# Shmaug/Stratum

Hardware: AMD Instinct MI355X
Metric: Mray/s at 1920x1080x1spp (1M-tri scene) (higher is better)
Workload: dtype f32; 1 GPU; procedural atrium, 1002352 triangles, 1920x1080, 1 sample(s)/pixel/step, default BDPT flags, radiance + albedo/visibility/depth/prev-uv AOVs written, pixel-tile shard 64x32 over 1 GPU(s); parallelism=single GPU, exchange=none, world_size=1, backend=none

## Files before the change

__graft_entry__.py:

```python
import os
import subprocess
import sys

ROOT = os.path.dirname(os.path.abspath(__file__))
if ROOT not in sys.path:
    sys.path.insert(0, ROOT)

CSRC = os.path.join(ROOT, "stratum_amd", "csrc")
LIB = os.path.join(ROOT, "stratum_amd", "libstratum_hip.so")

HIPCC_FLAGS = [
    "--offload-arch=gfx950",
    "-O3",
    "-std=c++17",
    "-fPIC",
    "-shared",
    "-ffp-contract=off",
    "-fno-fast-math",
    "-Wall",
    "-Wno-cuda-compat",
]


PRODUCT_SOURCES = ("api.hip", "shade_plain.hip", "shade_lt.hip", "shade_media.hip", "shade_media_lt.hip", "shade_media_lt2.hip", "trace_kernels.hip", "lbvh.hip", "lvc.hip", "hashgrid.hip", "wide.hip", "bvh_build.cpp",
                   "hdr_writer.cpp")


def _newer(target, sources):
    if not os.path.exists(target):
        return True
    t = os.path.getmtime(target)
    return any(os.path.getmtime(s) > t for s in sources)


def build_product(force=False):
    srcs = [os.path.join(CSRC, f) for f in PRODUCT_SOURCES]
    deps = srcs + [os.path.join(CSRC, f) for f in os.listdir(CSRC) if f.endswith(".h")]
    deps += [os.path.join(ROOT, "include", f) for f in os.listdir(os.path.join(ROOT, "include"))]
    if force or _newer(LIB, deps):
        from concurrent.futures import ThreadPoolExecutor

        hipcc = os.environ.get("HIPCC", "/opt/rocm/bin/hipcc")
        objdir = os.path.join(ROOT, "stratum_amd", "_obj")
        os.makedirs(objdir, exist_ok=True)
        compile_flags = [f for f in HIPCC_FLAGS if f != "-shared"]
        objs = [os.path.join(objdir, os.path.basename(s) + ".o") for s in srcs]

        headers = [d for d in deps if d not in srcs] + [os.path.abspath(__file__)]

        def compile_one(pair):
            src, obj = pair
            if force or _newer(obj, [src] + headers):
                subprocess.check_call([hipcc] + compile_flags + ["-c", "-o", obj, src])

        with ThreadPoolExecutor(max_workers=min(len(srcs), os.cpu_count() or 1)) as pool:
            list(pool.map(compile_one, zip(srcs, objs)))
        subprocess.check_call([hipcc, "--offload-arch=gfx950", "-shared", "-fPIC", "-o", LIB] + objs)
# ... 88 lines not shown
```

include/sthip.h:

```cpp
#ifndef STHIP_H
#define STHIP_H

#include <stdint.h>
#include "sthip_wire.h"

#ifdef __cplusplus
extern "C" {
#endif

#define STHIP_ABI_VERSION 11

typedef struct sthip_ctx sthip_ctx;

enum sthip_status {
  STHIP_OK = 0,
  STHIP_ERR_INVALID_ARGUMENT = -1,
  STHIP_ERR_NO_DEVICE = -2,
  STHIP_ERR_HIP = -3,
  STHIP_ERR_UNSUPPORTED = -4,
  STHIP_ERR_NO_SCENE = -5
};

typedef struct sthip_image_desc {
  const float* pixels;
// ... 120 lines not shown
  uint64_t rays_total;
  uint64_t rays_path;
  uint64_t rays_shadow;
  uint64_t nodes_visited;
  uint64_t tris_tested;
  uint64_t nodes_visited_shadow;
  uint64_t tris_tested_shadow;
  float ms_trace;
  float ms_shade;
  float ms_total;
  uint32_t launches_trace;
  uint32_t bvh_node_bytes;
  uint32_t bvh_tri_bytes;
  uint64_t bvh_nodes;
  uint64_t bvh_tris;
  float bvh_build_ms;
  float bvh_build_gpu_ms;
  uint64_t inner_slots[2];
  uint64_t tri_slots[2];
  uint64_t round_slots[2];
  uint64_t busy_rounds[2];
  uint64_t rays_primary_packets;
  uint64_t nodes_visited_primary;
  uint64_t tris_tested_primary;
  float ms_trace_primary;
  uint32_t launches_primary;
  uint64_t lane_states[8];
  uint64_t rays_answered;
  uint32_t paths_per_seed;
  uint32_t seeds_in_flight;
  uint64_t max_paths_in_flight;
  uint32_t batch_halvings;
  uint32_t full_rebuilds;
} sthip_stats;
int sthip_get_stats(sthip_ctx* ctx, sthip_stats* out);

enum { STHIP_CEILING_TRIAD = 0, STHIP_CEILING_NODE_GATHER_TABLE = 1, STHIP_CEILING_NODE_GATHER_L2 = 2, STHIP_CEILING_NODE_GATHER_L1 = 3 };
int sthip_measure_ceiling(sthip_ctx* ctx, uint32_t kind, double* gbytes_per_s);

int sthip_set_option(sthip_ctx* ctx, const char* name, int64_t value);


typedef struct sthip_accumulate_desc {
  uint32_t width, height;
  uint32_t view_count;
  uint32_t reprojection;
  uint32_t demodulate_albedo;
  float history_limit;
  uint32_t device_ptrs;
  uint32_t instance_count;
  const sthip_ViewData* gViews;
  const float* gRadiance;
  const float* gAlbedo;
  const sthip_VisibilityInfo* gVisibility;
  const sthip_DepthInfo* gDepth;
  const float* gPrevUVs;
  const sthip_VisibilityInfo* gPrevVisibility;
  const sthip_DepthInfo* gPrevDepth;
  const float* gPrevAccumColor;
  const float* gPrevAccumMoments;
  const uint32_t* gInstanceIndexMap;
  float* gAccumColor;
  float* gAccumMoments;
} sthip_accumulate_desc;
int sthip_accumulate(sthip_ctx* ctx, const sthip_accumulate_desc* desc);

// ... 43 lines not shown
```

stratum_amd/csrc/api.hip:

```cpp
#include <hip/hip_runtime.h>
#include <stdio.h>
#include <stdlib.h>
#include <string.h>

#include <algorithm>
#include <chrono>
#include <string>
#include <vector>

#include "../../include/sthip.h"
#include "bvh_build.h"
#include "kernel_instances.h"
#include "post.h"
#include "ceilings.h"

STHIP_DECLARE_KERNEL_INSTANCES

namespace sthip {
hipError_t lvc_compact(const float4* staging, uint32_t slots_per_seed, uint32_t seeds, uint32_t vertices_per_seed, float4* cache, uint32_t* counts, uint32_t* flags, uint32_t* offsets,
                       void* tmp, size_t& tmp_bytes, hipStream_t stream, uint32_t rec = 4, uint32_t flag_at = 2);
hipError_t hashgrid_build_device(const uint2* keys, const uint32_t* count, uint32_t slots, uint32_t buckets, uint32_t* checksums, uint32_t* counters, uint32_t* indices, uint32_t* dest, uint32_t* owner,
                                 uint32_t* bucket_of, uint32_t* append_index, uint32_t* sorted_bucket, uint32_t* sorted_append, unsigned long long* key64, unsigned long long* sorted_key64, void* tmp,
                                 size_t& tmp_bytes, hipStream_t stream, bool force_serial = false);
}
// ... 143 lines not shown
  std::vector<uint8_t> materials_host;
  std::vector<std::pair<uint32_t, uint32_t>> image_dims;
  uint32_t distribution_count = 0;
  bool has_specular = false;
  DevBuf<sthip_PackedVertexData> vertices;
  DevBuf<uint8_t> indices;
  DevBuf<sthip_InstanceData> instances;
  DevBuf<sthip_TransformData> xf, inv_xf, motion_xf;
  DevBuf<uint8_t> materials;
  DevBuf<uint32_t> lights;
  DevBuf<DeviceImage> images;
  DevBuf<float4> image_texels;
  uint32_t image_count = 0;
  DevBuf<float2> cone;
  uint32_t instance_count = 0, light_count = 0;
  DevBuf<BvhNodeSlot> nodes;
  DevBuf<BvhTri> tris;
  DevBuf<TlasEntry> entries;
  DevBuf<WideNode> wide_nodes;
  DevBuf<TlasEntry> wide_entries;
  DevBuf<Wide8Node> wide8_nodes;
  DevBuf<TlasEntry> wide8_entries;
  std::vector<Wide8Node> wide8_host;
  size_t wide8_node_count = 0;
  uint32_t tri_min_lanes = 1;
  DeviceBvh bvh{};
  uint64_t bvh_nodes = 0, bvh_tris = 0;
  PinnedNodes nodes_host;
  DevBuf<BvhNode> raw_nodes;
  DevBuf<BvhNodePacked> top_nodes;
  DevBuf<TlasEntry> top_entries;
  bool use_treetop = false;
  bool embed_leaves = false;
  int use_wide = 1;
  size_t wide_node_count = 0;
  sthip::DeviceWideScratch* wide_scratch = nullptr;
  bool want_wide = false;
  bool lds_materials = true;
  DevBuf<uint8_t> views;
  DevBuf<float4> ray_o, ray_d, hit, beta, radiance, shadow_sum, accum, shadow_rays, light_vertices, conn, media_state, shadow_hit, shadow_ext, shadow_result;
  DevBuf<uint32_t> view_medium;
  DevBuf<uint32_t> meta, queue0, queue1, queue_kept;
  int cull_terminal = 1;
  DevBuf<unsigned long long> counters;
  DevBuf<float> distributions;
  DevBuf<float4> presampled;
  DevBuf<float4> bdpt;
  DevBuf<float4> rr;
  DevBuf<uint2> cs_nee, cs_lvc;
  DevBuf<float4> lvc_staging, path_contrib;
  DevBuf<uint32_t> lvc_count, lvc_flags, lvc_offsets;
  DevBuf<uint8_t> lvc_tmp;
  DevBuf<float4> hg_appends, hg_compact, hg_data;
  DevBuf<uint32_t> hg_count, hg_flags, hg_offsets, hg_dest, hg_checksums, hg_counters, hg_indices;
  DevBuf<uint32_t> hg_owner, hg_bucket_of, hg_append, hg_sorted_bucket, hg_sorted_append;
  DevBuf<unsigned long long> hg_key64, hg_sorted_key64;
  DevBuf<uint2> hg_keys;
  DevBuf<uint8_t> hg_tmp;
  DevBuf<float4> lg_appends, lg_compact, lg_data;
  DevBuf<uint32_t> lg_checksums, lg_counters, lg_indices;
  DevBuf<uint32_t> light_trace;
  DevBuf<DeviceImage1> images1;
  DevBuf<float> image1_texels;
  DevBuf<BvhTriUv> tri_uvs;
  DevBuf<BvhTriShade> tri_shade;
  DevBuf<uint32_t> hit_leaf;
// ... 33 lines not shown
  DevBuf<float4> deep_rays;
  DevBuf<uint32_t> deep_count;
  sthip_stats stats{};
  hipError_t last_hip_error = hipSuccess;
  bool render_launched = false;
  bool stats_pending = false;
  hipEvent_t ev[2] = {nullptr, nullptr};
};

#define STHIP_MAX_STACK_LDS ((size_t)152 * 1024)
#define STHIP_MAX_STACK_DEPTH 512u

static const void* trace_kernel(bool count, bool alpha, bool bounded, bool top) {
  static const void* const table[16] = {
      (const void*)&k_trace<false, false, false, false>, (const void*)&k_trace<true, false, false, false>, (const void*)&k_trace<false, true, false, false>, (const void*)&k_trace<true, true, false, false>,
      (const void*)&k_trace<false, false, true, false>,  (const void*)&k_trace<true, false, true, false>,  (const void*)&k_trace<false, true, true, false>,  (const void*)&k_trace<true, true, true, false>,
      (const void*)&k_trace<false, false, false, true>,  (const void*)&k_trace<true, false, false, true>,  (const void*)&k_trace<false, true, false, true>,  (const void*)&k_trace<true, true, false, true>,
      (const void*)&k_trace<false, false, true, true>,   (const void*)&k_trace<true, false, true, true>,   (const void*)&k_trace<false, true, true, true>,   (const void*)&k_trace<true, true, true, true>};
  return table[(count ? 1 : 0) | (alpha ? 2 : 0) | (bounded ? 4 : 0) | (top ? 8 : 0)];
}
static const void* trace_kernel_wide8(bool count, bool alpha, bool bounded) {
  static const void* const table[8] = {
      (const void*)&k_trace<false, false, false, false, 2>, (const void*)&k_trace<true, false, false, false, 2>, (const void*)&k_trace<false, true, false, false, 2>, (const void*)&k_trace<true, true, false, false, 2>,
      (const void*)&k_trace<false, false, true, false, 2>,  (const void*)&k_trace<true, false, true, false, 2>,  (const void*)&k_trace<false, true, true, false, 2>,  (const void*)&k_trace<true, true, true, false, 2>};
  return table[(count ? 1 : 0) | (alpha ? 2 : 0) | (bounded ? 4 : 0)];
}
static const void* trace_kernel_wide(bool count, bool alpha, bool bounded) {
  static const void* const table[8] = {
      (const void*)&k_trace<false, false, false, false, 1>, (const void*)&k_trace<true, false, false, false, 1>, (const void*)&k_trace<false, true, false, false, 1>, (const void*)&k_trace<true, true, false, false, 1>,
      (const void*)&k_trace<false, false, true, false, 1>,  (const void*)&k_trace<true, false, true, false, 1>,  (const void*)&k_trace<false, true, true, false, 1>,  (const void*)&k_trace<true, true, true, false, 1>};
  return table[(count ? 1 : 0) | (alpha ? 2 : 0) | (bounded ? 4 : 0)];
}

#define HIP_TRY(ctx, expr)                                                                            \
  do {                                                                                                \
    hipError_t _e = (expr);                                                                           \
    if (_e != hipSuccess) {                                                                           \
      (ctx)->error = std::string(#expr) + ": " + hipGetErrorString(_e);                               \
      (ctx)->last_hip_error = _e;                                                                     \
      return STHIP_ERR_HIP;                                                                           \
    }                                                                                                 \
  } while (0)

static void fill_counter_stats(sthip_ctx* ctx, const unsigned long long* c) {
  ctx->stats.rays_total = c[CNT_RAYS_CLOSEST] + c[CNT_RAYS_SHADOW];
  ctx->stats.rays_path = c[CNT_RAYS_CLOSEST] - c[CNT_CROSSINGS];
  ctx->stats.rays_shadow = c[CNT_RAYS_SHADOW];
  ctx->stats.nodes_visited = c[CNT_NODES];
  ctx->stats.tris_tested = c[CNT_TRIS];
  ctx->stats.nodes_visited_shadow = c[CNT_NODES + 1];
  ctx->stats.tris_tested_shadow = c[CNT_TRIS + 1];
  for (int k = 0; k < 2; k++) {
    ctx->stats.inner_slots[k] = c[CNT_INNER_SLOTS + k];
    ctx->stats.tri_slots[k] = c[CNT_TRI_SLOTS + k];
    ctx->stats.round_slots[k] = c[CNT_ROUND_SLOTS + k];
    ctx->stats.busy_rounds[k] = c[CNT_BUSY_ROUNDS + k];
  }
  for (int k = 0; k < 8; k++) ctx->stats.lane_states[k] = c[CNT_LANE_STATES + k];
  ctx->stats.rays_answered = c[CNT_RAYS_ANSWERED];
  ctx->stats.nodes_visited_primary = c[CNT_NODES_PRIMARY];
  ctx->stats.tris_tested_primary = c[CNT_TRIS_PRIMARY];
}

static uint32_t grid_for_early(const sthip_ctx* ctx, size_t n) {
  const size_t blocks = (n + STHIP_BLOCK - 1) / STHIP_BLOCK;
  return (uint32_t)std::max<size_t>(1, std::min(blocks, (size_t)ctx->cu_count * 32));
}

static int fail(sthip_ctx* ctx, int code, const std::string& msg) {
  ctx->error = msg;
  return code;
}

extern "C" {

int sthip_abi_version(void) { return STHIP_ABI_VERSION; }

int sthip_create(int device, sthip_ctx** out_ctx) {
  if (!out_ctx) {
    g_create_error = "out_ctx is NULL";
    return STHIP_ERR_INVALID_ARGUMENT;
  }
  *out_ctx = nullptr;
  int count = 0;
  hipError_t e = hipGetDeviceCount(&count);
  if (e != hipSuccess || count == 0) {
    g_create_error = std::string("no HIP device: ") + (e != hipSuccess ? hipGetErrorString(e) : "device count is 0") +
                     " (libstratum_hip has no CPU backend)";
    return STHIP_ERR_NO_DEVICE;
  }
  if (device < 0 || device >= count) {
    g_create_error = "device index out of range";
    return STHIP_ERR_INVALID_ARGUMENT;
  }
  e = hipSetDevice(device);
  if (e != hipSuccess) {
    g_create_error = std::string("hipSetDevice: ") + hipGetErrorString(e);
    return STHIP_ERR_HIP;
  }
  sthip_ctx* ctx = new sthip_ctx();
  ctx->device = device;
  hipDeviceProp_t prop;
  if (hipGetDeviceProperties(&prop, device) == hipSuccess) {
    ctx->cu_count = prop.multiProcessorCount;
    size_t free_bytes = 0, total_bytes = 0;
    if (hipMemGetInfo(&free_bytes, &total_bytes) != hipSuccess) free_bytes = prop.totalGlobalMem;
    uint64_t paths = 1ull << 18;
    while (paths * 2 * 4096 <= (uint64_t)free_bytes && paths < (1ull << 27)) paths *= 2;
    ctx->max_paths_in_flight = paths;
  }
  (void)hipEventCreate(&ctx->ev[0]);
  (void)hipEventCreate(&ctx->ev[1]);
  {
    const int lds_max = 160 * 1024;
    for (int k = 0; k < 16; k++) (void)hipFuncSetAttribute(trace_kernel((k & 1) != 0, (k & 2) != 0, (k & 4) != 0, (k & 8) != 0), hipFuncAttributeMaxDynamicSharedMemorySize, lds_max);
    for (int k = 0; k < 8; k++) (void)hipFuncSetAttribute(trace_kernel_wide((k & 1) != 0, (k & 2) != 0, (k & 4) != 0), hipFuncAttributeMaxDynamicSharedMemorySize, lds_max);
    for (int k = 0; k < 8; k++) (void)hipFuncSetAttribute(trace_kernel_wide8((k & 1) != 0, (k & 2) != 0, (k & 4) != 0), hipFuncAttributeMaxDynamicSharedMemorySize, lds_max);
    (void)hipFuncSetAttribute(reinterpret_cast<const void*>(&k_trace_batch<false, false>), hipFuncAttributeMaxDynamicSharedMemorySize, lds_max);
    (void)hipFuncSetAttribute(reinterpret_cast<const void*>(&k_trace_batch<true, false>), hipFuncAttributeMaxDynamicSharedMemorySize, lds_max);
    (void)hipFuncSetAttribute(reinterpret_cast<const void*>(&k_trace_batch<false, true>), hipFuncAttributeMaxDynamicSharedMemorySize, lds_max);
    (void)hipFuncSetAttribute(reinterpret_cast<const void*>(&k_trace_batch<true, true>), hipFuncAttributeMaxDynamicSharedMemorySize, lds_max);
  }
  ctx->stats.bvh_node_bytes = sizeof(BvhNodePacked);
  ctx->stats.bvh_tri_bytes = sizeof(BvhTri);
  *out_ctx = ctx;
  return STHIP_OK;
}

void sthip_destroy(sthip_ctx* ctx) {
  if (!ctx) return;
  (void)hipSetDevice(ctx->device);
  (void)hipDeviceSynchronize();
  sthip::device_wide_scratch_destroy(ctx->wide_scratch);
  ctx->wide_scratch = nullptr;
  ctx->vertices.release();
  ctx->volume_words.release();
  ctx->volumes.release();
  ctx->indices.release();
  ctx->instances.release();
  ctx->xf.release();
  ctx->inv_xf.release();
  ctx->motion_xf.release();
  ctx->materials.release();
  ctx->lights.release();
  ctx->images.release();
  ctx->image_texels.release();
  ctx->cone.release();
  ctx->nodes.release();
  ctx->tris.release();
  ctx->entries.release();
// ... 56 lines not shown
int sthip_set_shard(sthip_ctx* ctx, uint32_t shard_rank, uint32_t shard_count, uint32_t tile_w, uint32_t tile_h) {
  if (!ctx) return STHIP_ERR_INVALID_ARGUMENT;
  if (shard_count == 0 || shard_rank >= shard_count || tile_w == 0 || tile_h == 0 || (tile_w & 7u) || (tile_h & 7u))
    return fail(ctx, STHIP_ERR_INVALID_ARGUMENT, "shard: need rank < count and tile sizes that are multiples of 8");
  ctx->shard_rank = shard_rank;
  ctx->shard_count = shard_count;
  ctx->tile_w = tile_w;
  ctx->tile_h = tile_h;
  return STHIP_OK;
}

int sthip_set_option(sthip_ctx* ctx, const char* name, int64_t value) {
  if (!ctx || !name) return STHIP_ERR_INVALID_ARGUMENT;
  if (!strcmp(name, "count_traversal"))
    ctx->count_traversal = value != 0;
  else if (!strcmp(name, "time_kernels"))
    ctx->time_kernels = value != 0;
  else if (!strcmp(name, "fuse_trace"))
    ctx->fuse_trace = value != 0;
  else if (!strcmp(name, "packet_primary"))
    ctx->packet_primary = value != 0;
  else if (!strcmp(name, "answer_last_rays"))
    ctx->answer_last_rays = value != 0;
  else if (!strcmp(name, "cull_terminal"))
    ctx->cull_terminal = value != 0;
  else if (!strcmp(name, "refill_idle"))
    ctx->refill_idle = (uint32_t)std::min<int64_t>(64, std::max<int64_t>(1, value));
  else if (!strcmp(name, "bvh_builder"))
    ctx->bvh_builder = value == 1 ? 1 : 0;
  else if (!strcmp(name, "lds_materials"))
    ctx->lds_materials = value != 0;
  else if (!strcmp(name, "embed_leaves"))
    ctx->embed_leaves = value != 0;
  else if (!strcmp(name, "keep_scene")) {
    ctx->keep_scene = value != 0;
    if (!ctx->keep_scene) ctx->kept = KeptScene();
  } else if (!strcmp(name, "wide_bvh"))
    ctx->use_wide = (int)std::min<int64_t>(std::max<int64_t>(value, 0), 3);
  else if (!strcmp(name, "poison_deep_queue")) {
    if (value && ctx->deep_count.p) {
      const uint32_t junk[2] = {5u, 3u};
      (void)hipSetDevice(ctx->device);
      (void)hipStreamSynchronize(ctx->stream);
      if (hipMemcpy(ctx->deep_count.p, junk, 8, hipMemcpyHostToDevice) != hipSuccess) return fail(ctx, STHIP_ERR_HIP, "poison_deep_queue: copy failed");
    }
  } else if (!strcmp(name, "tri_min_lanes"))
    ctx->tri_min_lanes = ctx->bvh.wide8_tri_min = (uint32_t)std::min<int64_t>(std::max<int64_t>(value, 1), 64);
  else if (!strcmp(name, "lbvh_algorithm"))
    ctx->lbvh_algorithm = value == 0 ? 0 : 1;
  else if (!strcmp(name, "lds_stack_levels")) {
    ctx->lds_stack_cap = ctx->lds_stack_threshold = (uint32_t)std::min<int64_t>(std::max<int64_t>(value, 4), 150);
  } else if (!strcmp(name, "ploc_radius"))
    ctx->ploc_radius = (int)std::min<int64_t>(std::max<int64_t>(value, 1), 32);
  else if (!strcmp(name, "sah_top"))
    ctx->sah_top_size = value <= 0 ? 0u : (uint32_t)std::min<int64_t>(std::max<int64_t>(value, 16), 1 << 20);
  else if (!strcmp(name, "max_paths_in_flight"))
    ctx->max_paths_in_flight = (uint64_t)std::max<int64_t>(1, value);
  else if (!strcmp(name, "trace_blocks_per_cu"))
    ctx->trace_blocks_per_cu = (uint32_t)std::min<int64_t>(16, std::max<int64_t>(0, value));
  else if (!strcmp(name, "treetop"))
    ctx->use_treetop = value != 0;
  else if (!strcmp(name, "hashgrid_serial"))
    ctx->hashgrid_serial = value != 0;
  else if (!strcmp(name, "reuse_grids_persist")) {
    ctx->reuse_persist = value != 0;
    ctx->reuse_grids_valid = false;
// ... 174 lines not shown
  if (s->image_count && !s->gImages) return fail(ctx, STHIP_ERR_INVALID_ARGUMENT, "scene: image_count > 0 but gImages is NULL");
  if (s->image1_count && !s->gImage1s) return fail(ctx, STHIP_ERR_INVALID_ARGUMENT, "scene: image1_count > 0 but gImage1s is NULL");
  if (s->volume_count && !s->gVolumes) return fail(ctx, STHIP_ERR_INVALID_ARGUMENT, "scene: volume_count > 0 but gVolumes is NULL");
  sthip::BuiltBvh built;
  std::string err;
  const uint32_t n = s->instance_count;
  const bool device_build = ctx->bvh_builder == sthip::BVH_BUILDER_LBVH_GPU;
  sthip::DeviceBuildTarget target;
  if (device_build) {
    ctx->has_scene = false;
    HIP_TRY(ctx, ctx->vertices.ensure(std::max(1u, s->vertex_count)));
    HIP_TRY(ctx, ctx->indices.ensure((size_t)s->indices_bytes + 8));
    if (s->vertex_count) HIP_TRY(ctx, hipMemcpy(ctx->vertices.p, s->gVertices, (size_t)s->vertex_count * sizeof(sthip_PackedVertexData), hipMemcpyHostToDevice));
    HIP_TRY(ctx, hipMemset(ctx->indices.p + s->indices_bytes, 0, 8));
    if (s->indices_bytes) HIP_TRY(ctx, hipMemcpy(ctx->indices.p, s->gIndices, s->indices_bytes, hipMemcpyHostToDevice));
    target.vertices = ctx->vertices.p;
    target.vertex_count = s->vertex_count;
    target.indices = ctx->indices.p;
    target.stream = ctx->stream;
    target.algorithm = ctx->lbvh_algorithm;
    target.ploc_radius = ctx->ploc_radius;
    target.sah_top_size = ctx->lbvh_algorithm == 1 ? ctx->sah_top_size : 0;
    target.user = ctx;
    target.reserve = [](void* user, size_t node_capacity, size_t tri_capacity, sthip::DeviceBuildTarget& self) {
      sthip_ctx* c = (sthip_ctx*)user;
      if (c->nodes.ensure(node_capacity) != hipSuccess || c->raw_nodes.ensure(node_capacity) != hipSuccess || c->tris.ensure(tri_capacity) != hipSuccess) return false;
      self.nodes = c->nodes.p;
      self.raw_nodes = c->raw_nodes.p;
      self.tris = c->tris.p;
      return true;
    };
  }
  const auto t_build0 = std::chrono::steady_clock::now();
  if (!sthip::build_scene_bvh(*s, built, err, ctx->bvh_builder, device_build ? &target : nullptr, ctx->embed_leaves && STHIP_NODE_STRIDE == 48))
    return fail(ctx, err.find("only triangle") != std::string::npos ? STHIP_ERR_UNSUPPORTED : STHIP_ERR_INVALID_ARGUMENT, "scene: " + err);

  if (((size_t)built.dev_nodes + built.nodes.size() + 2 * built.entries.size() + 2) * sizeof(BvhNodeSlot) > 0xFFFFFFFFull || ((size_t)built.dev_tris + built.tris.size()) * sizeof(BvhTri) > 0xFFFFFFFFull)
    return fail(ctx, STHIP_ERR_UNSUPPORTED, "scene: the acceleration structure exceeds 4 GiB (the traversal addresses nodes and triangles with 32-bit byte offsets)");
  if (built.stack_depth > STHIP_MAX_STACK_DEPTH) return fail(ctx, STHIP_ERR_UNSUPPORTED, "scene: the acceleration structure is too deep for the traversal stack (use the SAH builder)");
  ctx->stats.bvh_build_ms = std::chrono::duration<float, std::milli>(std::chrono::steady_clock::now() - t_build0).count();
  ctx->stats.bvh_build_gpu_ms = built.gpu_build_ms;
  {
    std::vector<EmitterBounds> bounds;
    bool usable = true;
    for (uint32_t i = 0; i < s->instance_count && usable; i++) {
      if ((s->gInstances[i].packed[0] & 0xF) != STHIP_INSTANCE_TYPE_TRIANGLES || !(ctx->inst_flags_host[i] & INST_FLAG_EMITS)) continue;
      if (bounds.size() == STHIP_MAX_EMITTER_BOUNDS) {
        usable = false;
        break;
      }
      const uint32_t prims = (s->gInstances[i].packed[1] >> 12) & 0xFFFFu, stride = s->gInstances[i].packed[1] >> 28;
      const uint32_t first_vertex = s->gInstances[i].packed[2];
      const uint8_t* ib = (const uint8_t*)s->gIndices + s->gInstances[i].packed[3];
      EmitterBounds b{};
      for (int a = 0; a < 3; a++) b.lo[a] = __builtin_inff(), b.hi[a] = -__builtin_inff();
      for (uint32_t k = 0; k < 3 * prims; k++) {
        uint32_t index;
        if (stride == 2) {
          uint16_t w;
          memcpy(&w, ib + 2 * (size_t)k, 2);
          index = w;
        } else {
          memcpy(&index, ib + 4 * (size_t)k, 4);
        }
        if ((size_t)first_vertex + index >= s->vertex_count) {
          usable = false;
          break;
// ... 195 lines not shown
    ctx->bvh.image1_texels = ctx->image1_texels.p;
    ctx->bvh.alpha_test = 0;
    ctx->bvh.flip_uvs = 0;
  }
  {
    size_t words = 0;
    for (uint32_t i = 0; i < s->volume_count; i++) {
      built.volumes[i].first_word = (uint32_t)words;
      words += (size_t)(s->gVolumes[i].bytes / 4);
    }
    if (words > 0xFFFFFFFFull) return fail(ctx, STHIP_ERR_INVALID_ARGUMENT, "scene: gVolumes exceed 16 GiB");
    HIP_TRY(ctx, ctx->volume_words.ensure(std::max<size_t>(1, words)));
    HIP_TRY(ctx, ctx->volumes.ensure(std::max<size_t>(1, built.volumes.size())));
    for (uint32_t i = 0; i < s->volume_count; i++)
      HIP_TRY(ctx, hipMemcpy(ctx->volume_words.p + built.volumes[i].first_word, s->gVolumes[i].data, (size_t)s->gVolumes[i].bytes, hipMemcpyHostToDevice));
    if (!built.volumes.empty()) HIP_TRY(ctx, hipMemcpy(ctx->volumes.p, built.volumes.data(), built.volumes.size() * sizeof(DeviceVolume), hipMemcpyHostToDevice));
    ctx->volume_count = s->volume_count;
    ctx->has_volumes = false;
    ctx->volume_instances = 0;
    ctx->instance_is_volume.assign(n, 0);
    for (uint32_t i = 0; i < n; i++)
      if ((s->gInstances[i].packed[0] & 0xF) == STHIP_INSTANCE_TYPE_VOLUME) {
        ctx->has_volumes = true;
        ctx->volume_instances++;
        ctx->instance_is_volume[i] = 1;
      }
    ctx->bvh.volumes = ctx->volumes.p;
  }
  ctx->bvh.nodes = reinterpret_cast<const float4*>(ctx->nodes.p);
  ctx->bvh.tris = built.embedded ? reinterpret_cast<const float4*>(ctx->nodes.p) : reinterpret_cast<const float4*>(ctx->tris.p);
  ctx->bvh.entries = ctx->entries.p;
  ctx->bvh.root_ref = built.root_ref;
  ctx->bvh.top_is_world_blas = built.top_is_world_blas;
  ctx->bvh.stack_depth = built.stack_depth;
  ctx->bvh.scene_cx = built.scene_center[0];
  ctx->bvh.scene_cy = built.scene_center[1];
  ctx->bvh.scene_cz = built.scene_center[2];
  ctx->bvh.scene_radius = built.scene_radius;
  ctx->bvh_nodes = nodes_total;
  ctx->bvh_tris = tris_total;
  ctx->top = std::move(built.top);
  if (ctx->want_wide && built.dev_nodes != 0) {
    const int rc = collapse_resident_tree(ctx);
    if (rc != STHIP_OK) return rc;
  }
  ctx->nodes_host.n = 0;
  if (ctx->use_treetop) {
    HIP_TRY(ctx, ctx->nodes_host.ensure(std::max<size_t>(nodes_total, ctx->nodes.n)));
    if (built.dev_nodes) HIP_TRY(ctx, hipMemcpy(ctx->nodes_host.p, ctx->raw_nodes.p, (size_t)built.dev_nodes * sizeof(BvhNode), hipMemcpyDeviceToHost));
    if (!built.nodes.empty()) memcpy(ctx->nodes_host.p + built.dev_nodes, built.nodes.data(), built.nodes.size() * sizeof(BvhNode));
    ctx->nodes_host.n = nodes_total;
  }
  {
    const size_t units = built.embedded ? nodes_total : tris_total;
    HIP_TRY(ctx, ctx->tri_shade.ensure(std::max<size_t>(1, units)));
    if (ctx->has_alpha) {
      HIP_TRY(ctx, ctx->tri_uvs.ensure(std::max<size_t>(1, units)));
      ctx->bvh.tri_uv = reinterpret_cast<const float2*>(ctx->tri_uvs.p);
    }
    if (units && s->vertex_count) {
      DevBuf<uint8_t> is_tri;
      if (built.embedded) {
        std::vector<uint8_t> flags(units, 0);
        for (size_t u = 0; u < built.unit_tri.size() && u < units; u++) flags[u] = built.unit_tri[u] != 0xFFFFFFFFu;
        HIP_TRY(ctx, is_tri.ensure(units));
        HIP_TRY(ctx, hipMemcpy(is_tri.p, flags.data(), units, hipMemcpyHostToDevice));
      }
      hipLaunchKernelGGL(k_fill_tri_shade, dim3(grid_for_early(ctx, units)), dim3(STHIP_BLOCK), 0, ctx->stream, reinterpret_cast<const BvhTri*>(ctx->bvh.tris), (uint32_t)units, is_tri.p, ctx->vertices.p, s->vertex_count,
                         ctx->indices.p, (uint64_t)s->indices_bytes, ctx->tri_shade.p, ctx->has_alpha ? ctx->tri_uvs.p : nullptr);
      HIP_TRY(ctx, hipGetLastError());
      HIP_TRY(ctx, hipStreamSynchronize(ctx->stream));
    }
  }
  {
    const int rc = configure_stack(ctx);
    if (rc != STHIP_OK) return rc;
  }
  ctx->has_scene = true;
  ctx->reuse_grids_valid = false;
  if (ctx->keep_scene) {
    if (s->gVertices != ctx->kept.vertices.data() || !ctx->kept.valid) ctx->kept.keep(*s);
  } else {
    ctx->kept = KeptScene();
  }
  if (getenv("STHIP_VERBOSE")) {
    int per_cu = 0;
    per_cu = trace_occupancy(ctx, trace_lds_bytes(ctx));
    fprintf(stderr, "[sthip] bvh (%s): %zu nodes, %zu tris, %zu top-level entries, stack depth %u (%zu B LDS / block%s, treetop %u nodes), %d trace blocks / CU, build %.1f ms (GPU kernels %.2f ms)\n",
            ctx->bvh_builder ? "lbvh/gpu" : "sah/host", (size_t)ctx->bvh_nodes, (size_t)ctx->bvh_tris, built.entries.size(), built.stack_depth, stack_bytes(ctx), ctx->bvh.spill ? ", bounded" : "", ctx->bvh.top_count, per_cu, ctx->stats.bvh_build_ms,
            ctx->stats.bvh_build_gpu_ms);
  }
  return STHIP_OK;
}

static unsigned long long* queue_ctl_host(unsigned long long* qctl, uint32_t kind, uint32_t depth) {
  return qctl + (size_t)((kind * 64u + depth) * QUEUE_SEGMENTS) * QCTL_STRIDE;
}
static uint32_t grid_for(const sthip_ctx* ctx, size_t n) {
  const size_t blocks = (n + STHIP_BLOCK - 1) / STHIP_BLOCK;
  const size_t cap = (size_t)ctx->cu_count * 32;
  return (uint32_t)std::max<size_t>(1, std::min(blocks, cap));
}
static int trace_occupancy(const sthip_ctx* ctx, size_t lds_bytes) {
  int per_cu = 0;
  hipError_t e;
  e = hipOccupancyMaxActiveBlocksPerMultiprocessor(&per_cu,
                                                   ctx->bvh.wide8_nodes  ? trace_kernel_wide8(false, false, ctx->bvh.spill != nullptr)
                                                   : ctx->bvh.wide_nodes ? trace_kernel_wide(false, false, ctx->bvh.spill != nullptr)
                                                                         : trace_kernel(false, false, ctx->bvh.spill != nullptr, ctx->use_treetop),
                                                   STHIP_BLOCK, lds_bytes);
  return e == hipSuccess ? per_cu : 0;
}
static uint32_t trace_grid(sthip_ctx* ctx, size_t lds_bytes) {
  int per_cu = trace_occupancy(ctx, lds_bytes);
  if (per_cu < 1) per_cu = 2;
  if (ctx->trace_blocks_per_cu) per_cu = (int)ctx->trace_blocks_per_cu;
  return (uint32_t)(ctx->cu_count * per_cu);
}
static size_t stack_bytes(const sthip_ctx* ctx) { return (size_t)ctx->bvh.lds_levels * STHIP_BLOCK * (ctx->bvh.wide8_nodes ? sizeof(uint2) : sizeof(uint32_t)); }

static size_t trace_lds_bytes(const sthip_ctx* ctx) { return stack_bytes(ctx) + (size_t)ctx->bvh.top_count * sizeof(BvhNodePacked); }

static int configure_stack(sthip_ctx* ctx) {
  const uint32_t need = ctx->bvh.wide8_nodes ? ctx->bvh.wide8_stack_depth : ctx->bvh.wide_nodes ? ctx->bvh.wide_stack_depth + 3u : ctx->bvh.stack_depth;
  const bool bounded = ctx->bvh.wide8_nodes ? 2u * need > ctx->lds_stack_threshold : need > ctx->lds_stack_threshold;
  ctx->bvh.lds_levels = bounded ? (ctx->bvh.wide8_nodes ? std::max(4u, ctx->lds_stack_cap / 2u) : ctx->lds_stack_cap) : need;
  ctx->bvh.spill = nullptr;
  if (bounded) {
    HIP_TRY(ctx, ctx->spill.ensure((size_t)ctx->cu_count * 8 * STHIP_BLOCK * ctx->bvh.stack_depth));
    ctx->bvh.spill = ctx->spill.p;
  }
  return refresh_treetop(ctx);
}

static int refresh_treetop(sthip_ctx* ctx) {
  ctx->bvh.top_nodes = nullptr;
  ctx->bvh.top_entries = ctx->bvh.entries;
  ctx->bvh.top_root_ref = ctx->bvh.root_ref;
  ctx->bvh.top_count = 0;
  if (!ctx->use_treetop || ctx->nodes_host.empty()) return STHIP_OK;
  int per_cu = 0;
  const size_t stack = stack_bytes(ctx);
  per_cu = trace_occupancy(ctx, stack);
// ... 711 lines not shown
      HIP_TRY(ctx, hipEventElapsedTime(&ms, ctx->ev[0], ctx->ev[1]));
      acc += ms;
    }
    return STHIP_OK;
  };

  ctx->render_launched = true;
  if (ctx->bvh.spill && ctx->deep_count.p) HIP_TRY(ctx, hipMemsetAsync(ctx->deep_count.p, 0, 8, st));
  bool counters_cleared = false;
  const bool nee = (sampling_flags & (1u << STHIP_eNEE)) != 0;
  const bool ext = ctx->has_spheres || has_env || bdpt || (sampling_flags & ((1u << STHIP_eNEEReservoirs) | (1u << STHIP_eShadingNormalShadowFix)));
  for (uint32_t s = 0; s < seed_count; s += batch) {
    const uint32_t in_flight = std::min(batch, seed_count - s);
    p.seed = seed_begin + s;
    p.seeds_in_flight = in_flight;
    p.write_aov = s == 0 ? 1u : 0u;
    int rc = STHIP_OK;
    auto reset_queues = [&]() -> int {
      const uint32_t per_depth = QUEUE_SEGMENTS * QCTL_STRIDE;
      const uint32_t words = (max_bounce_rounds + drain_rounds + 1) * per_depth;
      hipLaunchKernelGGL(k_clear, dim3(std::max(1u, std::min(64u, (2 * words + CNT_TOTAL + STHIP_BLOCK - 1) / STHIP_BLOCK))), dim3(STHIP_BLOCK), 0, st, queue_ctl_host(ctx->qctl.p, 0, 0), words,
                         queue_ctl_host(ctx->qctl.p, 1, 0), words, ctx->counters.p, counters_cleared ? 0u : (uint32_t)CNT_TOTAL);
      counters_cleared = true;
      if (p.shadow_debug) HIP_TRY(ctx, hipMemsetAsync(queue_ctl_host(ctx->qctl.p, 2, 0), 0, (size_t)words * 8, st));
      HIP_TRY(ctx, hipGetLastError());
      return STHIP_OK;
    };
    auto trace = [&](uint32_t dc, uint32_t ds) -> int {
      if (dc == TRACE_NONE && ds == TRACE_NONE) return STHIP_OK;
      launches_trace++;
      return timed(ms_trace, [&]() {
        const bool alpha = p.bvh.alpha_test || ctx->has_volumes;
        void* kargs[3] = {(void*)&p, (void*)&dc, (void*)&ds};
        (void)hipLaunchKernel(p.bvh.wide8_nodes  ? trace_kernel_wide8(ctx->count_traversal, alpha, p.bvh.spill != nullptr)
                              : p.bvh.wide_nodes ? trace_kernel_wide(ctx->count_traversal, alpha, p.bvh.spill != nullptr)
                                                 : trace_kernel(ctx->count_traversal, alpha, p.bvh.spill != nullptr, p.bvh.top_count != 0),
                              dim3(tgrid), dim3(STHIP_BLOCK), kargs, lds, st);
        if (p.bvh.spill) {
          const uint32_t dgrid = (uint32_t)ctx->cu_count * 8u;
          if (alpha) {
            if (ctx->count_traversal)
              hipLaunchKernelGGL((k_trace_deep<true, true>), dim3(dgrid), dim3(STHIP_BLOCK), 0, st, p);
            else
              hipLaunchKernelGGL((k_trace_deep<false, true>), dim3(dgrid), dim3(STHIP_BLOCK), 0, st, p);
          } else if (ctx->count_traversal)
            hipLaunchKernelGGL((k_trace_deep<true, false>), dim3(dgrid), dim3(STHIP_BLOCK), 0, st, p);
          else
            hipLaunchKernelGGL((k_trace_deep<false, false>), dim3(dgrid), dim3(STHIP_BLOCK), 0, st, p);
        }
        if (p.shadow_debug && ds != TRACE_NONE) {
          FrameParams q = p;
          q.shadow_rays = p.shadow_debug;
          q.radiance = p.debug;
          q.shadow_sum = p.debug;
          q.qctl = p.qctl + (size_t)64 * QUEUE_SEGMENTS * QCTL_STRIDE;
          const uint32_t none = TRACE_NONE;
          void* qargs[3] = {(void*)&q, (void*)&none, (void*)&ds};
          (void)hipLaunchKernel(p.bvh.wide8_nodes  ? trace_kernel_wide8(false, alpha, p.bvh.spill != nullptr)
                                : p.bvh.wide_nodes ? trace_kernel_wide(false, alpha, p.bvh.spill != nullptr)
                                                   : trace_kernel(false, alpha, p.bvh.spill != nullptr, p.bvh.top_count != 0),
                                dim3(tgrid), dim3(STHIP_BLOCK), qargs, lds, st);
          if (p.bvh.spill) {
            const uint32_t dgrid = (uint32_t)ctx->cu_count * 8u;
            if (alpha)
              hipLaunchKernelGGL((k_trace_deep<false, true>), dim3(dgrid), dim3(STHIP_BLOCK), 0, st, q);
            else
              hipLaunchKernelGGL((k_trace_deep<false, false>), dim3(dgrid), dim3(STHIP_BLOCK), 0, st, q);
          }
        }
      });
    };
    auto trace_primary = [&]() -> int {
      launches_primary++;
      rays_primary += (uint64_t)primary_rays * in_flight;
      const uint32_t packets = (p.path_count + 63) / 64;
      const unsigned pgrid = std::max(1u, std::min((packets + 3) / 4, (uint32_t)ctx->cu_count * 64u));
      const size_t plds = ((size_t)ctx->bvh.stack_depth * (STHIP_BLOCK / 64) + 13 * STHIP_BLOCK) * sizeof(uint32_t);
      return timed(ms_primary, [&]() {
        if (p.bvh.alpha_test) {
          if (ctx->count_traversal)
            hipLaunchKernelGGL((k_trace_primary<true, true>), dim3(pgrid), dim3(STHIP_BLOCK), plds, st, p);
          else
            hipLaunchKernelGGL((k_trace_primary<false, true>), dim3(pgrid), dim3(STHIP_BLOCK), plds, st, p);
        } else if (ctx->count_traversal)
          hipLaunchKernelGGL((k_trace_primary<true, false>), dim3(pgrid), dim3(STHIP_BLOCK), plds, st, p);
        else
          hipLaunchKernelGGL((k_trace_primary<false, false>), dim3(pgrid), dim3(STHIP_BLOCK), plds, st, p);
      });
    };
    auto run_rounds = [&](bool light, bool shadow_rays, auto&& shade) -> int {
      for (uint32_t depth = 0; depth <= max_bounce_rounds; depth++) {
        const uint32_t dc = depth < max_bounce_rounds ? depth : TRACE_NONE;
        const uint32_t ds = depth >= 1 && shadow_rays && depth - 1 <= max_shadow_round ? depth - 1 : TRACE_NONE;
        int r;
        if (!light && depth == 0 && dc == 0 && ctx->packet_primary && !ctx->has_volumes) {
          r = trace_primary();
        } else if (ctx->fuse_trace) {
          r = trace(dc, ds);
        } else {
          r = trace(TRACE_NONE, ds);
          if (!r) r = trace(dc, TRACE_NONE);
        }
        if (r) return r;
        if (media && ds != TRACE_NONE) {
          r = timed(ms_shade, [&]() { hipLaunchKernelGGL(k_shadow_media, dim3(grid), dim3(STHIP_BLOCK), 0, st, p, ds); });
          if (r) return r;
        }
        if (dc == TRACE_NONE) break;
        r = timed(ms_shade, [&]() { shade(depth); });
        if (r) return r;
      }
      if (media && shadow_rays)
        for (uint32_t ds = max_bounce_rounds; ds < max_bounce_rounds + drain_rounds; ds++) {
          int r = trace(TRACE_NONE, ds);
          if (!r) r = timed(ms_shade, [&]() { hipLaunchKernelGGL(k_shadow_media, dim3(grid), dim3(STHIP_BLOCK), 0, st, p, ds); });
          if (r) return r;
        }
      return STHIP_OK;
    };

// ... 539 lines not shown
```

stratum_amd/csrc/bvh.h:

```cpp
#pragma once
#include <stdint.h>

#define BVH_LEAF_BIT 0x80000000u
#define BVH_INST_BIT 0x40000000u
#define BVH_TOP_BIT 0x40000000u
#define BVH_MAX_LEAF_TRIS 2
#define BVH_INVALID_REF 0xFFFFFFFFu

struct BvhNode {
  float n0xy[4];
  float n1xy[4];
  float nz[4];
  uint32_t ref[4];
};

struct BvhTri {
  float v0[3];
  uint32_t id;
  float v1[3];
  uint32_t src_indices;
  float v2[3];
  uint32_t src_vertex;
};
struct BvhTriShade {
  float n0[3], v0;
  float n1[3], v1;
  float n2[3], v2;
  float u[3], pad;
};
struct BvhNodePacked {
  float n0xy[4];
  float n1xy[4];
  float nz[4];
};
#ifndef STHIP_NODE_STRIDE
#define STHIP_NODE_STRIDE 48
#endif
#define BVH_NODE_BYTES ((unsigned)STHIP_NODE_STRIDE)
struct BvhNodeSlot {
  BvhNodePacked n;
#if STHIP_NODE_STRIDE > 48
  uint32_t pad[(STHIP_NODE_STRIDE - 48) / 4];
#endif
};
struct WideNode {
  float origin[3];
  uint8_t exp[4];
  uint8_t q[6][4];
  uint32_t pad[2];
  uint32_t ref[4];
};
struct Wide8Node {
  float origin[3];
  uint8_t exp[3];
  uint8_t imask;
  uint32_t child_base;
// ... 47 lines not shown
```

stratum_amd/csrc/bvh_build.cpp:

```cpp
#include "bvh_build.h"

#include <math.h>
#include <cmath>
#include <stdlib.h>
#include <string.h>

#include <algorithm>
#include <atomic>
#include <limits>
#include <map>
#include <queue>
#include <thread>
#include <unordered_map>
#include <tuple>

namespace sthip {
namespace {

struct Box {
  float lo[3], hi[3];
  void reset() {
    for (int a = 0; a < 3; a++) {
      lo[a] = INFINITY;
      hi[a] = -INFINITY;
// ... 246 lines not shown
  return memcmp(&t, I, sizeof(I)) == 0;
}

struct InstView {
  uint32_t type, material_address, prim_count, stride, first_vertex, indices_byte_offset;
};
inline InstView view(const sthip_InstanceData& d) {
  InstView v;
  v.type = d.packed[0] & 0xF;
  v.material_address = d.packed[0] >> 4;
  v.prim_count = (d.packed[1] >> 12) & 0xFFFF;
  v.stride = d.packed[1] >> 28;
  v.first_vertex = d.packed[2];
  v.indices_byte_offset = d.packed[3];
  return v;
}
inline void load_tri(const sthip_scene_desc& s, const InstView& in, uint32_t prim, uint32_t tri[3]) {
  const uint8_t* ib = (const uint8_t*)s.gIndices;
  const size_t off = (size_t)in.indices_byte_offset + (size_t)prim * 3 * in.stride;
  if (in.stride == 2) {
    uint16_t w[3];
    memcpy(w, ib + off, 6);
    tri[0] = w[0];
    tri[1] = w[1];
    tri[2] = w[2];
  } else {
    memcpy(tri, ib + off, 12);
  }
  for (int k = 0; k < 3; k++) tri[k] += in.first_vertex;
}

}

bool build_scene_bvh(const sthip_scene_desc& s, BuiltBvh& out, std::string& err, int builder, DeviceBuildTarget* device, bool embed_leaves) {
  out = BuiltBvh();
  const bool dev_mode = device != nullptr && builder == BVH_BUILDER_LBVH_GPU;
  const uint32_t DEVICE_MIN_PRIMS = 64;
  out.embedded = embed_leaves && builder == BVH_BUILDER_SAH_HOST;
  const uint32_t BLAS_DEPTH_CAP = 22, TLAS_DEPTH_CAP = 18, LBVH_MAX_HEIGHT = 120;
  if (s.indices_bytes > 0xFFFFFFFFull || s.vertex_count >= 0x80000000u) {
    err = "gIndices beyond 4 GiB or more than 2^31 vertices";
    return false;
  }
  std::vector<uint32_t> merged, separate, spheres, volumes;
  for (uint32_t i = 0; i < s.volume_count; i++) {
    const uint8_t* b = (const uint8_t*)s.gVolumes[i].data;
    const uint64_t n = s.gVolumes[i].bytes;
    auto rd32 = [&](uint64_t off) { uint32_t v = 0; if (off + 4 <= n) memcpy(&v, b + off, 4); return v; };
    auto rd64 = [&](uint64_t off) { uint64_t v = 0; if (off + 8 <= n) memcpy(&v, b + off, 8); return v; };
    auto rdf = [&](uint64_t off) { float v = 0; if (off + 4 <= n) memcpy(&v, b + off, 4); return v; };
    if (!b || n < 672 + 64 + 64 || n > 0xFFFFFFF0ull || (n & 3) || rd64(0) != 0x304244566f6e614eull || rd32(636) != 1u) {
      err = "gVolumes entry is not a NanoVDB float grid (magic / grid type / size)";
      return false;
    }
    DeviceVolume v;
    memset(&v, 0, sizeof(v));
    v.bytes = (uint32_t)n;
    const uint64_t root = 672 + rd64(672 + 24);
    if (root + 64 > n) {
      err = "gVolumes entry: the root node lies outside the buffer";
      return false;
    }
    v.root = (uint32_t)root;
    const uint64_t tiles = rd32(root + 24);
    if (tiles > 65536 || root + 64 + 32 * tiles > n) {
      err = "gVolumes entry: the root tile table lies outside the buffer";
      return false;
// ... 39 lines not shown
      continue;
    }
    if (in.type != STHIP_INSTANCE_TYPE_TRIANGLES) {
      err = "unknown instance type";
      return false;
    }
    if (in.stride != 2 && in.stride != 4) {
      err = "index stride must be 2 or 4";
      return false;
    }
    const size_t end = (size_t)in.indices_byte_offset + (size_t)in.prim_count * 3 * in.stride;
    if (end > s.indices_bytes) {
      err = "instance index range exceeds gIndices";
      return false;
    }
    if ((size_t)in.material_address + sizeof(sthip_MaterialRecord) > s.material_bytes) {
      err = "instance material_address exceeds gMaterialData";
      return false;
    }
    if (!dev_mode)
      for (uint32_t p = 0; p < in.prim_count; p++) {
        uint32_t tri[3];
        load_tri(s, in, p, tri);
        for (int k = 0; k < 3; k++)
          if (tri[k] >= s.vertex_count) {
            err = "vertex index exceeds gVertices";
            return false;
          }
      }
    if (is_identity(s.gInstanceInverseTransforms[i]) && is_identity(s.gInstanceTransforms[i]))
      merged.push_back(i);
    else
      separate.push_back(i);
  }

  std::vector<uint32_t> inst_alpha(s.instance_count, BVH_NO_ALPHA);
  bool any_alpha = false;
  for (uint32_t i = 0; i < s.instance_count; i++) {
    const InstView in = view(s.gInstances[i]);
    if (in.type != STHIP_INSTANCE_TYPE_TRIANGLES) continue;
    sthip_MaterialRecord rec;
    memcpy(&rec, (const uint8_t*)s.gMaterialData + in.material_address, sizeof(rec));
    if (rec.alpha_mask_index < STHIP_IMAGE_COUNT) {
      if (rec.alpha_mask_index >= s.image1_count) {
        err = "a material refers to an alpha mask that is not in gImage1s";
        return false;
      }
      inst_alpha[i] = rec.alpha_mask_index;
      any_alpha = true;
    }
  }

  std::string gpu_err;
  auto prim_total = [&](const std::vector<uint32_t>& insts) {
    size_t n = 0;
    for (uint32_t i : insts) n += view(s.gInstances[i]).prim_count;
    return n;
  };
  uint32_t dev_node_cursor = 0, dev_tri_cursor = 0;
  if (dev_mode) {
    size_t dev_nodes = 0, dev_tris = 0, all_prims = 0, meshes_n = 0;
    auto account = [&](size_t n) {
      if (n == 0) return;
      all_prims += n;
      meshes_n++;
      if (n >= DEVICE_MIN_PRIMS) {
// ... 88 lines not shown
      std::vector<BvhTri> tin(prims.size());
      bounds.reset();
      for (size_t k = 0; k < prims.size(); k++) {
        const InstView in = view(s.gInstances[prims[k].first]);
        uint32_t tri[3];
        load_tri(s, in, prims[k].second, tri);
        BvhTri& t = tin[k];
        memcpy(t.v0, s.gVertices[tri[0]].position, 12);
        memcpy(t.v1, s.gVertices[tri[1]].position, 12);
        memcpy(t.v2, s.gVertices[tri[2]].position, 12);
        t.id = (prims[k].second << 16) | (with_instance_bits ? prims[k].first : 0u);
        t.src_indices = in.indices_byte_offset + prims[k].second * 3u * in.stride;
        t.src_vertex = in.first_vertex | (in.stride == 4u ? 0x80000000u : 0u);
        bounds.grow(t.v0);
        bounds.grow(t.v1);
        bounds.grow(t.v2);
      }
      uint32_t root = 0;
      float ms = 0;
      const size_t nodes_before = out.nodes.size(), tris_before = out.tris.size();
      if (!lbvh_build_gpu(tin, out.nodes, out.tris, root, depth, ms, gpu_err)) return BVH_INVALID_REF;
      out.gpu_build_ms += ms;
      if (depth <= LBVH_MAX_HEIGHT) return root;
      out.nodes.resize(nodes_before);
      out.tris.resize(tris_before);
    }
    std::vector<Box> boxes(prims.size());
    bounds.reset();
    for (size_t k = 0; k < prims.size(); k++) {
      const InstView in = view(s.gInstances[prims[k].first]);
      uint32_t tri[3];
      load_tri(s, in, prims[k].second, tri);
      boxes[k].reset();
      for (int v = 0; v < 3; v++) boxes[k].grow(s.gVertices[tri[v]].position);
      bounds.grow(boxes[k]);
    }
    uint32_t leaf_tris = BVH_MAX_LEAF_TRIS;
    if (const char* e = getenv("STHIP_LEAF_TRIS")) leaf_tris = (uint32_t)std::min(4, std::max(1, atoi(e)));
    Builder b(boxes, leaf_tris, BLAS_DEPTH_CAP);
    depth = b.max_depth;
    const uint32_t tri_base = (uint32_t)out.tris.size();
    out.tris.resize(tri_base + prims.size());
    for (size_t k = 0; k < prims.size(); k++) {
      const auto& pr = prims[b.order[k]];
      const InstView in = view(s.gInstances[pr.first]);
      uint32_t tri[3];
      load_tri(s, in, pr.second, tri);
      BvhTri& t = out.tris[tri_base + k];
      memcpy(t.v0, s.gVertices[tri[0]].position, 12);
      memcpy(t.v1, s.gVertices[tri[1]].position, 12);
      memcpy(t.v2, s.gVertices[tri[2]].position, 12);
      t.id = (pr.second << 16) | (with_instance_bits ? pr.first : 0u);
      t.src_indices = in.indices_byte_offset + pr.second * 3u * in.stride;
      t.src_vertex = in.first_vertex | (in.stride == 4u ? 0x80000000u : 0u);
    }
    const uint32_t root = flatten(b, 0, out.nodes, [&](uint32_t first, uint32_t count) {
      if (!out.embedded) return BVH_LEAF_BIT | ((tri_base + first) << 2) | (count - 1);
      out.unit_tri.resize(out.nodes.size(), 0xFFFFFFFFu);
      const uint32_t unit = (uint32_t)out.nodes.size();
      for (uint32_t k = 0; k < count; k++) {
        out.nodes.push_back(BvhNode());
        memset(&out.nodes.back(), 0, sizeof(BvhNode));
        out.unit_tri.push_back(tri_base + first + k);
      }
      return BVH_LEAF_BIT | (unit << 2) | (count - 1);
    });
    if (root & BVH_LEAF_BIT) {
      depth = 1;
      return wrap_leaf(out.nodes, bounds, root);
    }
    return root;
  };

  Box scene_box;
  scene_box.reset();
  uint32_t blas_depth = 0;
  std::vector<Box> entry_boxes;

  std::vector<uint8_t> entry_root_local;
  if (!merged.empty()) {
    const size_t total = prim_total(merged);
    if (total > 0) {
      if (total >= (1u << 28)) {
        err = "too many triangles";
        return false;
      }
      Box bounds;
// ... 109 lines not shown
    memset(&e, 0, sizeof(e));
    memcpy(e.inv, &s.gInstanceInverseTransforms[i], 48);
    e.root = s.gInstances[i].packed[2];
    e.id_bits = i;
    e.identity = TLAS_ENTRY_VOLUME;
    const DeviceVolume& v = out.volumes[e.root];
    const sthip_TransformData& xf = s.gInstanceTransforms[i];
    Box wb;
    wb.reset();
    for (int c = 0; c < 8; c++) {
      const float ip[3] = {(float)((c & 1) ? v.bbox_max[0] + 1 : v.bbox_min[0]), (float)((c & 2) ? v.bbox_max[1] + 1 : v.bbox_min[1]), (float)((c & 4) ? v.bbox_max[2] + 1 : v.bbox_min[2])};
      float gw[3], wp[3];
      for (int a = 0; a < 3; a++) gw[a] = ip[0] * v.matf[3 * a] + ip[1] * v.matf[3 * a + 1] + ip[2] * v.matf[3 * a + 2] + v.vecf[a];
      for (int a = 0; a < 3; a++) wp[a] = xf.m[a][0] * gw[0] + xf.m[a][1] * gw[1] + xf.m[a][2] * gw[2] + xf.m[a][3];
      wb.grow(wp);
    }
    for (int a = 0; a < 3; a++) {
      const float pad = 1e-3f * (wb.hi[a] - wb.lo[a]) + 1e-5f * std::max(fabsf(wb.lo[a]), fabsf(wb.hi[a]));
      wb.lo[a] -= pad;
      wb.hi[a] += pad;
    }
    out.entries.push_back(e);
    entry_boxes.push_back(wb);
    scene_box.grow(wb);
  }

  if (dev_mode)
    for (size_t k = 0; k < entry_root_local.size(); k++)
      if (entry_root_local[k]) out.entries[k].root += out.dev_nodes;
  out.top.entries = out.entries;
  out.top.volumes = out.volumes;
  out.top.instance_count = s.instance_count;
  out.top.merged.assign(s.instance_count, 0);
  for (uint32_t i : merged) out.top.merged[i] = 1;
  out.top.blas_nodes = out.dev_nodes + (uint32_t)out.nodes.size();
  out.top.blas_depth = blas_depth;
  out.top.obj_box.assign(6 * out.entries.size(), 0.f);
  for (size_t k = 0; k < out.entries.size(); k++) {
    const TlasEntry& e = out.entries[k];
    if (e.identity == TLAS_ENTRY_IDENTITY) {
      out.top.has_merged = true;
      memcpy(out.top.merged_box, entry_boxes[k].lo, 12);
      memcpy(out.top.merged_box + 3, entry_boxes[k].hi, 12);
    } else if (e.identity == TLAS_ENTRY_TRANSFORMED) {
      const InstView in = view(s.gInstances[e.id_bits]);
      const Box& ob = meshes.at(std::make_tuple(in.first_vertex, in.indices_byte_offset, in.prim_count, in.stride)).bounds;
      memcpy(&out.top.obj_box[6 * k], ob.lo, 12);
      memcpy(&out.top.obj_box[6 * k + 3], ob.hi, 12);
    }
  }

  uint32_t tlas_depth = 0;
  if (out.entries.empty()) {
    out.root_ref = BVH_INVALID_REF;
    out.top_is_world_blas = 1;
  } else if (out.entries.size() == 1 && out.entries[0].identity == TLAS_ENTRY_IDENTITY) {
    out.root_ref = out.entries[0].root;
    out.top_is_world_blas = 1;
  } else {
    if (out.entries.size() >= 0xFFFE) {
      err = "too many top-level entries";
      return false;
    }
    Builder b(entry_boxes, 1, TLAS_DEPTH_CAP);
    tlas_depth = b.max_depth + 1;
    out.root_ref = flatten(b, 0, out.nodes, [&](uint32_t first, uint32_t) { return BVH_LEAF_BIT | BVH_INST_BIT | b.order[first]; });
    if (out.root_ref & BVH_LEAF_BIT) {
// ... 642 lines not shown
  wide8_stack_depth = 0;
  if (st.wide8_root.size() != st.entries.size() || root_ref == BVH_INVALID_REF) return false;
  if (top_is_world_blas) {
    if (st.entries.empty() || st.wide8_root[0] == BVH_INVALID_REF) return false;
    entries = st.entries;
    for (size_t k = 0; k < entries.size(); k++)
      if (st.wide8_root[k] != BVH_INVALID_REF) entries[k].root = st.wide8_root[k];
    wide8_root = st.wide8_root[0];
    wide8_stack_depth = (st.wide8_height.empty() ? st.wide8_blas_height : st.wide8_height[0]) + 2;
    return true;
  }
  if ((root_ref & BVH_LEAF_BIT) || root_ref < tlas_base) return false;
  Wide8Builder wb(nodes);
  wb.st = &st;
  wb.tlas = tlas;
  wb.tlas_base = tlas_base;
  wb.entries_out = &entries;
  const uint32_t w = (uint32_t)nodes.size();
  nodes.push_back(Wide8Node());
  const uint32_t top_height = wb.fill(w, root_ref, true, st.wide8_blas_height);
  if (!wb.ok || nodes.size() >= (1u << 24) || entries.size() >= 0x7FFFFFFFu) return false;
  wide8_root = w;
  wide8_stack_depth = top_height + 2;
  return true;
}

bool rebuild_top_level(TopLevelState& st, const sthip_TransformData* xf, const sthip_TransformData* inv, uint32_t instance_count, std::vector<BvhNode>& tlas_nodes, uint32_t& root_ref,
                       uint32_t& top_is_world_blas, uint32_t& stack_depth, float scene_center[3], float& scene_radius, std::string& err) {
  const uint32_t TLAS_DEPTH_CAP = 18;
  if (instance_count != st.instance_count) {
    err = "the instance count changed: upload the scene again";
    return false;
  }
  for (uint32_t i = 0; i < instance_count; i++)
    if (st.merged[i] && !(is_identity(xf[i]) && is_identity(inv[i]))) {
      err = "an instance of the merged world-space mesh (identity transform at upload) moved: upload the scene again";
      return false;
    }
  Box scene_box;
  scene_box.reset();
  std::vector<Box> entry_boxes(st.entries.size());
  for (size_t k = 0; k < st.entries.size(); k++) {
    TlasEntry& e = st.entries[k];
    Box wb;
    wb.reset();
    if (e.identity == TLAS_ENTRY_IDENTITY) {
      memcpy(wb.lo, st.merged_box, 12);
      memcpy(wb.hi, st.merged_box + 3, 12);
    } else {
      const uint32_t i = e.id_bits;
      memcpy(e.inv, &inv[i], 48);
      const sthip_TransformData& M = xf[i];
      if (e.identity == TLAS_ENTRY_SPHERE) {
        const float r = fabsf(e.radius);
        for (int a = 0; a < 3; a++) {
          const float c = M.m[a][3];
          const float pad = 1e-3f * r + 1e-5f * fabsf(c);
          wb.lo[a] = c - r - pad;
          wb.hi[a] = c + r + pad;
        }
      } else {
        float corners[8][3];
        if (e.identity == TLAS_ENTRY_VOLUME) {
          const DeviceVolume& v = st.volumes[e.root];
          for (int c = 0; c < 8; c++) {
            const float ip[3] = {(float)((c & 1) ? v.bbox_max[0] + 1 : v.bbox_min[0]), (float)((c & 2) ? v.bbox_max[1] + 1 : v.bbox_min[1]), (float)((c & 4) ? v.bbox_max[2] + 1 : v.bbox_min[2])};
            for (int a = 0; a < 3; a++) corners[c][a] = ip[0] * v.matf[3 * a] + ip[1] * v.matf[3 * a + 1] + ip[2] * v.matf[3 * a + 2] + v.vecf[a];
          }
        } else {
          const float* ob = &st.obj_box[6 * k];
          for (int c = 0; c < 8; c++)
// ... 125 lines not shown
```

stratum_amd/csrc/bvh_build.h:

```cpp
#pragma once
#include <math.h>
#include <stdint.h>
#include <string.h>

#include <string>
#include <vector>

#include "../../include/sthip.h"
#include "bvh.h"

#if defined(__HIPCC__)
#define STHIP_BVH_HD __host__ __device__
#else
#define STHIP_BVH_HD
#endif

namespace sthip {

struct TopLevelState {
  std::vector<TlasEntry> entries;
  std::vector<float> obj_box;
  std::vector<uint8_t> merged;
  std::vector<DeviceVolume> volumes;
  uint32_t instance_count = 0;
  uint32_t blas_nodes = 0;
  uint32_t blas_depth = 0;
  float merged_box[6] = {0, 0, 0, 0, 0, 0};
  bool has_merged = false;
  std::vector<uint32_t> wide8_root;
  std::vector<uint32_t> wide8_height;
  uint32_t wide8_blas_nodes = 0;
  uint32_t wide8_blas_height = 0;
};

struct BuiltBvh {
  std::vector<BvhNode> nodes;
  std::vector<BvhTri> tris;
  bool any_alpha = false;
  std::vector<uint32_t> inst_alpha;
  std::vector<TlasEntry> entries;
  std::vector<DeviceVolume> volumes;
  uint32_t root_ref = BVH_INVALID_REF;
  uint32_t top_is_world_blas = 1;
  uint32_t stack_depth = 4;
  float scene_center[3] = {0, 0, 0};
  float scene_radius = 0;
  float gpu_build_ms = 0;
  uint32_t dev_nodes = 0, dev_tris = 0;
  std::vector<uint8_t> absolute_ref;
  bool embedded = false;
  std::vector<uint32_t> unit_tri;
  TopLevelState top;
  std::vector<WideNode> wide_nodes;
  std::vector<TlasEntry> wide_entries;
  uint32_t wide_root_ref = BVH_INVALID_REF;
  uint32_t wide_stack_depth = 0;
  std::vector<Wide8Node> wide8_nodes;
  std::vector<TlasEntry> wide8_entries;
  uint32_t wide8_root = BVH_INVALID_REF;
  uint32_t wide8_stack_depth = 0;
};

struct MeshPiece {
  uint32_t id_bits;
  uint32_t first_vertex;
  uint32_t indices_byte_offset;
  uint32_t stride;
  uint32_t prim_count;
  uint32_t prim_begin;
};

struct DeviceBuildTarget {
  const sthip_PackedVertexData* vertices = nullptr;
  uint32_t vertex_count = 0;
  const uint8_t* indices = nullptr;
  BvhNodeSlot* nodes = nullptr;
  BvhNode* raw_nodes = nullptr;
  BvhTri* tris = nullptr;
  void* stream = nullptr;
  int algorithm = 1;
  int ploc_radius = 4;
  uint32_t sah_top_size = 0;
  bool (*reserve)(void* user, size_t node_capacity, size_t tri_capacity, DeviceBuildTarget& self) = nullptr;
  void* user = nullptr;
};
struct FrontierEntry {
  float lo[3];
  uint32_t ref;
  float hi[3];
  uint32_t height;
};
bool lbvh_build_device(const DeviceBuildTarget& tgt, const std::vector<MeshPiece>& pieces, uint32_t node_base, uint32_t tri_base, uint32_t& root_ref, uint32_t& height, float bounds[6],
                       float& gpu_ms, std::string& err, std::vector<FrontierEntry>* frontier = nullptr, uint32_t frontier_size = 0);

enum BvhBuilderKind { BVH_BUILDER_SAH_HOST = 0, BVH_BUILDER_LBVH_GPU = 1 };

bool build_scene_bvh(const sthip_scene_desc& scene, BuiltBvh& out, std::string& err, int builder = BVH_BUILDER_SAH_HOST, DeviceBuildTarget* device = nullptr, bool embed_leaves = false);
void build_wide_bvh(BuiltBvh& out);

void build_wide8_bvh(BuiltBvh& out);
bool build_wide8_top(const TopLevelState& st, const BvhNode* tlas, uint32_t tlas_base, uint32_t root_ref, bool top_is_world_blas, std::vector<Wide8Node>& nodes, std::vector<TlasEntry>& entries,
                     uint32_t& wide8_root, uint32_t& wide8_stack_depth);

bool rebuild_top_level(TopLevelState& st, const sthip_TransformData* xf, const sthip_TransformData* inv, uint32_t instance_count, std::vector<BvhNode>& tlas_nodes, uint32_t& root_ref,
                       uint32_t& top_is_world_blas, uint32_t& stack_depth, float scene_center[3], float& scene_radius, std::string& err);

struct Treetop {
  std::vector<BvhNode> nodes;
  std::vector<TlasEntry> entries;
  uint32_t root_ref = BVH_INVALID_REF;
};
void build_treetop(const BvhNode* nodes, size_t node_count, const std::vector<TlasEntry>& entries, uint32_t root_ref, uint32_t capacity, Treetop& out);

STHIP_BVH_HD inline uint32_t pack_plane(float v, bool upper, uint32_t byte) {
  if (!(v > -3.0e38f)) v = -3.0e38f;
  if (v > 3.0e38f) v = 3.0e38f;
  uint32_t u;
  memcpy(&u, &v, 4);
  const bool negative = (u >> 31) != 0;
  const uint32_t m = u & 0x7FFFFFFFu;
  uint32_t sign, M;
  const bool outward_grows = upper != negative;
  if (outward_grows) {
    sign = negative ? 0x80000000u : 0u;
    M = (m + 255u) & ~255u;
  } else if (m >= 255u) {
    sign = negative ? 0x80000000u : 0u;
    M = (m - 255u) & ~255u;
  } else {
    sign = negative ? 0u : 0x80000000u;
// ... 151 lines not shown
```

stratum_amd/csrc/kernel_instances.h:

```cpp
#pragma once
#include "kernels.h"

#define STHIP_SHADE_PLAIN(X) \
  X(false, false, false, 0, false, false) X(true, false, false, 0, false, false) X(false, true, false, 0, false, false) X(true, true, false, 0, false, false) \
  X(false, true, false, 0, true, false) X(true, true, false, 0, true, false) X(true, true, false, 0, false, true)
#define STHIP_SHADE_LT(X) \
  X(false, true, true, 0, false, false) X(true, true, true, 0, false, false) X(false, true, true, 0, true, false) X(true, true, true, 0, true, false) X(true, true, true, 0, false, true)
#define STHIP_SHADE_MEDIA(X) \
  X(false, true, false, 1, false, false) X(true, true, false, 1, false, false) X(true, true, false, 1, false, true) X(false, true, false, 2, false, false) X(true, true, false, 2, false, false) \
  X(true, true, false, 2, false, true)
#define STHIP_SHADE_MEDIA_LT(X) X(false, true, true, 1, false, false) X(true, true, true, 1, false, false) X(true, true, true, 1, false, true)
#define STHIP_SHADE_MEDIA_LT2(X) X(false, true, true, 2, false, false) X(true, true, true, 2, false, false) X(true, true, true, 2, false, true)
#define STHIP_TRACE_ROWS(Y, TOP, WIDE) \
  Y(false, false, false, TOP, WIDE) Y(true, false, false, TOP, WIDE) Y(false, true, false, TOP, WIDE) Y(true, true, false, TOP, WIDE) Y(false, false, true, TOP, WIDE) Y(true, false, true, TOP, WIDE) \
  Y(false, true, true, TOP, WIDE) Y(true, true, true, TOP, WIDE)
#define STHIP_TRACE_ALL(Y) STHIP_TRACE_ROWS(Y, false, 0) STHIP_TRACE_ROWS(Y, true, 0) STHIP_TRACE_ROWS(Y, false, 1) STHIP_TRACE_ROWS(Y, false, 2)
#define STHIP_SHADE_LIGHT(Z) Z(false, true, false) Z(true, true, false) Z(false, true, true) Z(true, true, true)

#define STHIP_SHADE_EXTERN(T, E, L, M, P, D) extern template __global__ void k_shade<T, E, L, M, P, D>(FrameParams, uint32_t);
#define STHIP_SHADE_DEFINE(T, E, L, M, P, D) template __global__ void k_shade<T, E, L, M, P, D>(FrameParams, uint32_t);
#define STHIP_TRACE_EXTERN(C, A, B, T, W) extern template __global__ void k_trace<C, A, B, T, W>(FrameParams, uint32_t, uint32_t);
#define STHIP_TRACE_DEFINE(C, A, B, T, W) template __global__ void k_trace<C, A, B, T, W>(FrameParams, uint32_t, uint32_t);
#define STHIP_LIGHT_EXTERN(T, E, M) extern template __global__ void k_shade_light<T, E, M>(FrameParams, uint32_t);
#define STHIP_LIGHT_DEFINE(T, E, M) template __global__ void k_shade_light<T, E, M>(FrameParams, uint32_t);

#define STHIP_DECLARE_KERNEL_INSTANCES \
  STHIP_SHADE_PLAIN(STHIP_SHADE_EXTERN) STHIP_SHADE_LT(STHIP_SHADE_EXTERN) STHIP_SHADE_MEDIA(STHIP_SHADE_EXTERN) STHIP_SHADE_MEDIA_LT(STHIP_SHADE_EXTERN) STHIP_SHADE_MEDIA_LT2(STHIP_SHADE_EXTERN) STHIP_TRACE_ALL(STHIP_TRACE_EXTERN) \
      STHIP_SHADE_LIGHT(STHIP_LIGHT_EXTERN)
```

stratum_amd/csrc/kernels.h:

```cpp
#pragma once

#include "shading.h"
#include "hashgrid.h"
#include "medium.h"
#include "traverse.h"
#include <type_traits>

#define STHIP_BLOCK 256

enum {
  CNT_RAYS_CLOSEST = 0,
  CNT_RAYS_SHADOW = 1,
  CNT_NODES = 2,
  CNT_TRIS = 4,
  CNT_INNER_SLOTS = 6,
  CNT_TRI_SLOTS = 8,
  CNT_ROUND_SLOTS = 10,
  CNT_BUSY_ROUNDS = 12,
  CNT_NODES_PRIMARY = 14,
  CNT_TRIS_PRIMARY = 15,
  CNT_CROSSINGS = 16,
  CNT_RAYS_ANSWERED = 17,
  CNT_LANE_STATES = 20,
  CNT_TOTAL = 28
};

struct FrameParams {
  DeviceScene scene;
  DeviceBvh bvh;
  sthip_BDPTPushConstants pc;
  uint32_t sampling_flags;
  uint32_t scene_flags;
  uint32_t seed;
  uint32_t seeds_in_flight;
  uint32_t paths_per_seed;
  const sthip_ViewData* views;
  const sthip_TransformData* view_xf;
  const sthip_ViewData* prev_views;
  const sthip_TransformData* prev_inv_view_xf;
  uint32_t shard_rank, shard_count, tile_w, tile_h, tiles_x, tiles_y;
  uint32_t path_count;
  float4* ray_o;
  float4* ray_d;
  float4* hit;
  uint32_t debug_mode;
  float4* debug;
  void* out_debug;
  float4* shadow_debug;
  uint32_t* hit_leaf;
  float4* beta;
  uint32_t* meta;
  float4* radiance;
  float4* shadow_sum;
  float2* cone;
  float4* accum;
  uint32_t* queue[2];
  float4* bdpt;
// ... 228 lines not shown
    p.shadow_hit[slot] = make_float4(hit.t, hit.b1, hit.b2, __uint_as_float(hit.ip));
  } else if (!any) {
    p.hit[slot] = make_float4(hit.t, hit.b1, hit.b2, __uint_as_float(hit.ip));
    p.hit_leaf[slot] = hit.leaf;
  } else if (hit.ip == 0xFFFFFFFFu) {
    if (slot & 0x80000000u) {
      uint32_t* lt = p.light_trace + 4 * (size_t)(slot & 0x7FFFFFFFu);
      const float q = (float)p.light_trace_quantization;
      const float cf[3] = {fmaxf(0.0f, contribution.x) * q, fmaxf(0.0f, contribution.y) * q, fmaxf(0.0f, contribution.z) * q};
      uint32_t overflow = 0;
      for (int k = 0; k < 3; k++) {
        const uint32_t ci = cf[k] >= 4294967296.0f ? 0xFFFFFFFFu : (cf[k] == cf[k] ? (uint32_t)cf[k] : 0u);
        if (ci) {
          const uint32_t prev = atomicAdd(&lt[k], ci);
          if (ci > 0xFFFFFFFFu - prev) overflow |= 1u << k;
        }
      }
      if (overflow) atomicOr(&lt[3], overflow);
    } else if (slot & 0x40000000u) {
      p.conn[slot & 0x3FFFFFFFu] = make_float4(contribution.x, contribution.y, contribution.z, 0.0f);
    } else {
      float4 c = target[slot];
      c.x = c.x + contribution.x;
      c.y = c.y + contribution.y;
      c.z = c.z + contribution.z;
      target[slot] = c;
    }
  }
}

#ifndef STHIP_TRACE_ATTR
#define STHIP_TRACE_ATTR
#endif
template <bool COUNT, bool ALPHA, bool BOUNDED = false, bool TOP = false, int WIDE = 0>
__global__ void __launch_bounds__(STHIP_BLOCK) STHIP_TRACE_ATTR k_trace(FrameParams p, uint32_t depth_closest, uint32_t depth_shadow) {
  extern __shared__ uint32_t lds_stack[];
  float4* top_lds = reinterpret_cast<float4*>(lds_stack + (size_t)p.bvh.lds_levels * STHIP_BLOCK);
  DeviceBvh bvh = p.bvh;
  if (TOP) {
    for (uint32_t i = threadIdx.x; i < p.bvh.top_count * 3u; i += STHIP_BLOCK) top_lds[i] = p.bvh.top_nodes[i];
    __syncthreads();
    if (p.bvh.top_count) {
      bvh.entries = p.bvh.top_entries;
      bvh.root_ref = p.bvh.top_root_ref;
    }
  }
  const bool first = depth_closest == 0;
  const uint32_t* queue = p.queue[depth_closest & 1u];
  unsigned long long* ctl_c = queue_ctl(p.qctl, 0, depth_closest == TRACE_NONE ? 0u : depth_closest, 0);
  unsigned long long* ctl_s = queue_ctl(p.qctl, 1, depth_shadow == TRACE_NONE ? 0u : depth_shadow, 0);
  uint32_t* stack = lds_stack + (WIDE == 2 ? 2u * threadIdx.x : threadIdx.x);
  float4* target = flag(p, STHIP_eDeferShadowRays) ? p.shadow_sum : p.radiance;
  TraverseCounters cnt[2];
  cnt[0].clear();
  cnt[1].clear();
  uint32_t round_slots[2] = {0, 0}, busy_rounds[2] = {0, 0};
  if (WIDE == 1) {
    bvh.entries = p.bvh.wide_entries;
    bvh.root_ref = p.bvh.wide_root_ref;
  }
  if (WIDE == 2) {
    bvh.entries = p.bvh.wide8_entries;
    bvh.root_ref = p.bvh.wide8_root;
  }
  typename std::conditional<WIDE == 2, Traversal8<COUNT, STHIP_BLOCK, ALPHA, BOUNDED, STHIP_ENTRY_BATCH>,
                            Traversal<TRAV_MIXED, COUNT, STHIP_BLOCK, ALPHA, TOP, BOUNDED, true, STHIP_ENTRY_BATCH, WIDE == 1>>::type tr;
  if constexpr (WIDE == 2) {
    tr.tri_min = p.bvh.wide8_tri_min;
    if (BOUNDED) tr.limit = (p.bvh.lds_levels - 1u) * STHIP_BLOCK;
  } else {
    tr.top_lds = (const LdsFloat4*)top_lds;
    if (BOUNDED) tr.limit = (p.bvh.lds_levels - (WIDE ? 3u : 1u)) * STHIP_BLOCK;
  }
  tr.reset();
  tr.any = false;
  WaveWork work_c, work_s;
  work_c.init();
  work_s.init();
  work_c.exhausted = depth_closest == TRACE_NONE;
  work_s.exhausted = depth_shadow == TRACE_NONE;
  uint32_t slot = 0;
  f3 contribution = F3s(0.0f);
  bool busy = false;
  bool shadow_lane = false;
  for (;;) {
    const unsigned long long idle = __ballot(!busy || !tr.active());
    if ((uint32_t)__popcll(idle) >= p.refill_idle || idle == ~0ull) {
      if (COUNT && (threadIdx.x & 63u) == 0) cnt[0].st[7] += 64;
      if (busy && !tr.active()) {
        if (BOUNDED && tr.overflowed(stack)) {
          const uint32_t e = atomicAdd(p.deep_count, 1u);
          float4* rec = p.deep_rays + 4 * (size_t)e;
          rec[0] = make_float4(tr.o.x, tr.o.y, tr.o.z, tr.tmin);
          rec[1] = make_float4(tr.d.x, tr.d.y, tr.d.z, tr.tmax);
          rec[2] = make_float4(contribution.x, contribution.y, contribution.z, __uint_as_float(slot));
          rec[3] = make_float4(__uint_as_float((shadow_lane ? 1u : 0u) | (tr.any ? 2u : 0u)), 0.0f, 0.0f, 0.0f);
        } else {
          finish_ray<ALPHA>(p, target, slot, shadow_lane, tr.any, tr.hit, contribution);
        }
// ... 16 lines not shown
      }
      if (work_c.exhausted && !work_s.exhausted) {
        uint32_t idx = work_s.take(!busy, ctl_s, p.shadow_stride, 0);
        if (idx != 0xFFFFFFFFu) {
          if (ALPHA && p.media && (depth_shadow & 1u)) idx += p.shadow_alt;
          const float4 s0 = p.shadow_rays[3 * (size_t)idx], s1 = p.shadow_rays[3 * (size_t)idx + 1];
          slot = __float_as_uint(s1.w);
          contribution = xyz(p.shadow_rays[3 * (size_t)idx + 2]);
          if (ALPHA && p.media) slot = idx;
          tr.any = !(ALPHA && p.media);
          tr.start(bvh, stack, xyz(s0), xyz(s1), 0.0f, s0.w);
          busy = true;
          shadow_lane = true;
        }
      }
      if (!__any(busy)) {
        if (work_c.exhausted && work_s.exhausted) break;
        continue;
      }
    }
    if (COUNT) {
      const uint32_t k = work_c.exhausted && (uint32_t)__popcll(__ballot(busy && tr.active() && tr.any)) * 2u >= (uint32_t)__popcll(__ballot(busy && tr.active())) ? 1u : 0u;
      if ((threadIdx.x & 63u) == 0) round_slots[k] += 64;
      if (busy && tr.active()) busy_rounds[k]++;
      const uint32_t n0 = cnt[k].inner_slots, t0 = cnt[k].tri_slots;
      TraverseCounters c;
      c.clear();
      tr.round(bvh, stack, p.inner_min_lanes, c);
      cnt[tr.any ? 1 : 0].nodes += c.nodes;
      cnt[tr.any ? 1 : 0].tris += c.tris;
      cnt[k].inner_slots = n0 + c.inner_slots;
      cnt[k].tri_slots = t0 + c.tri_slots;
      for (int i = 0; i < 8; i++) cnt[0].st[i] += c.st[i];
    } else {
      tr.round(bvh, stack, p.inner_min_lanes, cnt[0]);
    }
  }
  if (COUNT) {
    for (uint32_t k = 0; k < 2; k++) {
      wave_add(&p.counters[CNT_NODES + k], cnt[k].nodes);
      wave_add(&p.counters[CNT_TRIS + k], cnt[k].tris);
      wave_add(&p.counters[CNT_INNER_SLOTS + k], cnt[k].inner_slots);
      wave_add(&p.counters[CNT_TRI_SLOTS + k], cnt[k].tri_slots);
      wave_add(&p.counters[CNT_ROUND_SLOTS + k], round_slots[k]);
      wave_add(&p.counters[CNT_BUSY_ROUNDS + k], busy_rounds[k]);
    }
    for (int i = 0; i < 8; i++) wave_add(&p.counters[CNT_LANE_STATES + i], cnt[0].st[i]);
  }
}

template <bool COUNT, bool ALPHA>
__global__ void __launch_bounds__(STHIP_BLOCK) k_trace_deep(FrameParams p) {
  const uint32_t count = *p.deep_count;
  const uint32_t tid = blockIdx.x * STHIP_BLOCK + threadIdx.x, threads = gridDim.x * STHIP_BLOCK;
  uint32_t* column = p.bvh.spill + (size_t)tid * p.bvh.stack_depth;
  float4* target = flag(p, STHIP_eDeferShadowRays) ? p.shadow_sum : p.radiance;
  TraverseCounters cnt[2];
  cnt[0].clear();
  cnt[1].clear();
  for (uint32_t e = tid; e < count; e += threads) {
    const float4* rec = p.deep_rays + 4 * (size_t)e;
    const float4 r0 = rec[0], r1 = rec[1], r2 = rec[2];
    const uint32_t bits = __float_as_uint(rec[3].x);
    const bool any = (bits & 2u) != 0;
    RayHit h;
    if (any)
      traverse<TRAV_ANY, COUNT, 1, ALPHA>(p.bvh, xyz(r0), xyz(r1), r0.w, r1.w, column, h, cnt[1]);
    else
      traverse<TRAV_CLOSEST, COUNT, 1, ALPHA>(p.bvh, xyz(r0), xyz(r1), r0.w, r1.w, column, h, cnt[0]);
    finish_ray<ALPHA>(p, target, __float_as_uint(r2.w), (bits & 1u) != 0, any, h, xyz(r2));
  }
  if (COUNT) {
    for (uint32_t k = 0; k < 2; k++) {
      if (cnt[k].nodes) atomicAdd(&p.counters[CNT_NODES + k], (unsigned long long)cnt[k].nodes);
      if (cnt[k].tris) atomicAdd(&p.counters[CNT_TRIS + k], (unsigned long long)cnt[k].tris);
    }
  }
  if (count == 0) return;
  __syncthreads();
  if (threadIdx.x == 0 && atomicAdd(p.deep_count + 1, 1u) == gridDim.x - 1u) {
    p.deep_count[0] = 0u;
    p.deep_count[1] = 0u;
  }
}

template <bool COUNT, bool ALPHA>
__global__ void __launch_bounds__(STHIP_BLOCK, PRIMARY_BLOCKS) k_trace_primary(FrameParams p) {
  extern __shared__ uint32_t lds_stack[];
  const uint32_t wave_in_block = threadIdx.x >> 6, lane = threadIdx.x & 63u;
  uint32_t* stack = lds_stack + wave_in_block * p.bvh.stack_depth;
  float* world_save = reinterpret_cast<float*>(lds_stack + (STHIP_BLOCK / 64) * p.bvh.stack_depth) + threadIdx.x;
  const uint32_t packets = (p.path_count + 63u) >> 6;
  TraverseCounters cnt;
  cnt.clear();
  for (uint32_t packet = blockIdx.x * (blockDim.x >> 6) + wave_in_block; packet < packets; packet += gridDim.x * (blockDim.x >> 6)) {
    const uint32_t slot = packet * 64u + lane;
    bool live = slot < p.path_count && p.meta[slot] < 0xFFFFFFFEu;
    f3 o = F3s(0.0f), d = F3(0.0f, 0.0f, 1.0f);
    if (live) {
      o = xyz(p.ray_o[slot]);
      d = xyz(p.ray_d[slot]);
    }
    RayHit hit;
    hit.t = __builtin_inff();
    hit.b1 = hit.b2 = 0.0f;
    hit.ip = 0xFFFFFFFFu;
    hit.leaf = 0xFFFFFFFFu;
    if (!__any(live)) {
      if (slot < p.path_count) p.hit[slot] = make_float4(hit.t, 0, 0, __uint_as_float(hit.ip));
      continue;
    }
    RaySpace sp;
    setup_space(sp, o, d, p.bvh.scene_cx, p.bvh.scene_cy, p.bvh.scene_cz, p.bvh.scene_radius);
    {
      const float w[13] = {sp.idir.x, sp.idir.y, sp.idir.z, sp.noodL.x, sp.noodL.y, sp.noodL.z, sp.noodH.x, sp.noodH.y, sp.noodH.z, sp.Sx, sp.Sy, sp.Sz, __int_as_float(sp.k)};
      for (int k = 0; k < 13; k++) world_save[k * STHIP_BLOCK] = w[k];
    }
    uint32_t id_bits = 0;
    uint32_t top = 0;
    uint32_t ref = p.bvh.root_ref;
    const char* nbase = reinterpret_cast<const char*>(p.bvh.nodes);
    const char* tbase = reinterpret_cast<const char*>(p.bvh.tris);
    while (ref != TRAV_DONE) {
      ref = (uint32_t)__builtin_amdgcn_readfirstlane((int)ref);
      if (!(ref & BVH_LEAF_BIT)) {
        const size_t nb = (size_t)ref * BVH_NODE_BYTES;
        const float4 n0 = uniform_load4(nbase, nb), n1 = uniform_load4(nbase, nb + 16), nz = uniform_load4(nbase, nb + 32);
        const uint2 cr = make_uint2((__float_as_uint(n0.x) & 0xFFu) | ((__float_as_uint(n0.y) & 0xFFu) << 8) | ((__float_as_uint(n0.z) & 0xFFu) << 16) | (__float_as_uint(n0.w) << 24),
                                    (__float_as_uint(n1.x) & 0xFFu) | ((__float_as_uint(n1.y) & 0xFFu) << 8) | ((__float_as_uint(n1.z) & 0xFFu) << 16) | (__float_as_uint(n1.w) << 24));
        if (COUNT && lane == 0) {
          cnt.nodes++;
          cnt.inner_slots += 64;
        }
        const float tbest = hit.t;
        const float a0x = fmaf(n0.x, sp.idir.x, sp.noodL.x), b0x = fmaf(n0.y, sp.idir.x, sp.noodH.x);
        const float a0y = fmaf(n0.z, sp.idir.y, sp.noodL.y), b0y = fmaf(n0.w, sp.idir.y, sp.noodH.y);
        const float a0z = fmaf(nz.x, sp.idir.z, sp.noodL.z), b0z = fmaf(nz.y, sp.idir.z, sp.noodH.z);
        const float a1x = fmaf(n1.x, sp.idir.x, sp.noodL.x), b1x = fmaf(n1.y, sp.idir.x, sp.noodH.x);
        const float a1y = fmaf(n1.z, sp.idir.y, sp.noodL.y), b1y = fmaf(n1.w, sp.idir.y, sp.noodH.y);
        const float a1z = fmaf(nz.z, sp.idir.z, sp.noodL.z), b1z = fmaf(nz.w, sp.idir.z, sp.noodH.z);
        const float tn0 = fmaxf(fmaxf(fminf(a0x, b0x), fminf(a0y, b0y)), fmaxf(fminf(a0z, b0z), 0.0f));
        const float tf0 = fminf(fminf(fmaxf(a0x, b0x), fmaxf(a0y, b0y)), fminf(fmaxf(a0z, b0z), tbest));
        const float tn1 = fmaxf(fmaxf(fminf(a1x, b1x), fminf(a1y, b1y)), fmaxf(fminf(a1z, b1z), 0.0f));
        const float tf1 = fminf(fminf(fmaxf(a1x, b1x), fmaxf(a1y, b1y)), fminf(fmaxf(a1z, b1z), tbest));
        const bool h0 = live & (tn0 <= tf0);
        const bool h1 = live & (tn1 <= tf1);
        const unsigned long long m0 = __ballot(h0), m1 = __ballot(h1);
        if (m0 | m1) {
          const unsigned long long prefer1 = __ballot(h1 & (!h0 | (tn1 < tn0)));
          const bool first1 = m1 && (!m0 || __popcll(prefer1) * 2 > __popcll(m0 | m1));
          ref = first1 ? cr.y : cr.x;
          if (m0 && m1) {
            stack[top] = first1 ? cr.x : cr.y;
            top++;
          }
        } else {
          ref = top ? stack[--top] : TRAV_DONE;
        }
        continue;
      }
      if (ref == TRAV_EXIT_INSTANCE) {
        sp.o = o;
        sp.idir = F3(world_save[0], world_save[STHIP_BLOCK], world_save[2 * STHIP_BLOCK]);
        sp.noodL = F3(world_save[3 * STHIP_BLOCK], world_save[4 * STHIP_BLOCK], world_save[5 * STHIP_BLOCK]);
        sp.noodH = F3(world_save[6 * STHIP_BLOCK], world_save[7 * STHIP_BLOCK], world_save[8 * STHIP_BLOCK]);
        sp.Sx = world_save[9 * STHIP_BLOCK];
        sp.Sy = world_save[10 * STHIP_BLOCK];
        sp.Sz = world_save[11 * STHIP_BLOCK];
        sp.k = __float_as_int(world_save[12 * STHIP_BLOCK]);
        id_bits = 0;
        ref = top ? stack[--top] : TRAV_DONE;
        continue;
      }
      if (ref & BVH_INST_BIT) {
        const TlasEntry* e = p.bvh.entries + (ref & 0xFFFFu);
        const float4* ev = reinterpret_cast<const float4*>(e);
        const uint4 info = *reinterpret_cast<const uint4*>(ev + 3);
        if (info.z != TLAS_ENTRY_IDENTITY) {
          const float4 r0 = ev[0], r1 = ev[1], r2 = ev[2];
          const float4 sph = ev[4];
          const float m[12] = {r0.x, r0.y, r0.z, r0.w, r1.x, r1.y, r1.z, r1.w, r2.x, r2.y, r2.z, r2.w};
          if (info.z == TLAS_ENTRY_SPHERE) {
            if (COUNT && lane == 0) {
              cnt.tris++;
              cnt.tri_slots += 64;
            }
            float t;
            if (live && sphere_test(obj_point(m, o), obj_vector(m, d), sph.w, 0.0f, __builtin_inff(), t)) {
              const uint32_t ip = info.y | 0xFFFF0000u;
              if (t < hit.t || (t == hit.t && hit.ip != 0xFFFFFFFFu && hit_key(ip) < hit_key(hit.ip))) {
                hit.t = t;
                hit.b1 = hit.b2 = 0.0f;
                hit.ip = ip;
              }
            }
            ref = top ? stack[--top] : TRAV_DONE;
            continue;
          }
          setup_space(sp, obj_point(m, o), obj_vector(m, d), sph.x, sph.y, sph.z, sph.w);
          id_bits = info.y;
          stack[top] = TRAV_EXIT_INSTANCE;
          top++;
        }
        ref = info.x;
        continue;
      }
      const uint32_t first = (ref & 0x3FFFFFFFu) >> 2;
      const uint32_t count = (ref & 3u) + 1u;
      for (uint32_t i = 0; i < count; i++) {
        const size_t tb = (size_t)((first + i) * 48u);
        const float4 v0 = uniform_load4(tbase, tb), v1 = uniform_load4(tbase, tb + 16), v2 = uniform_load4(tbase, tb + 32);
        if (COUNT && lane == 0) {
          cnt.tris++;
          cnt.tri_slots += 64;
        }
        float t, b1, b2;
        bool candidate = live & tri_test(sp, xyz(v0), xyz(v1), xyz(v2), 0.0f, __builtin_inff(), t, b1, b2);
        if (ALPHA && candidate) {
          const uint32_t mask = p.bvh.alpha_test ? p.bvh.inst_alpha[(__float_as_uint(v0.w) | id_bits) & 0xFFFFu] : BVH_NO_ALPHA;
          if (mask != BVH_NO_ALPHA) {
            const float2* q = p.bvh.tri_uv + (size_t)(first + i) * 3u;
            const float2 u0 = q[0], u1 = q[1], u2 = q[2];
            const float u = u0.x + (u1.x - u0.x) * b1 + (u2.x - u0.x) * b2;
            float v = u0.y + (u1.y - u0.y) * b1 + (u2.y - u0.y) * b2;
            if (p.bvh.flip_uvs) v = 1 - v;
            candidate = sample_image1(p.bvh, mask, u, v) >= 0.75f;
          }
        }
        const uint32_t ip = __float_as_uint(v0.w) | id_bits;
        const bool closer = candidate & ((t < hit.t) | ((t == hit.t) & (hit.ip != 0xFFFFFFFFu) & (hit_key(ip) < hit_key(hit.ip))));
        hit.t = closer ? t : hit.t;
        hit.b1 = closer ? b1 : hit.b1;
        hit.b2 = closer ? b2 : hit.b2;
        hit.ip = closer ? ip : hit.ip;
        hit.leaf = closer ? first + i : hit.leaf;
      }
      ref = top ? stack[--top] : TRAV_DONE;
    }
    if (slot < p.path_count) {
      p.hit[slot] = make_float4(hit.t, hit.b1, hit.b2, __uint_as_float(hit.ip));
      p.hit_leaf[slot] = hit.leaf;
    }
  }
  if (COUNT) {
    wave_add(&p.counters[CNT_NODES], cnt.nodes);
    wave_add(&p.counters[CNT_TRIS], cnt.tris);
    wave_add(&p.counters[CNT_NODES_PRIMARY], cnt.nodes);
    wave_add(&p.counters[CNT_TRIS_PRIMARY], cnt.tris);
    wave_add(&p.counters[CNT_INNER_SLOTS], cnt.inner_slots);
    wave_add(&p.counters[CNT_TRI_SLOTS], cnt.tri_slots);
// ... 2508 lines not shown
    uint32_t px, py;
    slot_to_pixel(p, slot, px, py);
    const f3 direction = xyz(p.ray_d[slot]);
    Environment env;
    env.load(p.scene, p.pc.gEnvironmentMaterialAddress);
    float4 dbg = p.debug[slot];
    if (p.debug_mode == STHIP_DEBUG_ENVIRONMENT_SAMPLE_TEST) {
      Rng rng;
      rng.x = px;
      rng.y = py;
      rng.seed = p.seed + slot / p.paths_per_seed;
      rng.counter = 0u;
      for (uint32_t i = 0; i < 8; i++) {
        float pdf;
        f3 dir;
        const float r0 = rng.next_float(), r1 = rng.next_float();
        (void)env.sample(p.scene, r0, r1, dir, pdf, flag(p, STHIP_eSampleEnvironmentMapDirectly));
        const float v = 1024 * det_powf(fmaxf(0.0f, dot3(dir, direction)), 1024.0f);
        dbg.x = dbg.x + v;
        dbg.y = dbg.y + v;
        dbg.z = dbg.z + v;
      }
    } else {
      const float pdf = env.eval_pdf(p.scene, direction, flag(p, STHIP_eSampleEnvironmentMapDirectly));
      dbg.x = dbg.y = dbg.z = pdf;
    }
    p.debug[slot] = dbg;
  }
}
#endif

#ifndef STHIP_TEMPLATE_INSTANCES_ONLY
inline __global__ void __launch_bounds__(STHIP_BLOCK) k_fill_tri_shade(const BvhTri* tris, uint32_t n, const uint8_t* is_tri, const sthip_PackedVertexData* vertices, uint32_t vertex_count, const uint8_t* indices,
                                                                uint64_t indices_bytes, BvhTriShade* out, BvhTriUv* out_uv) {
  for (uint32_t i = blockIdx.x * STHIP_BLOCK + threadIdx.x; i < n; i += gridDim.x * STHIP_BLOCK) {
    BvhTriShade r;
    memset(&r, 0, sizeof(r));
    if (!is_tri || is_tri[i]) {
      const BvhTri t = tris[i];
      const uint32_t stride = (t.src_vertex >> 31) ? 4u : 2u, first = t.src_vertex & 0x7FFFFFFFu;
      uint32_t idx[3] = {0, 0, 0};
      if ((uint64_t)t.src_indices + 3u * stride <= indices_bytes)
        for (int k = 0; k < 3; k++) {
          const uint8_t* q = indices + (size_t)t.src_indices + (size_t)k * stride;
          idx[k] = stride == 2u ? ((uint32_t)q[0] | (uint32_t)q[1] << 8) : ((uint32_t)q[0] | (uint32_t)q[1] << 8 | (uint32_t)q[2] << 16 | (uint32_t)q[3] << 24);
          idx[k] += first;
          if (idx[k] >= vertex_count) idx[k] = 0;
        }
      const sthip_PackedVertexData a = vertices[idx[0]], b = vertices[idx[1]], c = vertices[idx[2]];
      for (int k = 0; k < 3; k++) {
        r.n0[k] = a.normal[k];
        r.n1[k] = b.normal[k];
        r.n2[k] = c.normal[k];
      }
      r.v0 = a.v;
      r.v1 = b.v;
      r.v2 = c.v;
      r.u[0] = a.u;
      r.u[1] = b.u;
      r.u[2] = c.u;
    }
    out[i] = r;
    if (out_uv) {
      BvhTriUv q;
      q.uv[0][0] = r.u[0];
      q.uv[0][1] = r.v0;
      q.uv[1][0] = r.u[1];
      q.uv[1][1] = r.v1;
      q.uv[2][0] = r.u[2];
      q.uv[2][1] = r.v2;
      out_uv[i] = q;
    }
  }
// ... 34 lines not shown
```

stratum_amd/csrc/traverse.h:

```cpp
#pragma once

#include "bvh.h"
#include "device_math.h"
#include "media.h"

struct DeviceBvh {
  const float4* nodes;
  const float4* tris;
  const TlasEntry* entries;
  uint32_t root_ref;
  uint32_t top_is_world_blas;
  uint32_t stack_depth;
  float scene_cx, scene_cy, scene_cz, scene_radius;
  const float2* tri_uv;
  const uint32_t* inst_alpha;
  const struct DeviceImage1* images1;
  const float* image1_texels;
  uint32_t alpha_test;
  uint32_t flip_uvs;
  const DeviceVolume* volumes;
  const float4* top_nodes;
  const TlasEntry* top_entries;
  uint32_t top_root_ref;
  uint32_t top_count;
  uint32_t lds_levels;
  uint32_t* spill;
  const uint4* wide_nodes;
  const TlasEntry* wide_entries;
  uint32_t wide_root_ref;
  uint32_t wide_stack_depth;
  const uint4* wide8_nodes;
  const TlasEntry* wide8_entries;
  uint32_t wide8_root;
  uint32_t wide8_stack_depth;
  uint32_t wide8_tri_min;
};
struct DeviceImage1 {
  uint32_t offset, w, h, pad;
};
DEV float sample_image1(const DeviceBvh& bvh, uint32_t index, float u, float v) {
  const DeviceImage1 im = bvh.images1[index];
  const float x = u * (float)im.w - 0.5f, y = v * (float)im.h - 0.5f;
  const float x0 = floorf(x), y0 = floorf(y);
  const float fx = x - x0, fy = y - y0;
  const int w = (int)im.w, h = (int)im.h;
  const int ix = (int)x0, iy = (int)y0;
  const int xa = ((ix % w) + w) % w, xb = (((ix + 1) % w) + w) % w, ya = ((iy % h) + h) % h, yb = (((iy + 1) % h) + h) % h;
  const float* t = bvh.image1_texels + im.offset;
  const float a = lerp1(t[(size_t)ya * w + xa], t[(size_t)ya * w + xb], fx), b = lerp1(t[(size_t)yb * w + xa], t[(size_t)yb * w + xb], fx);
  return lerp1(a, b, fy);
}

typedef float lds_f4v __attribute__((ext_vector_type(4)));
typedef __attribute__((address_space(3))) lds_f4v LdsFloat4;
DEV float4 lds_load4(const LdsFloat4* p) {
  const lds_f4v v = *p;
  return make_float4(v.x, v.y, v.z, v.w);
}

DEV uint32_t packed_ref(float4 q) {
  return __builtin_amdgcn_perm(__float_as_uint(q.y), __float_as_uint(q.x), 0x0c0c0400u) | __builtin_amdgcn_perm(__float_as_uint(q.w), __float_as_uint(q.z), 0x04000c0cu);
}

struct RayHit {
  float t, b1, b2;
  uint32_t ip;
  uint32_t leaf;
};

struct TraverseCounters {
  uint32_t nodes, tris;
  uint32_t inner_slots, tri_slots;
  uint32_t st[8];
  DEV void clear() {
    nodes = tris = inner_slots = tri_slots = 0;
    for (int i = 0; i < 8; i++) st[i] = 0;
  }
};
DEV bool first_active_lane() { return (threadIdx.x & 63u) == (uint32_t)(__ffsll((long long)__ballot(1)) - 1); }

struct RaySpace {
  f3 o;
  f3 idir;
  f3 noodL, noodH;
  float Sx, Sy, Sz;
  int k;
};

DEV float safe_rcp_dir(float d) {
  const float eps = 1e-30f;
  const float dd = fabsf(d) < eps ? copysignf(eps, d) : d;
  return __builtin_amdgcn_rcpf(dd);
}

DEV void setup_space(RaySpace& s, f3 o, f3 d, float cx, float cy, float cz, float radius) {
  s.o = o;
  s.idir = F3(safe_rcp_dir(d.x), safe_rcp_dir(d.y), safe_rcp_dir(d.z));
  const float P = 4e-6f * (fabsf(o.x - cx) + fabsf(o.y - cy) + fabsf(o.z - cz) + radius);
  const float Px = P + 3e-7f * fabsf(o.x), Py = P + 3e-7f * fabsf(o.y), Pz = P + 3e-7f * fabsf(o.z);
  s.noodL = F3(-(o.x + Px) * s.idir.x, -(o.y + Py) * s.idir.y, -(o.z + Pz) * s.idir.z);
  s.noodH = F3(-(o.x - Px) * s.idir.x, -(o.y - Py) * s.idir.y, -(o.z - Pz) * s.idir.z);
  int kz = 0;
  float m = fabsf(d.x);
  if (fabsf(d.y) > m) {
    kz = 1;
    m = fabsf(d.y);
  }
  if (fabsf(d.z) > m) kz = 2;
  int kx = kz + 1;
  if (kx == 3) kx = 0;
  int ky = kx + 1;
  if (ky == 3) ky = 0;
  const float dz = comp3(d, kz);
  if (dz < 0.0f) {
    const int t = kx;
    kx = ky;
    ky = t;
  }
  s.k = kx | (ky << 2) | (kz << 4);
  s.Sx = comp3(d, kx) / dz;
  s.Sy = comp3(d, ky) / dz;
  s.Sz = 1.0f / dz;
}

DEV f3 obj_point(const float* m, f3 p) {
  return F3(fmaf(m[2], p.z, fmaf(m[1], p.y, m[0] * p.x)) + m[3], fmaf(m[6], p.z, fmaf(m[5], p.y, m[4] * p.x)) + m[7],
            fmaf(m[10], p.z, fmaf(m[9], p.y, m[8] * p.x)) + m[11]);
}
DEV f3 obj_vector(const float* m, f3 p) {
  return F3(fmaf(m[2], p.z, fmaf(m[1], p.y, m[0] * p.x)), fmaf(m[6], p.z, fmaf(m[5], p.y, m[4] * p.x)), fmaf(m[10], p.z, fmaf(m[9], p.y, m[8] * p.x)));
}

DEV bool sphere_test(f3 o, f3 d, float r, float tmin, float tmax, float& t) {
  const float a = dot3(d, d);
  const float b = dot3(o, d);
  const f3 l = F3(a * o.x - d.x * b, a * o.y - d.y * b, a * o.z - d.z * b);
  float det = (a * r) * (a * r) - dot3(l, l);
  if (det < 0) return false;
  const float inv_a = 1 / a;
  det = sqrtf(det * inv_a) * inv_a;
  const float e = (-b) * inv_a;
  const float t0 = e - det, t1 = e + det;
  if (!(t0 < t1)) return false;
  const float tt = t0 > tmin ? t0 : t1;
  if (!(tt > tmin && tt < tmax)) return false;
  t = tt;
  return true;
}

DEV uint32_t hit_key(uint32_t ip) { return (ip << 16) | (ip >> 16); }

DEV bool tri_test(const RaySpace& s, f3 p0, f3 p1, f3 p2, float tmin, float tmax, float& t, float& b1, float& b2) {
  const f3 A = p0 - s.o, B = p1 - s.o, C = p2 - s.o;
  const int kx = s.k & 3, ky = (s.k >> 2) & 3, kz = s.k >> 4;
  const float Akz = comp3(A, kz), Bkz = comp3(B, kz), Ckz = comp3(C, kz);
  const float Ax = fmaf(-s.Sx, Akz, comp3(A, kx)), Ay = fmaf(-s.Sy, Akz, comp3(A, ky));
  const float Bx = fmaf(-s.Sx, Bkz, comp3(B, kx)), By = fmaf(-s.Sy, Bkz, comp3(B, ky));
  const float Cx = fmaf(-s.Sx, Ckz, comp3(C, kx)), Cy = fmaf(-s.Sy, Ckz, comp3(C, ky));
  const float U = Cx * By - Cy * Bx;
  const float V = Ax * Cy - Ay * Cx;
  const float W = Bx * Ay - By * Ax;
  const bool edges_disagree = ((U < 0.0f) | (V < 0.0f) | (W < 0.0f)) & ((U > 0.0f) | (V > 0.0f) | (W > 0.0f));
  const float det = U + V + W;
  const float Az = s.Sz * Akz, Bz = s.Sz * Bkz, Cz = s.Sz * Ckz;
  const float T = fmaf(W, Cz, fmaf(V, Bz, U * Az));
  const float rcp = 1.0f / det;
  const float tt = T * rcp;
  t = tt;
  b1 = V * rcp;
  b2 = W * rcp;
  return !edges_disagree & (det != 0.0f) & (tt > tmin) & (tt < tmax);
}

#define TRAV_DONE 0xFFFFFFFFu
#define TRAV_EXIT_INSTANCE 0xFFFFFFFEu
#define TRAV_CANARY 0xFFFFFFFDu

#define TRAV_CLOSEST 0
#define TRAV_ANY 1
#define TRAV_MIXED 2
#ifndef STHIP_ENTRY_BATCH
#define STHIP_ENTRY_BATCH 12u
#endif
template <int MODE, bool COUNT, uint32_t STRIDE, bool ALPHA = false, bool TOP = false, bool BOUNDED = false, bool SAVE_WORLD = false, uint32_t ENTRY_BATCH = 1, bool WIDE = false>
struct Traversal {
  const LdsFloat4* top_lds;
  uint32_t limit;
  DEV bool overflowed(const uint32_t* stack) const { return BOUNDED && stack[limit] != TRAV_CANARY; }
  bool any;
  DEV bool is_any() const { return MODE == TRAV_ANY || (MODE == TRAV_MIXED && any); }
  f3 o, d;
  float tmin, tmax;
  RaySpace sp;
  f3 w_idir, w_noodL, w_noodH;
  float w_Sx, w_Sy, w_Sz;
  int w_k;
  RayHit hit;
  uint32_t ref;
  uint32_t top;
  uint32_t id_bits;

  DEV void orient_space() {
    if (!WIDE) return;
    const float lx = sp.noodL.x, ly = sp.noodL.y, lz = sp.noodL.z;
    const bool nx = sp.idir.x < 0.0f, ny = sp.idir.y < 0.0f, nz = sp.idir.z < 0.0f;
    sp.noodL.x = nx ? sp.noodH.x : lx;
    sp.noodH.x = nx ? lx : sp.noodH.x;
    sp.noodL.y = ny ? sp.noodH.y : ly;
    sp.noodH.y = ny ? ly : sp.noodH.y;
    sp.noodL.z = nz ? sp.noodH.z : lz;
    sp.noodH.z = nz ? lz : sp.noodH.z;
  }
  DEV bool active() const { return ref != TRAV_DONE; }
  DEV void reset() { ref = TRAV_DONE; }
  static DEV bool is_tri_leaf(uint32_t r) { return (r & (BVH_LEAF_BIT | BVH_INST_BIT)) == BVH_LEAF_BIT; }

  DEV void start(const DeviceBvh& bvh, uint32_t* stack, f3 ro, f3 rd, float t0, float t1) {
    o = ro;
    d = rd;
    tmin = t0;
    tmax = t1;
    hit.t = t1;
    hit.b1 = hit.b2 = 0.0f;
    hit.ip = 0xFFFFFFFFu;
    hit.leaf = 0xFFFFFFFFu;
    stack[0] = TRAV_DONE;
    top = STRIDE;
    if (BOUNDED) stack[limit] = TRAV_CANARY;
    id_bits = 0;
    ref = bvh.root_ref;
    setup_space(sp, ro, rd, bvh.scene_cx, bvh.scene_cy, bvh.scene_cz, bvh.scene_radius);
    orient_space();
    if (SAVE_WORLD) {
      w_idir = sp.idir;
      w_noodL = sp.noodL;
      w_noodH = sp.noodH;
      w_Sx = sp.Sx;
      w_Sy = sp.Sy;
      w_Sz = sp.Sz;
      w_k = sp.k;
    }
  }

  DEV void pop(const uint32_t* stack) {
    top -= STRIDE;
    ref = stack[top];
  }

  DEV void inner_loop(const DeviceBvh& bvh, uint32_t* stack, uint32_t min_lanes, TraverseCounters& cnt) {
    const char* base = reinterpret_cast<const char*>(bvh.nodes);
    const float tbest = hit.t;
    if (WIDE) {
      wide_loop(bvh, stack, min_lanes, cnt);
      return;
    }
    for (;;) {
      if (!(ref & BVH_LEAF_BIT)) {
      float4 n0, n1, nz;
      if (TOP && (ref & BVH_TOP_BIT)) {
        const LdsFloat4* n = top_lds + (uint32_t)((ref & ~BVH_TOP_BIT) * 3u);
        n0 = lds_load4(n);
        n1 = lds_load4(n + 1);
        nz = lds_load4(n + 2);
      } else {
        uint32_t offset;
        if (BVH_NODE_BYTES == 48u) {
// ... 20 lines not shown
      const float a0z = fmaf(nz.x, sp.idir.z, sp.noodL.z), b0z = fmaf(nz.y, sp.idir.z, sp.noodH.z);
      const float a1x = fmaf(n1.x, sp.idir.x, sp.noodL.x), b1x = fmaf(n1.y, sp.idir.x, sp.noodH.x);
      const float a1y = fmaf(n1.z, sp.idir.y, sp.noodL.y), b1y = fmaf(n1.w, sp.idir.y, sp.noodH.y);
      const float a1z = fmaf(nz.z, sp.idir.z, sp.noodL.z), b1z = fmaf(nz.w, sp.idir.z, sp.noodH.z);
      const float tn0 = fmaxf(fmaxf(fminf(a0x, b0x), fminf(a0y, b0y)), fmaxf(fminf(a0z, b0z), tmin));
      const float tf0 = fminf(fminf(fmaxf(a0x, b0x), fmaxf(a0y, b0y)), fmaxf(a0z, b0z));
      const float tn1 = fmaxf(fmaxf(fminf(a1x, b1x), fminf(a1y, b1y)), fmaxf(fminf(a1z, b1z), tmin));
      const float tf1 = fminf(fminf(fmaxf(a1x, b1x), fmaxf(a1y, b1y)), fmaxf(a1z, b1z));
      const bool h0 = (tn0 <= tf0) & (tn0 <= tbest);
      const bool h1 = (tn1 <= tf1) & (tn1 <= tbest);
      const bool first1 = h1 & (!h0 | (tn1 < tn0));
      slot[STRIDE] = first1 ? cr.x : cr.y;
      ref = (h0 || h1) ? (first1 ? cr.y : cr.x) : popped;
      const uint32_t next_top = (h0 && h1) ? top + STRIDE : ((h0 || h1) ? top : top - STRIDE);
      top = BOUNDED ? min(next_top, limit) : next_top;
      }
      if ((uint32_t)__popcll(__ballot(!(ref & BVH_LEAF_BIT))) < min_lanes) break;
    }
  }

  DEV void wide_loop(const DeviceBvh& bvh, uint32_t* stack, uint32_t min_lanes, TraverseCounters& cnt) {
    const char* base = reinterpret_cast<const char*>(bvh.wide_nodes);
    const float tbest = hit.t;
    const bool nx = sp.idir.x < 0.0f, ny = sp.idir.y < 0.0f, nz = sp.idir.z < 0.0f;
    const float cnx = sp.noodL.x, cfx = sp.noodH.x, cny = sp.noodL.y, cfy = sp.noodH.y, cnz = sp.noodL.z, cfz = sp.noodH.z;
    for (;;) {
      if (COUNT) {
        const unsigned long long here = __ballot(true), walking = __ballot(!(ref & BVH_LEAF_BIT)), leaf = __ballot(is_tri_leaf(ref));
        if (first_active_lane()) {
          cnt.st[0] += (uint32_t)__popcll(walking);
          cnt.st[1] += (uint32_t)__popcll(leaf);
          cnt.st[2] += (uint32_t)__popcll(here & ~walking & ~leaf);
          cnt.st[3] += 64u - (uint32_t)__popcll(here);
        }
      }
      if (!(ref & BVH_LEAF_BIT)) {
        const uint4* n = reinterpret_cast<const uint4*>(base + (ref << 6));
        const uint4 q0 = n[0], q1 = n[1], q2 = n[2];
        uint4 q3 = n[3];
        const uint32_t popped = stack[top - STRIDE];
        asm volatile("" : "+v"(q3.x), "+v"(q3.y), "+v"(q3.z), "+v"(q3.w));
        if (COUNT) {
          cnt.nodes++;
          if (first_active_lane()) cnt.inner_slots += 64;
        }
        const float ax = __builtin_amdgcn_ldexpf(sp.idir.x, (int)(q0.w << 24) >> 24);
        const float ay = __builtin_amdgcn_ldexpf(sp.idir.y, (int)(q0.w << 16) >> 24);
        const float az = __builtin_amdgcn_ldexpf(sp.idir.z, (int)(q0.w << 8) >> 24);
        const float ox = __uint_as_float(q0.x), oy = __uint_as_float(q0.y), oz = __uint_as_float(q0.z);
        const float enx = fmaf(ox, sp.idir.x, cnx), efx = fmaf(ox, sp.idir.x, cfx);
        const float eny = fmaf(oy, sp.idir.y, cny), efy = fmaf(oy, sp.idir.y, cfy);
        const float enz = fmaf(oz, sp.idir.z, cnz), efz = fmaf(oz, sp.idir.z, cfz);
        const uint32_t qnx = nx ? q1.y : q1.x, qfx = nx ? q1.x : q1.y;
        const uint32_t qny = ny ? q1.w : q1.z, qfy = ny ? q1.z : q1.w;
        const uint32_t qnz = nz ? q2.y : q2.x, qfz = nz ? q2.x : q2.y;
        uint32_t key[4];
#pragma unroll
        for (int c = 0; c < 4; c++) {
          const float tnx = fmaf((float)((qnx >> (8 * c)) & 0xFFu), ax, enx), tfx = fmaf((float)((qfx >> (8 * c)) & 0xFFu), ax, efx);
          const float tny = fmaf((float)((qny >> (8 * c)) & 0xFFu), ay, eny), tfy = fmaf((float)((qfy >> (8 * c)) & 0xFFu), ay, efy);
          const float tnz = fmaf((float)((qnz >> (8 * c)) & 0xFFu), az, enz), tfz = fmaf((float)((qfz >> (8 * c)) & 0xFFu), az, efz);
          const float tn = fmaxf(fmaxf(tnx, tny), fmaxf(tnz, tmin));
          const float tf = fminf(fminf(tfx, tfy), tfz);
          const bool h = (tn <= tf) & (tn <= tbest);
          key[c] = h ? ((__float_as_uint(tn) & 0x7FFFFFF8u) | (4u + (uint32_t)c)) : 0u;
        }
        uint32_t k0 = max(key[0], key[1]), k1 = min(key[0], key[1]), k2 = max(key[2], key[3]), k3 = min(key[2], key[3]);
        uint32_t t0 = max(k0, k2), t2 = min(k0, k2), t1 = max(k1, k3), t3 = min(k1, k3);
        k0 = t0;
        k1 = max(t1, t2);
        k2 = min(t1, t2);
        k3 = t3;
        auto child_ref = [&](uint32_t k) {
          uint32_t m0, m1, r;
          asm("v_bfe_i32 %0, %3, 0, 1\n\tv_bfe_i32 %1, %3, 1, 1\n\tv_bfi_b32 %2, %0, %5, %4\n\tv_bfi_b32 %0, %0, %7, %6\n\tv_bfi_b32 %2, %1, %0, %2"
              : "=&v"(m0), "=&v"(m1), "=&v"(r)
              : "v"(k), "v"(q3.x), "v"(q3.y), "v"(q3.z), "v"(q3.w));
          return r;
        };
        const uint32_t r0 = child_ref(k0), r1 = child_ref(k1), r2 = child_ref(k2), r3 = child_ref(k3);
        stack[top] = r0;
        stack[top + STRIDE] = r1;
        stack[top + 2u * STRIDE] = r2;
        const bool h1 = k0 != 0u, h2 = k1 != 0u, h3 = k2 != 0u, h4 = k3 != 0u;
        ref = h4 ? r3 : (h3 ? r2 : (h2 ? r1 : (h1 ? r0 : popped)));
        const uint32_t next_top = top - STRIDE + ((h1 ? STRIDE : 0u) + (h2 ? STRIDE : 0u) + (h3 ? STRIDE : 0u) + (h4 ? STRIDE : 0u));
        top = BOUNDED ? min(next_top, limit) : next_top;
      }
      if ((uint32_t)__popcll(__ballot(!(ref & BVH_LEAF_BIT))) < min_lanes) break;
    }
  }

  DEV void leaf_step(const DeviceBvh& bvh, uint32_t* stack, TraverseCounters& cnt) {
    const bool entries_due = ENTRY_BATCH > 1 ? !__any(ref < TRAV_EXIT_INSTANCE && !(ref & BVH_INST_BIT)) : true;
    if (COUNT) {
      const unsigned long long tri = __ballot(is_tri_leaf(ref));
      if (first_active_lane()) {
        cnt.st[4] += 64;
        cnt.st[5] += (uint32_t)__popcll(tri);
        cnt.st[6] += (uint32_t)__popcll(__ballot(true) & ~tri);
      }
    }
    if (special_step(bvh, stack, cnt, entries_due)) return;
    triangles_step(bvh, stack, cnt);
  }

  DEV bool special_step(const DeviceBvh& bvh, uint32_t* stack, TraverseCounters& cnt, bool entries_due) {
    if (ref >= TRAV_EXIT_INSTANCE) {
      if (ref == TRAV_EXIT_INSTANCE) {
        if (SAVE_WORLD) {
          sp.o = o;
          sp.idir = w_idir;
          sp.noodL = w_noodL;
          sp.noodH = w_noodH;
          sp.Sx = w_Sx;
          sp.Sy = w_Sy;
          sp.Sz = w_Sz;
          sp.k = w_k;
        } else {
          setup_space(sp, o, d, bvh.scene_cx, bvh.scene_cy, bvh.scene_cz, bvh.scene_radius);
          orient_space();
        }
        id_bits = 0;
        pop(stack);
      }
      return true;
    }
    if (ref & BVH_INST_BIT) {
      if (ENTRY_BATCH > 1) {
        const uint32_t entering = (uint32_t)__popcll(__ballot(true));
        if (entering < ENTRY_BATCH && !entries_due) return true;
      }
      const TlasEntry* e = bvh.entries + (ref & 0xFFFFu);
      const float4* ev = reinterpret_cast<const float4*>(e);
      const uint4 info = *reinterpret_cast<const uint4*>(ev + 3);
      if (info.z != TLAS_ENTRY_IDENTITY) {
        const float4 r0 = ev[0], r1 = ev[1], r2 = ev[2];
        const float4 sph = ev[4];
        const float m[12] = {r0.x, r0.y, r0.z, r0.w, r1.x, r1.y, r1.z, r1.w, r2.x, r2.y, r2.z, r2.w};
        if (info.z == TLAS_ENTRY_SPHERE) {
          if (COUNT) {
            cnt.tris++;
            if (first_active_lane()) cnt.tri_slots += 64;
          }
          float t;
          if (sphere_test(obj_point(m, o), obj_vector(m, d), sph.w, tmin, tmax, t)) {
            if (is_any()) {
              hit.ip = 0;
              ref = TRAV_DONE;
              return true;
            }
            const uint32_t ip = info.y | 0xFFFF0000u;
            if (t < hit.t || (t == hit.t && hit.ip != 0xFFFFFFFFu && hit_key(ip) < hit_key(hit.ip))) {
              hit.t = t;
              hit.b1 = hit.b2 = 0.0f;
              hit.ip = ip;
            }
          }
          pop(stack);
          return true;
        }
        if (ALPHA && info.z == TLAS_ENTRY_VOLUME) {
          if (COUNT) {
            cnt.tris++;
            if (first_active_lane()) cnt.tri_slots += 64;
// ... 5 lines not shown
              ref = TRAV_DONE;
              return true;
            }
            const uint32_t ip = info.y | 0xFFFF0000u;
            if (t < hit.t || (t == hit.t && hit.ip != 0xFFFFFFFFu && hit_key(ip) < hit_key(hit.ip))) {
              hit.t = t;
              hit.b1 = hit.b2 = 0.0f;
              hit.ip = ip;
            }
          }
          pop(stack);
          return true;
        }
        setup_space(sp, obj_point(m, o), obj_vector(m, d), sph.x, sph.y, sph.z, sph.w);
        orient_space();
        id_bits = info.y;
        stack[top] = TRAV_EXIT_INSTANCE;
        top = BOUNDED ? min(top + STRIDE, limit) : top + STRIDE;
      }
      ref = info.x;
      return true;
    }
    return false;
  }

  DEV bool one_triangle(const DeviceBvh& bvh, uint32_t index, TraverseCounters& cnt) {
    const float4* tv = reinterpret_cast<const float4*>(reinterpret_cast<const char*>(bvh.tris) + (size_t)(index * 48u));
    const float4 v0 = tv[0], v1 = tv[1], v2 = tv[2];
    if (COUNT) {
      cnt.tris++;
      if (first_active_lane()) cnt.tri_slots += 64;
    }
    float t, b1, b2;
    bool candidate = tri_test(sp, xyz(v0), xyz(v1), xyz(v2), tmin, tmax, t, b1, b2);
    if (ALPHA && candidate) {
      const uint32_t mask = bvh.alpha_test ? bvh.inst_alpha[(__float_as_uint(v0.w) | id_bits) & 0xFFFFu] : BVH_NO_ALPHA;
      if (mask != BVH_NO_ALPHA) {
        const float2* q = bvh.tri_uv + (size_t)index * 3u;
        const float2 u0 = q[0], u1 = q[1], u2 = q[2];
        const float u = u0.x + (u1.x - u0.x) * b1 + (u2.x - u0.x) * b2;
        float v = u0.y + (u1.y - u0.y) * b1 + (u2.y - u0.y) * b2;
        if (bvh.flip_uvs) v = 1 - v;
        candidate = sample_image1(bvh, mask, u, v) >= 0.75f;
      }
    }
    const bool any_lane = is_any();
    const uint32_t ip = __float_as_uint(v0.w) | id_bits;
    const bool closer = candidate & !any_lane & ((t < hit.t) | ((t == hit.t) & (hit.ip != 0xFFFFFFFFu) & (hit_key(ip) < hit_key(hit.ip))));
    hit.t = closer ? t : hit.t;
    hit.b1 = closer ? b1 : hit.b1;
    hit.b2 = closer ? b2 : hit.b2;
    hit.ip = closer ? ip : hit.ip;
    hit.leaf = closer ? index : hit.leaf;
    return candidate & any_lane;
  }

  DEV void triangles_step(const DeviceBvh& bvh, uint32_t* stack, TraverseCounters& cnt) {
    const uint32_t first = (ref & 0x3FFFFFFFu) >> 2;
    const uint32_t count = (ref & 3u) + 1u;
    bool occluded = false;
    for (uint32_t i = 0; i < count; i++) occluded |= one_triangle(bvh, first + i, cnt);
    const uint32_t popped = stack[top - STRIDE];
    hit.ip = occluded ? 0u : hit.ip;
    ref = occluded ? TRAV_DONE : popped;
    top = occluded ? top : top - STRIDE;
  }

  DEV void round(const DeviceBvh& bvh, uint32_t* stack, uint32_t min_lanes, TraverseCounters& cnt) {
    if (active()) inner_loop(bvh, stack, min_lanes, cnt);
    if (active() && (ref & BVH_LEAF_BIT)) leaf_step(bvh, stack, cnt);
  }
};

#define W8_DONE 0xFFFFFFFFu
#define W8_EXIT 0xFFFFFFFEu
#define W8_CANARY 0xFFFFFFFDu
#ifndef STHIP_WIDE8_STRIDE
#define STHIP_WIDE8_STRIDE 80u
#endif
template <bool COUNT, uint32_t STRIDE, bool ALPHA, bool BOUNDED, uint32_t ENTRY_BATCH, bool SAVE_WORLD = false>
struct Traversal8 {
  uint32_t limit;
  bool any;
  DEV bool is_any() const { return any; }
  f3 o, d;
  float tmin, tmax;
  RaySpace sp;
  f3 w_idir, w_noodL, w_noodH;
  float w_Sx, w_Sy, w_Sz;
  int w_k;
  RayHit hit;
  uint32_t gx, gy, tx, ty;
  uint32_t top;
  uint32_t id_bits;
  uint32_t tri_min;

  static DEV uint2* column(uint32_t* stack) { return reinterpret_cast<uint2*>(stack); }
  DEV bool overflowed(const uint32_t* stack) const { return BOUNDED && reinterpret_cast<const uint2*>(stack)[limit].x != W8_CANARY; }
  DEV bool walking() const { return (gy > 0x00FFFFFFu) & (ty == 0u); }
  DEV bool active() const { return (ty != 0u) | (gy > 0x00FFFFFFu) | (gx != W8_DONE); }
  DEV void reset() {
    gx = W8_DONE;
    gy = ty = tx = 0u;
  }
  DEV void orient_space() {
    const float lx = sp.noodL.x, ly = sp.noodL.y, lz = sp.noodL.z;
    const bool nx = sp.idir.x < 0.0f, ny = sp.idir.y < 0.0f, nz = sp.idir.z < 0.0f;
    sp.noodL.x = nx ? sp.noodH.x : lx;
    sp.noodH.x = nx ? lx : sp.noodH.x;
    sp.noodL.y = ny ? sp.noodH.y : ly;
    sp.noodH.y = ny ? ly : sp.noodH.y;
    sp.noodL.z = nz ? sp.noodH.z : lz;
    sp.noodH.z = nz ? lz : sp.noodH.z;
  }
  DEV void start(const DeviceBvh& bvh, uint32_t* stack, f3 ro, f3 rd, float t0, float t1) {
    o = ro;
    d = rd;
    tmin = t0;
    tmax = t1;
    hit.t = t1;
    hit.b1 = hit.b2 = 0.0f;
    hit.ip = 0xFFFFFFFFu;
    hit.leaf = 0xFFFFFFFFu;
    uint2* st = column(stack);
    st[0] = make_uint2(W8_DONE, 0u);
    top = STRIDE;
    if (BOUNDED) st[limit] = make_uint2(W8_CANARY, 0u);
    id_bits = 0;
    gx = bvh.root_ref;
    gy = bvh.root_ref == BVH_INVALID_REF ? 0u : 0x80000000u;
    tx = ty = 0u;
    setup_space(sp, ro, rd, bvh.scene_cx, bvh.scene_cy, bvh.scene_cz, bvh.scene_radius);
    orient_space();
    if (SAVE_WORLD) {
      w_idir = sp.idir;
      w_noodL = sp.noodL;
      w_noodH = sp.noodH;
      w_Sx = sp.Sx;
      w_Sy = sp.Sy;
      w_Sz = sp.Sz;
      w_k = sp.k;
    }
  }
  DEV bool push(uint2* st, uint32_t x, uint32_t y, bool keep) {
    const bool lost = BOUNDED && top == limit;
    st[top] = make_uint2(x, y);
    top = keep && !lost ? top + STRIDE : top;
    return lost;
  }
  DEV void give_up() {
    gx = W8_DONE;
    gy = ty = 0u;
  }
  DEV void take(uint2 P) {
    gx = P.x;
    gy = P.y;
    tx = P.x;
    ty = P.y <= 0x00FFFFFFu ? P.y : 0u;
  }
  DEV void finish_occluded() {
    hit.ip = 0u;
    gx = W8_DONE;
    gy = ty = 0u;
  }

  DEV void node_loop(const DeviceBvh& bvh, uint32_t* stack, uint32_t min_lanes, TraverseCounters& cnt) {
// ... 53 lines not shown
        uint32_t hitmask = 0u;
#pragma unroll
        for (int c = 0; c < 8; c++) {
          const int w = c >> 2, b = 8 * (c & 3);
          const float tnx = fmaf((float)((qnx[w] >> b) & 0xFFu), ax, enx), tfx = fmaf((float)((qfx[w] >> b) & 0xFFu), ax, efx);
          const float tny = fmaf((float)((qny[w] >> b) & 0xFFu), ay, eny), tfy = fmaf((float)((qfy[w] >> b) & 0xFFu), ay, efy);
          const float tnz = fmaf((float)((qnz[w] >> b) & 0xFFu), az, enz), tfz = fmaf((float)((qfz[w] >> b) & 0xFFu), az, efz);
          const float tn = fmaxf(fmaxf(tnx, tny), fmaxf(tnz, tmin));
          const float tf = fminf(fminf(tfx, tfy), tfz);
          const bool h = (tn <= tf) & (tn <= tbest);
          const uint32_t add = ((bits4[w] >> b) & 0xFFu) << ((at4[w] >> b) & 0xFFu);
          hitmask |= h ? add : 0u;
        }
        const bool nohit = hitmask == 0u;
        gx = nohit ? P.x : n1.x;
        gy = nohit ? P.y : ((hitmask & 0xFF000000u) | (n0.w >> 24));
        tx = nohit ? P.x : n1.y;
        ty = nohit ? (P.y <= 0x00FFFFFFu ? P.y : 0u) : (hitmask & 0x00FFFFFFu);
        top = nohit ? ntop - STRIDE : ntop;
        if (lost) give_up();
      }
      if ((uint32_t)__popcll(__ballot(walking())) < min_lanes) break;
    }
  }

  DEV bool one_triangle(const DeviceBvh& bvh, uint32_t index, TraverseCounters& cnt) {
    const float4* tv = reinterpret_cast<const float4*>(reinterpret_cast<const char*>(bvh.tris) + (size_t)(index * 48u));
    const float4 v0 = tv[0], v1 = tv[1], v2 = tv[2];
    if (COUNT) {
      cnt.tris++;
      if (first_active_lane()) cnt.tri_slots += 64;
    }
    float t, b1, b2;
    bool candidate = tri_test(sp, xyz(v0), xyz(v1), xyz(v2), tmin, tmax, t, b1, b2);
    if (ALPHA && candidate) {
      const uint32_t mask = bvh.alpha_test ? bvh.inst_alpha[(__float_as_uint(v0.w) | id_bits) & 0xFFFFu] : BVH_NO_ALPHA;
      if (mask != BVH_NO_ALPHA) {
        const float2* q = bvh.tri_uv + (size_t)index * 3u;
        const float2 u0 = q[0], u1 = q[1], u2 = q[2];
        const float u = u0.x + (u1.x - u0.x) * b1 + (u2.x - u0.x) * b2;
        float v = u0.y + (u1.y - u0.y) * b1 + (u2.y - u0.y) * b2;
        if (bvh.flip_uvs) v = 1 - v;
        candidate = sample_image1(bvh, mask, u, v) >= 0.75f;
      }
    }
    const uint32_t ip = __float_as_uint(v0.w) | id_bits;
    const bool closer = candidate & !any & ((t < hit.t) | ((t == hit.t) & (hit.ip != 0xFFFFFFFFu) & (hit_key(ip) < hit_key(hit.ip))));
    hit.t = closer ? t : hit.t;
    hit.b1 = closer ? b1 : hit.b1;
    hit.b2 = closer ? b2 : hit.b2;
    hit.ip = closer ? ip : hit.ip;
    hit.leaf = closer ? index : hit.leaf;
    return candidate & any;
  }
  DEV bool fold_entry_hit(bool found, float t, uint32_t instance) {
    if (!found) return false;
    if (any) return true;
    const uint32_t ip = instance | 0xFFFF0000u;
    if (t < hit.t || (t == hit.t && hit.ip != 0xFFFFFFFFu && hit_key(ip) < hit_key(hit.ip))) {
      hit.t = t;
      hit.b1 = hit.b2 = 0.0f;
      hit.ip = ip;
    }
    return false;
  }

  DEV void leaf_step(const DeviceBvh& bvh, uint32_t* stack, TraverseCounters& cnt) {
// ... 77 lines not shown
        finish_occluded();
      } else if (ty == 0u && gy <= 0x00FFFFFFu) {
        top -= STRIDE;
        take(st[top]);
      }
    }
    for (;;) {
      const bool has = ty != 0u && !(tx & WIDE8_ENTRY_BIT);
      if (has) {
        const uint32_t bit = (uint32_t)__ffs((int)ty) - 1u;
        ty &= ty - 1u;
        const uint2 P = st[top - STRIDE];
        const bool occluded = one_triangle(bvh, tx + bit, cnt);
        const bool pop = !occluded & (ty == 0u) & (gy <= 0x00FFFFFFu);
        hit.ip = occluded ? 0u : hit.ip;
        gx = occluded ? W8_DONE : (pop ? P.x : gx);
        gy = occluded ? 0u : (pop ? P.y : gy);
        tx = pop ? P.x : tx;
        ty = occluded ? 0u : (pop ? (P.y <= 0x00FFFFFFu ? P.y : 0u) : ty);
        top = pop ? top - STRIDE : top;
      }
      if ((uint32_t)__popcll(__ballot(ty != 0u && !(tx & WIDE8_ENTRY_BIT))) < tri_min) break;
    }
  }

  DEV void round(const DeviceBvh& bvh, uint32_t* stack, uint32_t min_lanes, TraverseCounters& cnt) {
    if (active()) node_loop(bvh, stack, min_lanes, cnt);
    if (active() && !walking()) leaf_step(bvh, stack, cnt);
  }
};

template <int MODE, bool COUNT, uint32_t STRIDE, bool ALPHA = false>
DEV bool traverse(const DeviceBvh& bvh, f3 o, f3 d, float tmin, float tmax, uint32_t* stack, RayHit& hit, TraverseCounters& cnt) {
  Traversal<MODE, COUNT, STRIDE, ALPHA> tr;
  tr.any = MODE == TRAV_ANY;
  tr.start(bvh, stack, o, d, tmin, tmax);
  while (tr.active()) tr.round(bvh, stack, 1, cnt);
  hit = tr.hit;
  return hit.ip != 0xFFFFFFFFu;
}

#define QUEUE_SEGMENTS 8u
#define QCTL_STRIDE 32u
#define QCTL_SIZE 0u
#define QCTL_KEPT 1u
#define QCTL_ANSWERED 2u
#define QCTL_HEAD 16u
DEV unsigned long long* queue_ctl(unsigned long long* qctl, uint32_t kind, uint32_t depth, uint32_t seg) {
  return qctl + (size_t)((kind * 64u + depth) * QUEUE_SEGMENTS + seg) * QCTL_STRIDE;
}

#ifndef WORK_CHUNK
#define WORK_CHUNK 64u
#endif
struct WaveWork {
  uint32_t next, end;
  uint32_t cur, dry;
  bool exhausted;
  DEV void init() {
    next = end = 0;
    cur = blockIdx.x % QUEUE_SEGMENTS;
    dry = 0;
    exhausted = false;
  }
  DEV uint32_t take(bool want, unsigned long long* ctl, uint32_t stride, uint32_t n) {
    const unsigned long long mask = __ballot(want);
    if (!mask) return 0xFFFFFFFFu;
// ... 41 lines not shown
```

stratum_amd/wire.py:

```python
import ctypes as C

import numpy as np

InstanceData = np.dtype([("packed", "<u4", (4,))])
PackedVertexData = np.dtype([("position", "<f4", (3,)), ("u", "<f4"), ("normal", "<f4", (3,)), ("v", "<f4")])
TransformData = np.dtype([("m", "<f4", (3, 4))])
ProjectionData = np.dtype(
    [
        ("scale", "<f4", (2,)),
        ("offset", "<f4", (2,)),
        ("near_plane", "<f4"),
        ("far_plane", "<f4"),
        ("sensor_area", "<f4"),
        ("vertical_fov", "<f4"),
    ]
)
ViewData = np.dtype([("projection", ProjectionData), ("image_min", "<i4", (2,)), ("image_max", "<i4", (2,))])
VisibilityInfo = np.dtype([("instance_primitive_index", "<u4"), ("packed_normal", "<u4")])
DepthInfo = np.dtype([("z", "<f4"), ("prev_z", "<f4"), ("dz_dxy", "<f4", (2,))])
ShadingData = np.dtype(
    [
        ("position", "<f4", (3,)),
        ("flags", "<u4"),
        ("packed_geometry_normal", "<u4"),
# ... 171 lines not shown
        ("rays_total", C.c_uint64),
        ("rays_path", C.c_uint64),
        ("rays_shadow", C.c_uint64),
        ("nodes_visited", C.c_uint64),
        ("tris_tested", C.c_uint64),
        ("nodes_visited_shadow", C.c_uint64),
        ("tris_tested_shadow", C.c_uint64),
        ("ms_trace", C.c_float),
        ("ms_shade", C.c_float),
        ("ms_total", C.c_float),
        ("launches_trace", C.c_uint32),
        ("bvh_node_bytes", C.c_uint32),
        ("bvh_tri_bytes", C.c_uint32),
        ("bvh_nodes", C.c_uint64),
        ("bvh_tris", C.c_uint64),
        ("bvh_build_ms", C.c_float),
        ("bvh_build_gpu_ms", C.c_float),
        ("inner_slots", C.c_uint64 * 2),
        ("tri_slots", C.c_uint64 * 2),
        ("round_slots", C.c_uint64 * 2),
        ("busy_rounds", C.c_uint64 * 2),
        ("rays_primary_packets", C.c_uint64),
        ("nodes_visited_primary", C.c_uint64),
        ("tris_tested_primary", C.c_uint64),
        ("ms_trace_primary", C.c_float),
        ("launches_primary", C.c_uint32),
        ("lane_states", C.c_uint64 * 8),
        ("rays_answered", C.c_uint64),
        ("paths_per_seed", C.c_uint32),
        ("seeds_in_flight", C.c_uint32),
        ("max_paths_in_flight", C.c_uint64),
        ("batch_halvings", C.c_uint32),
        ("full_rebuilds", C.c_uint32),
    ]


def ptr(a):
    if a is None:
        return None
    assert a.flags["C_CONTIGUOUS"]
    return a.ctypes.data_as(C.c_void_p)


def default_push_constants(width, height, light_count, view_count=1):
    pc = BDPTPushConstants()
    pc.gOutputExtent[0], pc.gOutputExtent[1] = width, height
    pc.gViewCount = view_count
    pc.gLightCount = light_count
    pc.gLightDistributionPDF = 0
    pc.gLightDistributionCDF = 0
    pc.gEnvironmentMaterialAddress = 0xFFFFFFFF
    pc.gEnvironmentSampleProbability = 0.5
    pc.gRandomSeed = 0
    pc.gMinPathVertices = 4
    pc.gMaxPathVertices = 8
    pc.gMaxDiffuseVertices = 2
    pc.gMaxNullCollisions = 64
    pc.gLightPresampleTileSize = 1024
    pc.gLightPresampleTileCount = 128
    pc.gLightPathCount = width * height
    pc.gReservoirM = 16
    pc.gReservoirMaxM = 64
    pc.gReservoirSpatialM = 4
    pc.gHashGridBucketCount = 200000
    pc.gHashGridMinBucketRadius = 0.1
    pc.gHashGridBucketPixelRadius = 6
# ... 65 lines not shown
```

Before: 3433 Mray/s.

## Flatten instanced BLAS triangles into the top-level BVH with per-triangle inverse transforms

Adds an optional host-SAH build path that merges separate instances (within an error/conditioning bound and a triangle budget) into the merged world BVH. Flattened triangles keep object-space vertices, are tagged with a flag bit, and carry an instance id. Traversal rebuilds a watertight ray space from the instance inverse transform when the instance changes. This removes instance-entry/exit steps and the two-level traversal overhead. In exchange it adds per-triangle branching, extra registers for a second ray space, new kernel variants, and lane-stop counters.

Measured after the change: 3660 Mray/s, median of 6. 1.07x the previous value.

```diff
diff --git a/__graft_entry__.py b/__graft_entry__.py
--- a/__graft_entry__.py
+++ b/__graft_entry__.py
@@ -22,7 +22,7 @@
 ]
 
 
-PRODUCT_SOURCES = ("api.hip", "shade_plain.hip", "shade_lt.hip", "shade_media.hip", "shade_media_lt.hip", "shade_media_lt2.hip", "trace_kernels.hip", "lbvh.hip", "lvc.hip", "hashgrid.hip", "wide.hip", "bvh_build.cpp",
+PRODUCT_SOURCES = ("api.hip", "shade_plain.hip", "shade_lt.hip", "shade_media.hip", "shade_media_lt.hip", "shade_media_lt2.hip", "trace_kernels.hip", "trace_flat_kernels.hip", "lbvh.hip", "lvc.hip", "hashgrid.hip", "wide.hip", "bvh_build.cpp",
                    "hdr_writer.cpp")
 
 
diff --git a/include/sthip.h b/include/sthip.h
--- a/include/sthip.h
+++ b/include/sthip.h
@@ -176,6 +176,7 @@
   uint64_t max_paths_in_flight;
   uint32_t batch_halvings;
   uint32_t full_rebuilds;
+  uint64_t lane_stops[4];
 } sthip_stats;
 int sthip_get_stats(sthip_ctx* ctx, sthip_stats* out);
 
diff --git a/stratum_amd/csrc/api.hip b/stratum_amd/csrc/api.hip
--- a/stratum_amd/csrc/api.hip
+++ b/stratum_amd/csrc/api.hip
@@ -199,6 +199,9 @@
   DevBuf<TlasEntry> top_entries;
   bool use_treetop = false;
   bool embed_leaves = false;
+  uint64_t flatten_instances = (uint64_t)1 << 20;
+  bool flatten_mixed = false;
+  int flat_mode = 0;
   int use_wide = 1;
   size_t wide_node_count = 0;
   sthip::DeviceWideScratch* wide_scratch = nullptr;
@@ -298,6 +301,21 @@
   return table[(count ? 1 : 0) | (alpha ? 2 : 0) | (bounded ? 4 : 0)];
 }
 
+#define STHIP_FLAT_TABLE(W, F)                                                                                                                                                                  \
+  {(const void*)&k_trace<false, false, false, false, W, F>, (const void*)&k_trace<true, false, false, false, W, F>, (const void*)&k_trace<false, true, false, false, W, F>, (const void*)&k_trace<true, true, false, false, W, F>, \
+   (const void*)&k_trace<false, false, true, false, W, F>,  (const void*)&k_trace<true, false, true, false, W, F>,  (const void*)&k_trace<false, true, true, false, W, F>,  (const void*)&k_trace<true, true, true, false, W, F>}
+static const void* trace_kernel_flat(int wide, int flat, bool count, bool alpha, bool bounded) {
+  static const void* const table[4][8] = {STHIP_FLAT_TABLE(0, 1), STHIP_FLAT_TABLE(1, 1), STHIP_FLAT_TABLE(1, 2), STHIP_FLAT_TABLE(2, 1)};
+  const int row = wide == 0 ? 0 : (wide == 2 ? 3 : (flat == 2 ? 2 : 1));
+  return table[row][(count ? 1 : 0) | (alpha ? 2 : 0) | (bounded ? 4 : 0)];
+}
+
+static const void* trace_kernel_for(const DeviceBvh& bvh, int flat_mode, bool count, bool alpha, bool top) {
+  const bool bounded = bvh.spill != nullptr;
+  if (flat_mode) return trace_kernel_flat(bvh.wide8_nodes ? 2 : (bvh.wide_nodes ? 1 : 0), flat_mode, count, alpha, bounded);
+  return bvh.wide8_nodes ? trace_kernel_wide8(count, alpha, bounded) : bvh.wide_nodes ? trace_kernel_wide(count, alpha, bounded) : trace_kernel(count, alpha, bounded, top);
+}
+
 #define HIP_TRY(ctx, expr)                                                                            \
   do {                                                                                                \
     hipError_t _e = (expr);                                                                           \
@@ -323,6 +341,7 @@
     ctx->stats.busy_rounds[k] = c[CNT_BUSY_ROUNDS + k];
   }
   for (int k = 0; k < 8; k++) ctx->stats.lane_states[k] = c[CNT_LANE_STATES + k];
+  for (int k = 0; k < 4; k++) ctx->stats.lane_stops[k] = c[CNT_LANE_STOPS + k];
   ctx->stats.rays_answered = c[CNT_RAYS_ANSWERED];
   ctx->stats.nodes_visited_primary = c[CNT_NODES_PRIMARY];
   ctx->stats.tris_tested_primary = c[CNT_TRIS_PRIMARY];
@@ -382,6 +401,9 @@
     for (int k = 0; k < 16; k++) (void)hipFuncSetAttribute(trace_kernel((k & 1) != 0, (k & 2) != 0, (k & 4) != 0, (k & 8) != 0), hipFuncAttributeMaxDynamicSharedMemorySize, lds_max);
     for (int k = 0; k < 8; k++) (void)hipFuncSetAttribute(trace_kernel_wide((k & 1) != 0, (k & 2) != 0, (k & 4) != 0), hipFuncAttributeMaxDynamicSharedMemorySize, lds_max);
     for (int k = 0; k < 8; k++) (void)hipFuncSetAttribute(trace_kernel_wide8((k & 1) != 0, (k & 2) != 0, (k & 4) != 0), hipFuncAttributeMaxDynamicSharedMemorySize, lds_max);
+    for (int k = 0; k < 8; k++)
+      for (int w = 0; w < 3; w++)
+        for (int f = 1; f <= (w == 1 ? 2 : 1); f++) (void)hipFuncSetAttribute(trace_kernel_flat(w, f, (k & 1) != 0, (k & 2) != 0, (k & 4) != 0), hipFuncAttributeMaxDynamicSharedMemorySize, lds_max);
     (void)hipFuncSetAttribute(reinterpret_cast<const void*>(&k_trace_batch<false, false>), hipFuncAttributeMaxDynamicSharedMemorySize, lds_max);
     (void)hipFuncSetAttribute(reinterpret_cast<const void*>(&k_trace_batch<true, false>), hipFuncAttributeMaxDynamicSharedMemorySize, lds_max);
     (void)hipFuncSetAttribute(reinterpret_cast<const void*>(&k_trace_batch<false, true>), hipFuncAttributeMaxDynamicSharedMemorySize, lds_max);
@@ -504,6 +526,10 @@
     ctx->lds_materials = value != 0;
   else if (!strcmp(name, "embed_leaves"))
     ctx->embed_leaves = value != 0;
+  else if (!strcmp(name, "flatten_instances"))
+    ctx->flatten_instances = (uint64_t)std::max<int64_t>(value, 0);
+  else if (!strcmp(name, "flatten_mixed"))
+    ctx->flatten_mixed = value != 0;
   else if (!strcmp(name, "keep_scene")) {
     ctx->keep_scene = value != 0;
     if (!ctx->keep_scene) ctx->kept = KeptScene();
@@ -744,7 +770,7 @@
     };
   }
   const auto t_build0 = std::chrono::steady_clock::now();
-  if (!sthip::build_scene_bvh(*s, built, err, ctx->bvh_builder, device_build ? &target : nullptr, ctx->embed_leaves && STHIP_NODE_STRIDE == 48))
+  if (!sthip::build_scene_bvh(*s, built, err, ctx->bvh_builder, device_build ? &target : nullptr, ctx->embed_leaves && STHIP_NODE_STRIDE == 48, ctx->use_treetop ? 0 : ctx->flatten_instances, ctx->flatten_mixed))
     return fail(ctx, err.find("only triangle") != std::string::npos ? STHIP_ERR_UNSUPPORTED : STHIP_ERR_INVALID_ARGUMENT, "scene: " + err);
 
   if (((size_t)built.dev_nodes + built.nodes.size() + 2 * built.entries.size() + 2) * sizeof(BvhNodeSlot) > 0xFFFFFFFFull || ((size_t)built.dev_tris + built.tris.size()) * sizeof(BvhTri) > 0xFFFFFFFFull)
@@ -1006,6 +1032,8 @@
   ctx->bvh.entries = ctx->entries.p;
   ctx->bvh.root_ref = built.root_ref;
   ctx->bvh.top_is_world_blas = built.top_is_world_blas;
+  ctx->bvh.flat_inv = built.flat_tris ? reinterpret_cast<const float4*>(ctx->inv_xf.p) : nullptr;
+  ctx->flat_mode = built.flat_tris ? (built.top_is_world_blas ? 2 : 1) : 0;
   ctx->bvh.stack_depth = built.stack_depth;
   ctx->bvh.scene_cx = built.scene_center[0];
   ctx->bvh.scene_cy = built.scene_center[1];
@@ -1041,7 +1069,7 @@
         HIP_TRY(ctx, hipMemcpy(is_tri.p, flags.data(), units, hipMemcpyHostToDevice));
       }
       hipLaunchKernelGGL(k_fill_tri_shade, dim3(grid_for_early(ctx, units)), dim3(STHIP_BLOCK), 0, ctx->stream, reinterpret_cast<const BvhTri*>(ctx->bvh.tris), (uint32_t)units, is_tri.p, ctx->vertices.p, s->vertex_count,
-                         ctx->indices.p, (uint64_t)s->indices_bytes, ctx->tri_shade.p, ctx->has_alpha ? ctx->tri_uvs.p : nullptr);
+                         ctx->indices.p, (uint64_t)s->indices_bytes, ctx->tri_shade.p, ctx->has_alpha ? ctx->tri_uvs.p : nullptr, built.flat_tris ? 0x7FFFFFFFu & ~BVH_TRI_FLAT_BIT : 0x7FFFFFFFu);
       HIP_TRY(ctx, hipGetLastError());
       HIP_TRY(ctx, hipStreamSynchronize(ctx->stream));
     }
@@ -1078,11 +1106,7 @@
 static int trace_occupancy(const sthip_ctx* ctx, size_t lds_bytes) {
   int per_cu = 0;
   hipError_t e;
-  e = hipOccupancyMaxActiveBlocksPerMultiprocessor(&per_cu,
-                                                   ctx->bvh.wide8_nodes  ? trace_kernel_wide8(false, false, ctx->bvh.spill != nullptr)
-                                                   : ctx->bvh.wide_nodes ? trace_kernel_wide(false, false, ctx->bvh.spill != nullptr)
-                                                                         : trace_kernel(false, false, ctx->bvh.spill != nullptr, ctx->use_treetop),
-                                                   STHIP_BLOCK, lds_bytes);
+  e = hipOccupancyMaxActiveBlocksPerMultiprocessor(&per_cu, trace_kernel_for(ctx->bvh, ctx->flat_mode, false, false, ctx->use_treetop), STHIP_BLOCK, lds_bytes);
   return e == hipSuccess ? per_cu : 0;
 }
 static uint32_t trace_grid(sthip_ctx* ctx, size_t lds_bytes) {
@@ -1860,10 +1884,7 @@
       return timed(ms_trace, [&]() {
         const bool alpha = p.bvh.alpha_test || ctx->has_volumes;
         void* kargs[3] = {(void*)&p, (void*)&dc, (void*)&ds};
-        (void)hipLaunchKernel(p.bvh.wide8_nodes  ? trace_kernel_wide8(ctx->count_traversal, alpha, p.bvh.spill != nullptr)
-                              : p.bvh.wide_nodes ? trace_kernel_wide(ctx->count_traversal, alpha, p.bvh.spill != nullptr)
-                                                 : trace_kernel(ctx->count_traversal, alpha, p.bvh.spill != nullptr, p.bvh.top_count != 0),
-                              dim3(tgrid), dim3(STHIP_BLOCK), kargs, lds, st);
+        (void)hipLaunchKernel(trace_kernel_for(p.bvh, ctx->flat_mode, ctx->count_traversal, alpha, p.bvh.top_count != 0), dim3(tgrid), dim3(STHIP_BLOCK), kargs, lds, st);
         if (p.bvh.spill) {
           const uint32_t dgrid = (uint32_t)ctx->cu_count * 8u;
           if (alpha) {
@@ -1884,10 +1905,7 @@
           q.qctl = p.qctl + (size_t)64 * QUEUE_SEGMENTS * QCTL_STRIDE;
           const uint32_t none = TRACE_NONE;
           void* qargs[3] = {(void*)&q, (void*)&none, (void*)&ds};
-          (void)hipLaunchKernel(p.bvh.wide8_nodes  ? trace_kernel_wide8(false, alpha, p.bvh.spill != nullptr)
-                                : p.bvh.wide_nodes ? trace_kernel_wide(false, alpha, p.bvh.spill != nullptr)
-                                                   : trace_kernel(false, alpha, p.bvh.spill != nullptr, p.bvh.top_count != 0),
-                                dim3(tgrid), dim3(STHIP_BLOCK), qargs, lds, st);
+          (void)hipLaunchKernel(trace_kernel_for(p.bvh, ctx->flat_mode, false, alpha, p.bvh.top_count != 0), dim3(tgrid), dim3(STHIP_BLOCK), qargs, lds, st);
           if (p.bvh.spill) {
             const uint32_t dgrid = (uint32_t)ctx->cu_count * 8u;
             if (alpha)
@@ -1905,15 +1923,12 @@
       const unsigned pgrid = std::max(1u, std::min((packets + 3) / 4, (uint32_t)ctx->cu_count * 64u));
       const size_t plds = ((size_t)ctx->bvh.stack_depth * (STHIP_BLOCK / 64) + 13 * STHIP_BLOCK) * sizeof(uint32_t);
       return timed(ms_primary, [&]() {
-        if (p.bvh.alpha_test) {
-          if (ctx->count_traversal)
-            hipLaunchKernelGGL((k_trace_primary<true, true>), dim3(pgrid), dim3(STHIP_BLOCK), plds, st, p);
-          else
-            hipLaunchKernelGGL((k_trace_primary<false, true>), dim3(pgrid), dim3(STHIP_BLOCK), plds, st, p);
-        } else if (ctx->count_traversal)
-          hipLaunchKernelGGL((k_trace_primary<true, false>), dim3(pgrid), dim3(STHIP_BLOCK), plds, st, p);
-        else
-          hipLaunchKernelGGL((k_trace_primary<false, false>), dim3(pgrid), dim3(STHIP_BLOCK), plds, st, p);
+        static const void* const primary[3][4] = {
+            {(const void*)&k_trace_primary<false, false, 0>, (const void*)&k_trace_primary<true, false, 0>, (const void*)&k_trace_primary<false, true, 0>, (const void*)&k_trace_primary<true, true, 0>},
+            {(const void*)&k_trace_primary<false, false, 1>, (const void*)&k_trace_primary<true, false, 1>, (const void*)&k_trace_primary<false, true, 1>, (const void*)&k_trace_primary<true, true, 1>},
+            {(const void*)&k_trace_primary<false, false, 2>, (const void*)&k_trace_primary<true, false, 2>, (const void*)&k_trace_primary<false, true, 2>, (const void*)&k_trace_primary<true, true, 2>}};
+        void* pargs[1] = {(void*)&p};
+        (void)hipLaunchKernel(primary[ctx->flat_mode][(ctx->count_traversal ? 1 : 0) | (p.bvh.alpha_test ? 2 : 0)], dim3(pgrid), dim3(STHIP_BLOCK), pargs, plds, st);
       });
     };
     auto run_rounds = [&](bool light, bool shadow_rays, auto&& shade) -> int {
diff --git a/stratum_amd/csrc/bvh.h b/stratum_amd/csrc/bvh.h
--- a/stratum_amd/csrc/bvh.h
+++ b/stratum_amd/csrc/bvh.h
@@ -22,6 +22,7 @@
   float v2[3];
   uint32_t src_vertex;
 };
+#define BVH_TRI_FLAT_BIT 0x40000000u
 struct BvhTriShade {
   float n0[3], v0;
   float n1[3], v1;
diff --git a/stratum_amd/csrc/bvh_build.cpp b/stratum_amd/csrc/bvh_build.cpp
--- a/stratum_amd/csrc/bvh_build.cpp
+++ b/stratum_amd/csrc/bvh_build.cpp
@@ -302,7 +302,38 @@
 
 }
 
-bool build_scene_bvh(const sthip_scene_desc& s, BuiltBvh& out, std::string& err, int builder, DeviceBuildTarget* device, bool embed_leaves) {
+struct FlattenFit {
+  bool ok = false;
+  double e_lin = 0, e_trans = 0, kappa = 0;
+  double pad(double R) const { return 2.0 * (2.0 * e_lin * R + e_trans + 12.0 * ldexp(1.0, -24) * kappa * R); }
+};
+static FlattenFit flatten_fit(const sthip_TransformData& M, const sthip_TransformData& Minv) {
+  FlattenFit f;
+  for (int r = 0; r < 3; r++)
+    for (int c = 0; c < 4; c++)
+      if (!std::isfinite(M.m[r][c]) || !std::isfinite(Minv.m[r][c])) return f;
+  for (int r = 0; r < 3; r++) {
+    double row_e = 0, row_k = 0;
+    for (int c = 0; c < 3; c++) {
+      double e = 0, k = 0;
+      for (int j = 0; j < 3; j++) {
+        e += (double)M.m[r][j] * (double)Minv.m[j][c];
+        k += fabs((double)M.m[r][j]) * fabs((double)Minv.m[j][c]);
+      }
+      row_e += fabs(e - (r == c ? 1.0 : 0.0));
+      row_k += k;
+    }
+    double t = (double)M.m[r][3];
+    for (int j = 0; j < 3; j++) t += (double)M.m[r][j] * (double)Minv.m[j][3];
+    f.e_lin = std::max(f.e_lin, row_e);
+    f.kappa = std::max(f.kappa, row_k);
+    f.e_trans = std::max(f.e_trans, fabs(t));
+  }
+  f.ok = f.kappa <= 8.0 && f.e_lin <= 1e-4;
+  return f;
+}
+
+bool build_scene_bvh(const sthip_scene_desc& s, BuiltBvh& out, std::string& err, int builder, DeviceBuildTarget* device, bool embed_leaves, uint64_t flatten_budget, bool flatten_partial) {
   out = BuiltBvh();
   const bool dev_mode = device != nullptr && builder == BVH_BUILDER_LBVH_GPU;
   const uint32_t DEVICE_MIN_PRIMS = 64;
@@ -408,6 +439,73 @@
       merged.push_back(i);
     else
       separate.push_back(i);
+  }
+
+  out.flattened.assign(s.instance_count, 0);
+  std::vector<double> flat_pad(s.instance_count, 0.0);
+  if (flatten_budget && !dev_mode && builder == BVH_BUILDER_SAH_HOST && !separate.empty()) {
+    bool bit_free = true;
+    for (uint32_t i : merged) bit_free &= view(s.gInstances[i]).first_vertex < BVH_TRI_FLAT_BIT;
+    for (uint32_t i : separate) bit_free &= view(s.gInstances[i]).first_vertex < BVH_TRI_FLAT_BIT;
+    double max_abs = 0, lo[3] = {INFINITY, INFINITY, INFINITY}, hi[3] = {-INFINITY, -INFINITY, -INFINITY};
+    auto grow = [&](const double* w) {
+      for (int a = 0; a < 3; a++) {
+        lo[a] = std::min(lo[a], w[a]);
+        hi[a] = std::max(hi[a], w[a]);
+        max_abs = std::max(max_abs, fabs(w[a]));
+      }
+    };
+    auto grow_instance = [&](uint32_t i) {
+      const InstView in = view(s.gInstances[i]);
+      const sthip_TransformData& M = s.gInstanceTransforms[i];
+      for (uint32_t p = 0; p < in.prim_count; p++) {
+        uint32_t tri[3];
+        load_tri(s, in, p, tri);
+        for (int v = 0; v < 3; v++) {
+          const float* q = s.gVertices[tri[v]].position;
+          double w[3];
+          for (int r = 0; r < 3; r++) w[r] = (double)M.m[r][0] * q[0] + (double)M.m[r][1] * q[1] + (double)M.m[r][2] * q[2] + (double)M.m[r][3];
+          grow(w);
+        }
+      }
+    };
+    if (bit_free) {
+      for (uint32_t i : merged) grow_instance(i);
+      for (uint32_t i : separate) grow_instance(i);
+      for (uint32_t i : spheres) {
+        float r;
+        memcpy(&r, &s.gInstances[i].packed[2], 4);
+        for (int c = 0; c < 2; c++) {
+          double w[3];
+          for (int a = 0; a < 3; a++) w[a] = (double)s.gInstanceTransforms[i].m[a][3] + (c ? fabs(r) : -fabs(r));
+          grow(w);
+        }
+      }
+    }
+    const double diag = lo[0] <= hi[0] ? sqrt((hi[0] - lo[0]) * (hi[0] - lo[0]) + (hi[1] - lo[1]) * (hi[1] - lo[1]) + (hi[2] - lo[2]) * (hi[2] - lo[2])) : 0.0;
+    const double R = max_abs + 4.0 * diag;
+    uint64_t used = 0;
+    std::vector<uint32_t> kept;
+    for (uint32_t i : separate) {
+      const InstView in = view(s.gInstances[i]);
+      const FlattenFit fit = flatten_fit(s.gInstanceTransforms[i], s.gInstanceInverseTransforms[i]);
+      if (bit_free && std::isfinite(R) && in.prim_count && fit.ok && fit.e_trans <= 1e-4 * std::max(R, 1e-30) && used + in.prim_count <= flatten_budget) {
+        used += in.prim_count;
+        out.flattened[i] = 1;
+        flat_pad[i] = fit.pad(R);
+        merged.push_back(i);
+      } else {
+        kept.push_back(i);
+      }
+    }
+    if (!flatten_partial && used && (!kept.empty() || !spheres.empty() || !volumes.empty())) {
+      for (uint32_t i : merged) out.flattened[i] = 0;
+      merged.resize(merged.size() - (separate.size() - kept.size()));
+      used = 0;
+    } else {
+      separate.swap(kept);
+    }
+    out.flat_tris = used;
   }
 
   std::vector<uint32_t> inst_alpha(s.instance_count, BVH_NO_ALPHA);
@@ -562,7 +660,25 @@
       uint32_t tri[3];
       load_tri(s, in, prims[k].second, tri);
       boxes[k].reset();
-      for (int v = 0; v < 3; v++) boxes[k].grow(s.gVertices[tri[v]].position);
+      if (with_instance_bits && out.flattened[prims[k].first]) {
+        const sthip_TransformData& M = s.gInstanceTransforms[prims[k].first];
+        double lo[3] = {INFINITY, INFINITY, INFINITY}, hi[3] = {-INFINITY, -INFINITY, -INFINITY};
+        for (int v = 0; v < 3; v++) {
+          const float* q = s.gVertices[tri[v]].position;
+          for (int r = 0; r < 3; r++) {
+            const double w = (double)M.m[r][0] * q[0] + (double)M.m[r][1] * q[1] + (double)M.m[r][2] * q[2] + (double)M.m[r][3];
+            lo[r] = std::min(lo[r], w);
+            hi[r] = std::max(hi[r], w);
+          }
+        }
+        const double pad = flat_pad[prims[k].first];
+        for (int r = 0; r < 3; r++) {
+          boxes[k].lo[r] = nextafterf((float)(lo[r] - pad), -INFINITY);
+          boxes[k].hi[r] = nextafterf((float)(hi[r] + pad), INFINITY);
+        }
+      } else {
+        for (int v = 0; v < 3; v++) boxes[k].grow(s.gVertices[tri[v]].position);
+      }
       bounds.grow(boxes[k]);
     }
     uint32_t leaf_tris = BVH_MAX_LEAF_TRIS;
@@ -582,7 +698,7 @@
       memcpy(t.v2, s.gVertices[tri[2]].position, 12);
       t.id = (pr.second << 16) | (with_instance_bits ? pr.first : 0u);
       t.src_indices = in.indices_byte_offset + pr.second * 3u * in.stride;
-      t.src_vertex = in.first_vertex | (in.stride == 4u ? 0x80000000u : 0u);
+      t.src_vertex = in.first_vertex | (in.stride == 4u ? 0x80000000u : 0u) | (with_instance_bits && out.flattened[pr.first] ? BVH_TRI_FLAT_BIT : 0u);
     }
     const uint32_t root = flatten(b, 0, out.nodes, [&](uint32_t first, uint32_t count) {
       if (!out.embedded) return BVH_LEAF_BIT | ((tri_base + first) << 2) | (count - 1);
@@ -758,7 +874,11 @@
   out.top.volumes = out.volumes;
   out.top.instance_count = s.instance_count;
   out.top.merged.assign(s.instance_count, 0);
-  for (uint32_t i : merged) out.top.merged[i] = 1;
+  for (uint32_t i : merged) out.top.merged[i] = out.flattened[i] ? 2 : 1;
+  if (out.flat_tris) {
+    out.top.flat_xf.assign(s.gInstanceTransforms, s.gInstanceTransforms + s.instance_count);
+    out.top.flat_inv.assign(s.gInstanceInverseTransforms, s.gInstanceInverseTransforms + s.instance_count);
+  }
   out.top.blas_nodes = out.dev_nodes + (uint32_t)out.nodes.size();
   out.top.blas_depth = blas_depth;
   out.top.obj_box.assign(6 * out.entries.size(), 0.f);
@@ -1467,11 +1587,16 @@
     err = "the instance count changed: upload the scene again";
     return false;
   }
-  for (uint32_t i = 0; i < instance_count; i++)
-    if (st.merged[i] && !(is_identity(xf[i]) && is_identity(inv[i]))) {
+  for (uint32_t i = 0; i < instance_count; i++) {
+    if (st.merged[i] == 2 && !(memcmp(&xf[i], &st.flat_xf[i], sizeof(xf[i])) == 0 && memcmp(&inv[i], &st.flat_inv[i], sizeof(inv[i])) == 0)) {
+      err = "a flattened instance (flatten_instances) moved: upload the scene again";
+      return false;
+    }
+    if (st.merged[i] == 1 && !(is_identity(xf[i]) && is_identity(inv[i]))) {
       err = "an instance of the merged world-space mesh (identity transform at upload) moved: upload the scene again";
       return false;
     }
+  }
   Box scene_box;
   scene_box.reset();
   std::vector<Box> entry_boxes(st.entries.size());
diff --git a/stratum_amd/csrc/bvh_build.h b/stratum_amd/csrc/bvh_build.h
--- a/stratum_amd/csrc/bvh_build.h
+++ b/stratum_amd/csrc/bvh_build.h
@@ -21,6 +21,7 @@
   std::vector<TlasEntry> entries;
   std::vector<float> obj_box;
   std::vector<uint8_t> merged;
+  std::vector<sthip_TransformData> flat_xf, flat_inv;
   std::vector<DeviceVolume> volumes;
   uint32_t instance_count = 0;
   uint32_t blas_nodes = 0;
@@ -51,6 +52,8 @@
   bool embedded = false;
   std::vector<uint32_t> unit_tri;
   TopLevelState top;
+  std::vector<uint8_t> flattened;
+  uint64_t flat_tris = 0;
   std::vector<WideNode> wide_nodes;
   std::vector<TlasEntry> wide_entries;
   uint32_t wide_root_ref = BVH_INVALID_REF;
@@ -95,7 +98,8 @@
 
 enum BvhBuilderKind { BVH_BUILDER_SAH_HOST = 0, BVH_BUILDER_LBVH_GPU = 1 };
 
-bool build_scene_bvh(const sthip_scene_desc& scene, BuiltBvh& out, std::string& err, int builder = BVH_BUILDER_SAH_HOST, DeviceBuildTarget* device = nullptr, bool embed_leaves = false);
+bool build_scene_bvh(const sthip_scene_desc& scene, BuiltBvh& out, std::string& err, int builder = BVH_BUILDER_SAH_HOST, DeviceBuildTarget* device = nullptr, bool embed_leaves = false,
+                     uint64_t flatten_budget = 0, bool flatten_partial = true);
 void build_wide_bvh(BuiltBvh& out);
 
 void build_wide8_bvh(BuiltBvh& out);
diff --git a/stratum_amd/csrc/kernel_instances.h b/stratum_amd/csrc/kernel_instances.h
--- a/stratum_amd/csrc/kernel_instances.h
+++ b/stratum_amd/csrc/kernel_instances.h
@@ -15,15 +15,21 @@
   Y(false, false, false, TOP, WIDE) Y(true, false, false, TOP, WIDE) Y(false, true, false, TOP, WIDE) Y(true, true, false, TOP, WIDE) Y(false, false, true, TOP, WIDE) Y(true, false, true, TOP, WIDE) \
   Y(false, true, true, TOP, WIDE) Y(true, true, true, TOP, WIDE)
 #define STHIP_TRACE_ALL(Y) STHIP_TRACE_ROWS(Y, false, 0) STHIP_TRACE_ROWS(Y, true, 0) STHIP_TRACE_ROWS(Y, false, 1) STHIP_TRACE_ROWS(Y, false, 2)
+#define STHIP_TRACE_FLAT_ROWS(F, WIDE, FLAT) \
+  F(false, false, false, WIDE, FLAT) F(true, false, false, WIDE, FLAT) F(false, true, false, WIDE, FLAT) F(true, true, false, WIDE, FLAT) F(false, false, true, WIDE, FLAT) F(true, false, true, WIDE, FLAT) \
+  F(false, true, true, WIDE, FLAT) F(true, true, true, WIDE, FLAT)
+#define STHIP_TRACE_FLAT_ALL(F) STHIP_TRACE_FLAT_ROWS(F, 0, 1) STHIP_TRACE_FLAT_ROWS(F, 1, 1) STHIP_TRACE_FLAT_ROWS(F, 1, 2) STHIP_TRACE_FLAT_ROWS(F, 2, 1)
 #define STHIP_SHADE_LIGHT(Z) Z(false, true, false) Z(true, true, false) Z(false, true, true) Z(true, true, true)
 
 #define STHIP_SHADE_EXTERN(T, E, L, M, P, D) extern template __global__ void k_shade<T, E, L, M, P, D>(FrameParams, uint32_t);
 #define STHIP_SHADE_DEFINE(T, E, L, M, P, D) template __global__ void k_shade<T, E, L, M, P, D>(FrameParams, uint32_t);
 #define STHIP_TRACE_EXTERN(C, A, B, T, W) extern template __global__ void k_trace<C, A, B, T, W>(FrameParams, uint32_t, uint32_t);
 #define STHIP_TRACE_DEFINE(C, A, B, T, W) template __global__ void k_trace<C, A, B, T, W>(FrameParams, uint32_t, uint32_t);
+#define STHIP_TRACE_FLAT_EXTERN(C, A, B, W, F) extern template __global__ void k_trace<C, A, B, false, W, F>(FrameParams, uint32_t, uint32_t);
+#define STHIP_TRACE_FLAT_DEFINE(C, A, B, W, F) template __global__ void k_trace<C, A, B, false, W, F>(FrameParams, uint32_t, uint32_t);
 #define STHIP_LIGHT_EXTERN(T, E, M) extern template __global__ void k_shade_light<T, E, M>(FrameParams, uint32_t);
 #define STHIP_LIGHT_DEFINE(T, E, M) template __global__ void k_shade_light<T, E, M>(FrameParams, uint32_t);
 
 #define STHIP_DECLARE_KERNEL_INSTANCES \
-  STHIP_SHADE_PLAIN(STHIP_SHADE_EXTERN) STHIP_SHADE_LT(STHIP_SHADE_EXTERN) STHIP_SHADE_MEDIA(STHIP_SHADE_EXTERN) STHIP_SHADE_MEDIA_LT(STHIP_SHADE_EXTERN) STHIP_SHADE_MEDIA_LT2(STHIP_SHADE_EXTERN) STHIP_TRACE_ALL(STHIP_TRACE_EXTERN) \
+  STHIP_SHADE_PLAIN(STHIP_SHADE_EXTERN) STHIP_SHADE_LT(STHIP_SHADE_EXTERN) STHIP_SHADE_MEDIA(STHIP_SHADE_EXTERN) STHIP_SHADE_MEDIA_LT(STHIP_SHADE_EXTERN) STHIP_SHADE_MEDIA_LT2(STHIP_SHADE_EXTERN) STHIP_TRACE_ALL(STHIP_TRACE_EXTERN) STHIP_TRACE_FLAT_ALL(STHIP_TRACE_FLAT_EXTERN) \
       STHIP_SHADE_LIGHT(STHIP_LIGHT_EXTERN)
diff --git a/stratum_amd/csrc/kernels.h b/stratum_amd/csrc/kernels.h
--- a/stratum_amd/csrc/kernels.h
+++ b/stratum_amd/csrc/kernels.h
@@ -22,7 +22,8 @@
   CNT_CROSSINGS = 16,
   CNT_RAYS_ANSWERED = 17,
   CNT_LANE_STATES = 20,
-  CNT_TOTAL = 28
+  CNT_LANE_STOPS = 28,
+  CNT_TOTAL = 32
 };
 
 struct FrameParams {
@@ -317,7 +318,7 @@
 #ifndef STHIP_TRACE_ATTR
 #define STHIP_TRACE_ATTR
 #endif
-template <bool COUNT, bool ALPHA, bool BOUNDED = false, bool TOP = false, int WIDE = 0>
+template <bool COUNT, bool ALPHA, bool BOUNDED = false, bool TOP = false, int WIDE = 0, int FLAT = 0>
 __global__ void __launch_bounds__(STHIP_BLOCK) STHIP_TRACE_ATTR k_trace(FrameParams p, uint32_t depth_closest, uint32_t depth_shadow) {
   extern __shared__ uint32_t lds_stack[];
   float4* top_lds = reinterpret_cast<float4*>(lds_stack + (size_t)p.bvh.lds_levels * STHIP_BLOCK);
@@ -348,8 +349,8 @@
     bvh.entries = p.bvh.wide8_entries;
     bvh.root_ref = p.bvh.wide8_root;
   }
-  typename std::conditional<WIDE == 2, Traversal8<COUNT, STHIP_BLOCK, ALPHA, BOUNDED, STHIP_ENTRY_BATCH>,
-                            Traversal<TRAV_MIXED, COUNT, STHIP_BLOCK, ALPHA, TOP, BOUNDED, true, STHIP_ENTRY_BATCH, WIDE == 1>>::type tr;
+  typename std::conditional<WIDE == 2, Traversal8<COUNT, STHIP_BLOCK, ALPHA, BOUNDED, STHIP_ENTRY_BATCH, false, FLAT != 0>,
+                            Traversal<TRAV_MIXED, COUNT, STHIP_BLOCK, ALPHA, TOP, BOUNDED, FLAT != 2, STHIP_ENTRY_BATCH, WIDE == 1, FLAT>>::type tr;
   if constexpr (WIDE == 2) {
     tr.tri_min = p.bvh.wide8_tri_min;
     if (BOUNDED) tr.limit = (p.bvh.lds_levels - 1u) * STHIP_BLOCK;
@@ -432,6 +433,8 @@
       cnt[k].inner_slots = n0 + c.inner_slots;
       cnt[k].tri_slots = t0 + c.tri_slots;
       for (int i = 0; i < 8; i++) cnt[0].st[i] += c.st[i];
+      for (int i = 0; i < 3; i++) cnt[0].stop[i] += c.stop[i];
+      cnt[0].stop[3] += c.stop[3];
     } else {
       tr.round(bvh, stack, p.inner_min_lanes, cnt[0]);
     }
@@ -446,6 +449,7 @@
       wave_add(&p.counters[CNT_BUSY_ROUNDS + k], busy_rounds[k]);
     }
     for (int i = 0; i < 8; i++) wave_add(&p.counters[CNT_LANE_STATES + i], cnt[0].st[i]);
+    for (int i = 0; i < 4; i++) wave_add(&p.counters[CNT_LANE_STOPS + i], cnt[0].stop[i]);
   }
 }
 
@@ -484,7 +488,7 @@
   }
 }
 
-template <bool COUNT, bool ALPHA>
+template <bool COUNT, bool ALPHA, int FLAT = 0>
 __global__ void __launch_bounds__(STHIP_BLOCK, PRIMARY_BLOCKS) k_trace_primary(FrameParams p) {
   extern __shared__ uint32_t lds_stack[];
   const uint32_t wave_in_block = threadIdx.x >> 6, lane = threadIdx.x & 63u;
@@ -512,7 +516,14 @@
     }
     RaySpace sp;
     setup_space(sp, o, d, p.bvh.scene_cx, p.bvh.scene_cy, p.bvh.scene_cz, p.bvh.scene_radius);
-    {
+    TriSpace tsp;
+    tsp.o = sp.o;
+    tsp.Sx = sp.Sx;
+    tsp.Sy = sp.Sy;
+    tsp.Sz = sp.Sz;
+    tsp.k = sp.k;
+    uint32_t tspace = 0u;
+    if (FLAT != 2) {
       const float w[13] = {sp.idir.x, sp.idir.y, sp.idir.z, sp.noodL.x, sp.noodL.y, sp.noodL.z, sp.noodH.x, sp.noodH.y, sp.noodH.z, sp.Sx, sp.Sy, sp.Sz, __int_as_float(sp.k)};
       for (int k = 0; k < 13; k++) world_save[k * STHIP_BLOCK] = w[k];
     }
@@ -559,7 +570,7 @@
         }
         continue;
       }
-      if (ref == TRAV_EXIT_INSTANCE) {
+      if (FLAT != 2 && ref == TRAV_EXIT_INSTANCE) {
         sp.o = o;
         sp.idir = F3(world_save[0], world_save[STHIP_BLOCK], world_save[2 * STHIP_BLOCK]);
         sp.noodL = F3(world_save[3 * STHIP_BLOCK], world_save[4 * STHIP_BLOCK], world_save[5 * STHIP_BLOCK]);
@@ -572,7 +583,7 @@
         ref = top ? stack[--top] : TRAV_DONE;
         continue;
       }
-      if (ref & BVH_INST_BIT) {
+      if (FLAT != 2 && (ref & BVH_INST_BIT)) {
         const TlasEntry* e = p.bvh.entries + (ref & 0xFFFFu);
         const float4* ev = reinterpret_cast<const float4*>(e);
         const uint4 info = *reinterpret_cast<const uint4*>(ev + 3);
@@ -615,7 +626,26 @@
           cnt.tri_slots += 64;
         }
         float t, b1, b2;
-        bool candidate = live & tri_test(sp, xyz(v0), xyz(v1), xyz(v2), 0.0f, __builtin_inff(), t, b1, b2);
+        bool candidate;
+        if (FLAT) {
+          const bool flat = (FLAT == 2 || p.bvh.flat_inv != nullptr) && (__float_as_uint(v2.w) & BVH_TRI_FLAT_BIT);
+          const uint32_t space = (uint32_t)__builtin_amdgcn_readfirstlane((int)tri_space_of(v0, v2));
+          if ((FLAT == 2 || flat) && space != tspace) {
+            make_tri_space(tsp, p.bvh.flat_inv, space, o, d);
+            tspace = space;
+          }
+          TriSpace use = tsp;
+          if (FLAT != 2 && !flat) {
+            use.o = sp.o;
+            use.Sx = sp.Sx;
+            use.Sy = sp.Sy;
+            use.Sz = sp.Sz;
+            use.k = sp.k;
+          }
+          candidate = live & tri_test(use, xyz(v0), xyz(v1), xyz(v2), 0.0f, __builtin_inff(), t, b1, b2);
+        } else {
+          candidate = live & tri_test(sp, xyz(v0), xyz(v1), xyz(v2), 0.0f, __builtin_inff(), t, b1, b2);
+        }
         if (ALPHA && candidate) {
           const uint32_t mask = p.bvh.alpha_test ? p.bvh.inst_alpha[(__float_as_uint(v0.w) | id_bits) & 0xFFFFu] : BVH_NO_ALPHA;
           if (mask != BVH_NO_ALPHA) {
@@ -3190,13 +3220,13 @@
 
 #ifndef STHIP_TEMPLATE_INSTANCES_ONLY
 inline __global__ void __launch_bounds__(STHIP_BLOCK) k_fill_tri_shade(const BvhTri* tris, uint32_t n, const uint8_t* is_tri, const sthip_PackedVertexData* vertices, uint32_t vertex_count, const uint8_t* indices,
-                                                                uint64_t indices_bytes, BvhTriShade* out, BvhTriUv* out_uv) {
+                                                                uint64_t indices_bytes, BvhTriShade* out, BvhTriUv* out_uv, uint32_t vertex_mask) {
   for (uint32_t i = blockIdx.x * STHIP_BLOCK + threadIdx.x; i < n; i += gridDim.x * STHIP_BLOCK) {
     BvhTriShade r;
     memset(&r, 0, sizeof(r));
     if (!is_tri || is_tri[i]) {
       const BvhTri t = tris[i];
-      const uint32_t stride = (t.src_vertex >> 31) ? 4u : 2u, first = t.src_vertex & 0x7FFFFFFFu;
+      const uint32_t stride = (t.src_vertex >> 31) ? 4u : 2u, first = t.src_vertex & vertex_mask;
       uint32_t idx[3] = {0, 0, 0};
       if ((uint64_t)t.src_indices + 3u * stride <= indices_bytes)
         for (int k = 0; k < 3; k++) {
diff --git a/stratum_amd/csrc/trace_flat_kernels.hip b/stratum_amd/csrc/trace_flat_kernels.hip
--- /dev/null
+++ b/stratum_amd/csrc/trace_flat_kernels.hip
@@ -0,0 +1,10 @@
+#define STHIP_TEMPLATE_INSTANCES_ONLY
+#include <hip/hip_runtime.h>
+#include <stdio.h>
+#include <string.h>
+#include <string>
+#include <vector>
+#include "../../include/sthip.h"
+#include "bvh_build.h"
+#include "kernel_instances.h"
+STHIP_TRACE_FLAT_ALL(STHIP_TRACE_FLAT_DEFINE)
diff --git a/stratum_amd/csrc/traverse.h b/stratum_amd/csrc/traverse.h
--- a/stratum_amd/csrc/traverse.h
+++ b/stratum_amd/csrc/traverse.h
@@ -34,6 +34,7 @@
   uint32_t wide8_root;
   uint32_t wide8_stack_depth;
   uint32_t wide8_tri_min;
+  const float4* flat_inv;
 };
 struct DeviceImage1 {
   uint32_t offset, w, h, pad;
@@ -72,9 +73,11 @@
   uint32_t nodes, tris;
   uint32_t inner_slots, tri_slots;
   uint32_t st[8];
+  uint32_t stop[4];
   DEV void clear() {
     nodes = tris = inner_slots = tri_slots = 0;
     for (int i = 0; i < 8; i++) st[i] = 0;
+    for (int i = 0; i < 4; i++) stop[i] = 0;
   }
 };
 DEV bool first_active_lane() { return (threadIdx.x & 63u) == (uint32_t)(__ffsll((long long)__ballot(1)) - 1); }
@@ -93,13 +96,13 @@
   return __builtin_amdgcn_rcpf(dd);
 }
 
-DEV void setup_space(RaySpace& s, f3 o, f3 d, float cx, float cy, float cz, float radius) {
-  s.o = o;
-  s.idir = F3(safe_rcp_dir(d.x), safe_rcp_dir(d.y), safe_rcp_dir(d.z));
-  const float P = 4e-6f * (fabsf(o.x - cx) + fabsf(o.y - cy) + fabsf(o.z - cz) + radius);
-  const float Px = P + 3e-7f * fabsf(o.x), Py = P + 3e-7f * fabsf(o.y), Pz = P + 3e-7f * fabsf(o.z);
-  s.noodL = F3(-(o.x + Px) * s.idir.x, -(o.y + Py) * s.idir.y, -(o.z + Pz) * s.idir.z);
-  s.noodH = F3(-(o.x - Px) * s.idir.x, -(o.y - Py) * s.idir.y, -(o.z - Pz) * s.idir.z);
+struct TriSpace {
+  f3 o;
+  float Sx, Sy, Sz;
+  int k;
+};
+template <class S>
+DEV void setup_watertight(S& s, f3 d) {
   int kz = 0;
   float m = fabsf(d.x);
   if (fabsf(d.y) > m) {
@@ -123,12 +126,37 @@
   s.Sz = 1.0f / dz;
 }
 
+
+DEV void setup_space(RaySpace& s, f3 o, f3 d, float cx, float cy, float cz, float radius) {
+  s.o = o;
+  s.idir = F3(safe_rcp_dir(d.x), safe_rcp_dir(d.y), safe_rcp_dir(d.z));
+  const float P = 4e-6f * (fabsf(o.x - cx) + fabsf(o.y - cy) + fabsf(o.z - cz) + radius);
+  const float Px = P + 3e-7f * fabsf(o.x), Py = P + 3e-7f * fabsf(o.y), Pz = P + 3e-7f * fabsf(o.z);
+  s.noodL = F3(-(o.x + Px) * s.idir.x, -(o.y + Py) * s.idir.y, -(o.z + Pz) * s.idir.z);
+  s.noodH = F3(-(o.x - Px) * s.idir.x, -(o.y - Py) * s.idir.y, -(o.z - Pz) * s.idir.z);
+  setup_watertight(s, d);
+}
+
 DEV f3 obj_point(const float* m, f3 p) {
   return F3(fmaf(m[2], p.z, fmaf(m[1], p.y, m[0] * p.x)) + m[3], fmaf(m[6], p.z, fmaf(m[5], p.y, m[4] * p.x)) + m[7],
             fmaf(m[10], p.z, fmaf(m[9], p.y, m[8] * p.x)) + m[11]);
 }
 DEV f3 obj_vector(const float* m, f3 p) {
   return F3(fmaf(m[2], p.z, fmaf(m[1], p.y, m[0] * p.x)), fmaf(m[6], p.z, fmaf(m[5], p.y, m[4] * p.x)), fmaf(m[10], p.z, fmaf(m[9], p.y, m[8] * p.x)));
+}
+
+DEV uint32_t tri_space_of(float4 v0, float4 v2) { return (__float_as_uint(v2.w) & BVH_TRI_FLAT_BIT) ? (__float_as_uint(v0.w) & 0xFFFFu) + 1u : 0u; }
+DEV void make_tri_space(TriSpace& ts, const float4* flat_inv, uint32_t space, f3 o, f3 d) {
+  f3 oo = o, dd = d;
+  if (space) {
+    const float4* mv = flat_inv + (size_t)(space - 1u) * 3u;
+    const float4 r0 = mv[0], r1 = mv[1], r2 = mv[2];
+    const float m[12] = {r0.x, r0.y, r0.z, r0.w, r1.x, r1.y, r1.z, r1.w, r2.x, r2.y, r2.z, r2.w};
+    oo = obj_point(m, o);
+    dd = obj_vector(m, d);
+  }
+  ts.o = oo;
+  setup_watertight(ts, dd);
 }
 
 DEV bool sphere_test(f3 o, f3 d, float r, float tmin, float tmax, float& t) {
@@ -150,7 +178,8 @@
 
 DEV uint32_t hit_key(uint32_t ip) { return (ip << 16) | (ip >> 16); }
 
-DEV bool tri_test(const RaySpace& s, f3 p0, f3 p1, f3 p2, float tmin, float tmax, float& t, float& b1, float& b2) {
+template <class S>
+DEV bool tri_test(const S& s, f3 p0, f3 p1, f3 p2, float tmin, float tmax, float& t, float& b1, float& b2) {
   const f3 A = p0 - s.o, B = p1 - s.o, C = p2 - s.o;
   const int kx = s.k & 3, ky = (s.k >> 2) & 3, kz = s.k >> 4;
   const float Akz = comp3(A, kz), Bkz = comp3(B, kz), Ckz = comp3(C, kz);
@@ -182,7 +211,7 @@
 #ifndef STHIP_ENTRY_BATCH
 #define STHIP_ENTRY_BATCH 12u
 #endif
-template <int MODE, bool COUNT, uint32_t STRIDE, bool ALPHA = false, bool TOP = false, bool BOUNDED = false, bool SAVE_WORLD = false, uint32_t ENTRY_BATCH = 1, bool WIDE = false>
+template <int MODE, bool COUNT, uint32_t STRIDE, bool ALPHA = false, bool TOP = false, bool BOUNDED = false, bool SAVE_WORLD = false, uint32_t ENTRY_BATCH = 1, bool WIDE = false, int FLAT = 0>
 struct Traversal {
   const LdsFloat4* top_lds;
   uint32_t limit;
@@ -199,6 +228,8 @@
   uint32_t ref;
   uint32_t top;
   uint32_t id_bits;
+  TriSpace tsp;
+  uint32_t tspace;
 
   DEV void orient_space() {
     if (!WIDE) return;
@@ -231,7 +262,17 @@
     ref = bvh.root_ref;
     setup_space(sp, ro, rd, bvh.scene_cx, bvh.scene_cy, bvh.scene_cz, bvh.scene_radius);
     orient_space();
-    if (SAVE_WORLD) {
+    if (FLAT == 2) {
+      tsp.o = sp.o;
+      tsp.Sx = sp.Sx;
+      tsp.Sy = sp.Sy;
+      tsp.Sz = sp.Sz;
+      tsp.k = sp.k;
+      tspace = 0u;
+    } else if (FLAT) {
+      tspace = 0xFFFFFFFFu;
+    }
+    if (SAVE_WORLD && FLAT != 2) {
       w_idir = sp.idir;
       w_noodL = sp.noodL;
       w_noodH = sp.noodH;
@@ -318,6 +359,12 @@
           cnt.st[1] += (uint32_t)__popcll(leaf);
           cnt.st[2] += (uint32_t)__popcll(here & ~walking & ~leaf);
           cnt.st[3] += 64u - (uint32_t)__popcll(here);
+        }
+        const unsigned long long done = __ballot(ref == TRAV_DONE), leaving = __ballot(ref == TRAV_EXIT_INSTANCE);
+        if (first_active_lane()) {
+          cnt.stop[0] += (uint32_t)__popcll(done);
+          cnt.stop[1] += (uint32_t)__popcll(leaving);
+          cnt.stop[2] += (uint32_t)__popcll(here & ~walking & ~leaf & ~done & ~leaving);
         }
       }
       if (!(ref & BVH_LEAF_BIT)) {
@@ -378,7 +425,7 @@
   }
 
   DEV void leaf_step(const DeviceBvh& bvh, uint32_t* stack, TraverseCounters& cnt) {
-    const bool entries_due = ENTRY_BATCH > 1 ? !__any(ref < TRAV_EXIT_INSTANCE && !(ref & BVH_INST_BIT)) : true;
+    const bool entries_due = ENTRY_BATCH > 1 && FLAT != 2 ? !__any(ref < TRAV_EXIT_INSTANCE && !(ref & BVH_INST_BIT)) : true;
     if (COUNT) {
       const unsigned long long tri = __ballot(is_tri_leaf(ref));
       if (first_active_lane()) {
@@ -386,6 +433,10 @@
         cnt.st[5] += (uint32_t)__popcll(tri);
         cnt.st[6] += (uint32_t)__popcll(__ballot(true) & ~tri);
       }
+    }
+    if (FLAT == 2) {
+      if (ref != TRAV_DONE) triangles_step(bvh, stack, cnt);
+      return;
     }
     if (special_step(bvh, stack, cnt, entries_due)) return;
     triangles_step(bvh, stack, cnt);
@@ -417,6 +468,7 @@
         const uint32_t entering = (uint32_t)__popcll(__ballot(true));
         if (entering < ENTRY_BATCH && !entries_due) return true;
       }
+      if (COUNT) cnt.stop[3]++;
       const TlasEntry* e = bvh.entries + (ref & 0xFFFFu);
       const float4* ev = reinterpret_cast<const float4*>(e);
       const uint4 info = *reinterpret_cast<const uint4*>(ev + 3);
@@ -488,7 +540,26 @@
       if (first_active_lane()) cnt.tri_slots += 64;
     }
     float t, b1, b2;
-    bool candidate = tri_test(sp, xyz(v0), xyz(v1), xyz(v2), tmin, tmax, t, b1, b2);
+    bool candidate;
+    if (FLAT) {
+      const bool flat = (FLAT == 2 || bvh.flat_inv != nullptr) && (__float_as_uint(v2.w) & BVH_TRI_FLAT_BIT);
+      const uint32_t space = FLAT == 2 || flat ? tri_space_of(v0, v2) : 0u;
+      if ((FLAT == 2 || flat) && space != tspace) {
+        make_tri_space(tsp, bvh.flat_inv, space, o, d);
+        tspace = space;
+      }
+      TriSpace use = tsp;
+      if (FLAT != 2 && !flat) {
+        use.o = sp.o;
+        use.Sx = sp.Sx;
+        use.Sy = sp.Sy;
+        use.Sz = sp.Sz;
+        use.k = sp.k;
+      }
+      candidate = tri_test(use, xyz(v0), xyz(v1), xyz(v2), tmin, tmax, t, b1, b2);
+    } else {
+      candidate = tri_test(sp, xyz(v0), xyz(v1), xyz(v2), tmin, tmax, t, b1, b2);
+    }
     if (ALPHA && candidate) {
       const uint32_t mask = bvh.alpha_test ? bvh.inst_alpha[(__float_as_uint(v0.w) | id_bits) & 0xFFFFu] : BVH_NO_ALPHA;
       if (mask != BVH_NO_ALPHA) {
@@ -534,7 +605,7 @@
 #ifndef STHIP_WIDE8_STRIDE
 #define STHIP_WIDE8_STRIDE 80u
 #endif
-template <bool COUNT, uint32_t STRIDE, bool ALPHA, bool BOUNDED, uint32_t ENTRY_BATCH, bool SAVE_WORLD = false>
+template <bool COUNT, uint32_t STRIDE, bool ALPHA, bool BOUNDED, uint32_t ENTRY_BATCH, bool SAVE_WORLD = false, bool FLAT = false>
 struct Traversal8 {
   uint32_t limit;
   bool any;
@@ -550,6 +621,8 @@
   uint32_t top;
   uint32_t id_bits;
   uint32_t tri_min;
+  TriSpace tsp;
+  uint32_t tspace;
 
   static DEV uint2* column(uint32_t* stack) { return reinterpret_cast<uint2*>(stack); }
   DEV bool overflowed(const uint32_t* stack) const { return BOUNDED && reinterpret_cast<const uint2*>(stack)[limit].x != W8_CANARY; }
@@ -588,6 +661,7 @@
     tx = ty = 0u;
     setup_space(sp, ro, rd, bvh.scene_cx, bvh.scene_cy, bvh.scene_cz, bvh.scene_radius);
     orient_space();
+    if (FLAT) tspace = 0xFFFFFFFFu;
     if (SAVE_WORLD) {
       w_idir = sp.idir;
       w_noodL = sp.noodL;
@@ -707,7 +781,26 @@
       if (first_active_lane()) cnt.tri_slots += 64;
     }
     float t, b1, b2;
-    bool candidate = tri_test(sp, xyz(v0), xyz(v1), xyz(v2), tmin, tmax, t, b1, b2);
+    bool candidate;
+    if (FLAT) {
+      const bool flat = bvh.flat_inv != nullptr && (__float_as_uint(v2.w) & BVH_TRI_FLAT_BIT);
+      const uint32_t space = flat ? tri_space_of(v0, v2) : 0u;
+      if (flat && space != tspace) {
+        make_tri_space(tsp, bvh.flat_inv, space, o, d);
+        tspace = space;
+      }
+      TriSpace use = tsp;
+      if (!flat) {
+        use.o = sp.o;
+        use.Sx = sp.Sx;
+        use.Sy = sp.Sy;
+        use.Sz = sp.Sz;
+        use.k = sp.k;
+      }
+      candidate = tri_test(use, xyz(v0), xyz(v1), xyz(v2), tmin, tmax, t, b1, b2);
+    } else {
+      candidate = tri_test(sp, xyz(v0), xyz(v1), xyz(v2), tmin, tmax, t, b1, b2);
+    }
     if (ALPHA && candidate) {
       const uint32_t mask = bvh.alpha_test ? bvh.inst_alpha[(__float_as_uint(v0.w) | id_bits) & 0xFFFFu] : BVH_NO_ALPHA;
       if (mask != BVH_NO_ALPHA) {
@@ -851,7 +944,7 @@
 
 template <int MODE, bool COUNT, uint32_t STRIDE, bool ALPHA = false>
 DEV bool traverse(const DeviceBvh& bvh, f3 o, f3 d, float tmin, float tmax, uint32_t* stack, RayHit& hit, TraverseCounters& cnt) {
-  Traversal<MODE, COUNT, STRIDE, ALPHA> tr;
+  Traversal<MODE, COUNT, STRIDE, ALPHA, false, false, false, 1, false, 1> tr;
   tr.any = MODE == TRAV_ANY;
   tr.start(bvh, stack, o, d, tmin, tmax);
   while (tr.active()) tr.round(bvh, stack, 1, cnt);
diff --git a/stratum_amd/wire.py b/stratum_amd/wire.py
--- a/stratum_amd/wire.py
+++ b/stratum_amd/wire.py
@@ -227,6 +227,7 @@
         ("max_paths_in_flight", C.c_uint64),
         ("batch_halvings", C.c_uint32),
         ("full_rebuilds", C.c_uint32),
+        ("lane_stops", C.c_uint64 * 4),
     ]
 
 
```
